# Alanlee0323/ISWM

Hardware: AMD Instinct MI355X
Metric: training images/sec (513x513) DeepLabV3+-ResNet101 (higher is better)
Workload: dtype f32; 1 GPU; deeplabv3plus_resnet101 output_stride=16, 513x513 synthetic tiles, 16 images/GPU (BASELINE.json configs[2]: global batch 128 over 8 GPUs), weighted CE [1,3], SGD-nesterov + cosine LR; fp32 tensors, conv products via six bf16 MFMAs on an exact 3-way operand split (bf16x6, fp32-level error); conv_math=bf16x6, global_batch=16, parallelism=dp1

## Files before the change

### include/iswm_hip.h

```cpp
#ifndef ISWM_HIP_H
#define ISWM_HIP_H

#include <stddef.h>
#include <stdint.h>

#ifdef __cplusplus
extern "C" {
#endif

typedef void* iswm_stream_t;

const char* iswm_last_error(void);
int iswm_version(void);

typedef struct {
    int N, H, W, Cin;
    int Ho, Wo, Cout;
    int KH, KW, stride, pad, dil;
    int ldx;
    int ldy;
} iswm_conv_desc;

int iswm_set_conv_math(int mode);
int iswm_get_conv_math(void);
int iswm_conv2d_kernel_name(const iswm_conv_desc* d, int kind, char* buf, int buflen);
int iswm_conv2d_stat_tile_rows(const iswm_conv_desc* d);
int iswm_conv2d_stat_tiles(const iswm_conv_desc* d);
int iswm_conv2d_fwd(const iswm_conv_desc* d, const float* x, const float* w, const float* bias,
                    float* y, float* stat_partials, iswm_stream_t stream);
int iswm_conv2d_dgrad(const iswm_conv_desc* d, const float* dy, const float* w, float* dx,
                      int accumulate, iswm_stream_t stream);
int iswm_transpose_weights(const iswm_conv_desc* d, const float* w, float* wt, iswm_stream_t stream);
int iswm_conv2d_dgrad_wants_wt(const iswm_conv_desc* d);
int iswm_conv2d_dgrad_wt(const iswm_conv_desc* d, const float* dy, const float* wt, float* dx, int accumulate,
                         iswm_stream_t stream);
size_t iswm_conv2d_packed_weight_bytes(const iswm_conv_desc* d, int kind);
int iswm_conv2d_pack_weights(const iswm_conv_desc* d, int kind, const float* w, void* packed, iswm_stream_t stream);
typedef struct iswm_pack_job {
    const float* w;
    void* packed;
    int Cout, taps, Cin, kind;
    int first_block, reserved;
} iswm_pack_job;
size_t iswm_packed_weight_bytes(int Cout, int taps, int Cin, int kind);
int iswm_pack_job_blocks(int Cout, int taps, int Cin, int kind);
int iswm_pack_weights_batch(const iswm_pack_job* jobs_dev, int njobs, int total_blocks, iswm_stream_t stream);
int iswm_conv2d_fwd_packed_stat_layout(const iswm_conv_desc* d, int* tiles, int* tile_rows);
int iswm_conv2d_fwd_packed(const iswm_conv_desc* d, const float* x, const void* wpk, const float* bias,
                           float* y, float* stat_partials, iswm_stream_t stream);
int iswm_conv2d_dgrad_packed(const iswm_conv_desc* d, const float* dy, const void* wpk, float* dx, int accumulate,
                             iswm_stream_t stream);
int iswm_split_planes(const float* x, int64_t M, int C, int ldx, void* planes, int ldp, int64_t plane_stride,
                      iswm_stream_t stream);
int iswm_join_planes(const void* planes, int ldp, int64_t plane_stride, int64_t M, int C, float* x, int ldx,
                     iswm_stream_t stream);
int iswm_bn_apply_pl(const float* y, int64_t M, int C, int ldy, const float* scale, const float* shift, const float* mean,
                     const void* residual, int ldr, int64_t res_ps, int relu, void* out, int ldo, int64_t out_ps,
                     iswm_stream_t stream);
int iswm_bn_backward_pl(const float* dout, int ldd, const void* out, int ldo, int64_t out_ps, const float* y, int ldy,
                        int64_t M, int C, const float* mean, const float* invstd, const float* gamma,
                        const float* mask_scale, const float* mask_shift, int relu, int training, float* dgamma,
                        float* dbeta, void* dy, int lddy, int64_t dy_ps, float* dres, int lddres, void* workspace,
                        size_t workspace_bytes, iswm_stream_t stream);
int iswm_maxpool3x3s2_fwd_pl(const float* x, int N, int H, int W, int C, void* y, int64_t y_ps, uint8_t* idx, int Ho,
                             int Wo, iswm_stream_t stream);
int iswm_gap_fwd_pl(const void* x, int64_t x_ps, int N, int HW, int C, int ldx, float* y, iswm_stream_t stream);
int iswm_bcast_fwd_pl(const float* v, int N, int HW, int C, void* y, int ldy, int64_t y_ps, iswm_stream_t stream);
int iswm_bilinear_fwd_pl(const float* x, int N, int Hi, int Wi, int C, int ldx, void* y, int64_t y_ps, int Ho, int Wo,
                         int ldy, iswm_stream_t stream);
size_t iswm_conv2d_pl2_weight_bytes(const iswm_conv_desc* d, int kind);
int iswm_conv2d_pl2_pack_weights(const iswm_conv_desc* d, int kind, const float* w, void* packed, iswm_stream_t stream);
int iswm_conv2d_pl2_tile_rows(const iswm_conv_desc* d, int kind);
int iswm_conv2d_fwd_pl2(const iswm_conv_desc* d, const void* xp, int64_t plane_stride, const void* wpk,
                        const float* bias, float* y, float* stat_partials, iswm_stream_t stream);
int iswm_conv2d_dgrad_pl2(const iswm_conv_desc* d, const void* dyp, int64_t plane_stride, const void* wpk,
                          float* dx, int accumulate, iswm_stream_t stream);
int iswm_conv2d_dgrad_pl2_stat_tiles(const iswm_conv_desc* d);
int iswm_conv2d_dgrad_pl2_bn(const iswm_conv_desc* d, const void* dyp, int64_t plane_stride, const void* wpk, float* dx,
                             int accumulate, const float* y, int ldy, const float* mean, const float* invstd,
                             const float* mask_scale, const float* mask_shift, int relu, const void* mask_hi,
                             int ld_mask, double* partials, int tiles, iswm_stream_t stream);
int iswm_bn_backward_stats_pl(const float* dout, int ldd, const void* out, int ldo, int64_t out_ps, const float* y, int ldy,
                              int64_t M, int C, const float* mean, const float* invstd, const float* gamma,
                              const float* mask_scale, const float* mask_shift, int relu, int training, float* dgamma,
                              float* dbeta, void* dy, int lddy, int64_t dy_ps, float* dres, int lddres,
                              const double* partials, int tiles, void* workspace, size_t workspace_bytes,
                              iswm_stream_t stream);
size_t iswm_aspp_plan_bytes(const iswm_conv_desc* d, int nbranch, const int* ksize, const int* dil, int kind);
int iswm_aspp_plan(const iswm_conv_desc* d, int nbranch, const int* ksize, const int* dil, int kind, void* host_plan,
                   int grid_hint);
int iswm_aspp_fwd(const iswm_conv_desc* d, int nbranch, const int* ksize, const int* dil, const void* plan_dev, const void* xp,
                  int64_t x_ps, const void* const* wpk, float* const* y, float* const* stats, iswm_stream_t stream);
int iswm_aspp_bwd(const iswm_conv_desc* d, int nbranch, const int* ksize, const int* dil, const void* plan_dev, const void* dyp,
                  int64_t dy_ps, int ld_dy, const void* const* wpk, float* dx, int accumulate, const void* xp, int64_t x_ps,
                  float* const* dw, float* workspace, size_t workspace_bytes, iswm_stream_t stream);
int iswm_conv2d_wgrad_planes_ok(const iswm_conv_desc* d);
size_t iswm_conv2d_wgrad_planes_workspace(const iswm_conv_desc* d);
int iswm_conv2d_wgrad_planes(const iswm_conv_desc* d, const void* xp, int64_t x_ps, const void* dyp, int64_t dy_ps, float* dw,
                             float* workspace, size_t workspace_bytes, iswm_stream_t stream);
int iswm_dwconv2d_fwd(const iswm_conv_desc* d, const float* x, const float* w, int Cw, const float* bias, float* y,
                      iswm_stream_t stream);
int iswm_dwconv2d_dgrad(const iswm_conv_desc* d, const float* dy, const float* w, int Cw, float* dx, int accumulate,
                        iswm_stream_t stream);
size_t iswm_dwconv2d_wgrad_workspace(const iswm_conv_desc* d);
int iswm_dwconv2d_wgrad(const iswm_conv_desc* d, const float* x, const float* dy, int Cw, float* dw, void* workspace,
                        size_t workspace_bytes, iswm_stream_t stream);
int iswm_dwconv3x3_stat_tile_rows(const iswm_conv_desc* d);
int iswm_dwconv3x3_stat_tiles(const iswm_conv_desc* d);
int iswm_dwconv3x3_fwd_stats(const iswm_conv_desc* d, const float* x, const float* w, int Cw, float* y,
                             float* stat_partials, iswm_stream_t stream);
size_t iswm_dwconv3x3_bwd_workspace(const iswm_conv_desc* d);
int iswm_dwconv3x3_bwd(const iswm_conv_desc* d, const float* x, const float* dy, const float* w, int Cw, float* dx,
                       int lddx, int accumulate, float* dw, void* workspace, size_t workspace_bytes, iswm_stream_t stream);
size_t iswm_conv2d_wgrad_workspace(const iswm_conv_desc* d);
int iswm_conv2d_wgrad(const iswm_conv_desc* d, const float* x, const float* dy, float* dw,
                      float* workspace, size_t workspace_bytes, iswm_stream_t stream);

int iswm_colstat_tiles(int64_t M);
int64_t iswm_colstat_tile_rows(int64_t M);
int iswm_colstat(const float* x, int64_t M, int C, int ld, float* partials, iswm_stream_t stream);
int iswm_bn_finalize(const float* partials, int tiles, int C, int64_t count, int64_t tile_rows,
                     const float* gamma, const float* beta, float* running_mean, float* running_var, float momentum,
                     float eps, float* scale, float* shift, float* save_mean, float* save_invstd,
                     iswm_stream_t stream);
int iswm_bn_eval_coeffs(int C, const float* gamma, const float* beta, const float* running_mean,
                        const float* running_var, float eps, float* scale, float* shift,
                        float* save_mean, float* save_invstd, iswm_stream_t stream);
int iswm_bn_apply(const float* y, int64_t M, int C, int ldy, const float* scale, const float* shift,
                  const float* mean, const float* residual, int ldr, int relu, float* out, int ldo,
                  iswm_stream_t stream);
size_t iswm_bn_bwd_workspace(int64_t M, int C);
int iswm_bn_backward(const float* dout, int ldd, const float* out, int ldo, const float* y, int ldy,
                     int64_t M, int C, const float* mean, const float* invstd, const float* gamma,
                     const float* mask_scale, const float* mask_shift,
                     int relu, int training, float* dgamma, float* dbeta, float* dy, int lddy,
                     float* dres, int lddres, void* workspace, size_t workspace_bytes,
                     iswm_stream_t stream);
int iswm_colsum_finalize(const float* partials, int tiles, int C, float* out, float* scratch,
                         iswm_stream_t stream);

int iswm_maxpool3x3s2_fwd(const float* x, int N, int H, int W, int C, float* y, uint8_t* idx, int Ho,
                          int Wo, iswm_stream_t stream);
int iswm_maxpool3x3s2_bwd(const float* dy, const uint8_t* idx, int N, int H, int W, int C, int Ho,
                          int Wo, float* dx, iswm_stream_t stream);
int iswm_gap_fwd(const float* x, int N, int HW, int C, int ldx, float* y, iswm_stream_t stream);
int iswm_gap_bwd(const float* dy, int N, int HW, int C, float* dx, int lddx, int accumulate,
                 iswm_stream_t stream);
int iswm_bcast_fwd(const float* v, int N, int HW, int C, float* y, int ldy, iswm_stream_t stream);
int iswm_bcast_bwd(const float* dy, int lddy, int N, int HW, int C, float* dv, iswm_stream_t stream);

int iswm_bilinear_fwd(const float* x, int N, int Hi, int Wi, int C, int ldx, float* y, int Ho, int Wo,
                      int ldy, iswm_stream_t stream);
int iswm_bilinear_bwd(const float* dy, int N, int Hi, int Wi, int C, int lddy, int Ho, int Wo, float* dx,
                      int lddx, iswm_stream_t stream);
int iswm_bilinear_nhwc_to_nchw_fwd(const float* x, int N, int Hi, int Wi, int C, int ldx, float* y,
                                   int Ho, int Wo, iswm_stream_t stream);
int iswm_bilinear_nhwc_to_nchw_bwd(const float* dy, int N, int Hi, int Wi, int C, int lddx, int Ho,
                                   int Wo, float* dx, iswm_stream_t stream);

int iswm_nchw_to_nhwc(const float* x, int N, int C, int HW, float* y, int Cp, iswm_stream_t stream);
int iswm_nhwc_to_nchw(const float* x, int N, int C, int HW, int ldx, float* y, iswm_stream_t stream);
int iswm_copy_channels(const float* src, int lds, float* dst, int ldd, int64_t M, int C,
                       iswm_stream_t stream);
int iswm_add_inplace(float* dst, const float* src, int64_t n, iswm_stream_t stream);
int iswm_scale_inplace(float* x, int64_t n, const float* scalar_dev, float host_mul, iswm_stream_t stream);
int iswm_bn_apply_classify(const float* y, int64_t M, int C, int ldy, const float* scale, const float* shift, const float* mean,
                           const float* wc4, const float* bias4, float* logits, int ldl, iswm_stream_t stream);
size_t iswm_bn_classify_bwd_workspace(int64_t M, int C);
int iswm_bn_backward_classify(const float* dlogit, int ldl, const float* wc4, const float* y, int ldy, int64_t M, int C,
                              const float* mean, const float* invstd, const float* gamma, const float* mask_scale,
                              const float* mask_shift, int training, float* dgamma, float* dbeta, float* dwc4, void* dy, int lddy,
                              int64_t dy_ps, void* workspace, size_t workspace_bytes, iswm_stream_t stream);
int iswm_pad_weights(const float* w, int cout, int cin, int kh, int kw, const int64_t* strides, int cout_p, int cin_p, float* out_ohwi,
                     iswm_stream_t stream);
int iswm_unpad_weights(const float* dw_ohwi, int cout_p, int cin_p, int cout, int cin, int kh, int kw, float* grad,
                       const int64_t* strides, iswm_stream_t stream);
int iswm_fill_zero(void* p, size_t bytes, iswm_stream_t stream);
int iswm_zero_cols(void* y, int64_t M, int64_t ld_bytes, int byte0, int byte1, int64_t plane_bytes, int nplanes, iswm_stream_t stream);
int iswm_dropout_fwd(const float* x, float* y, uint8_t* mask, int64_t n, float p, uint64_t seed,
                     uint64_t offset, iswm_stream_t stream);
int iswm_dropout_bwd(const float* dy, const uint8_t* mask, float* dx, int64_t n, float p,
                     iswm_stream_t stream);

int iswm_loss_blocks(int64_t npix);
int iswm_loss_fwd(const float* logits, const void* labels, int label_bytes, int B, int C, int64_t HW,
                  const float* class_weight, int ignore_index, float alpha, float gamma, int mode,
                  float* grad_unnorm, float* partials, iswm_stream_t stream);
int iswm_loss_finalize(const float* partials, int blocks, int mode, int64_t npix, float* sums,
                       float* loss, iswm_stream_t stream);
int iswm_loss_bwd_scale(float* grad, int64_t n, const float* sums, const float* upstream, int mode,
                        int64_t npix, iswm_stream_t stream);
int iswm_argmax_nchw(const float* logits, int B, int C, int64_t HW, int64_t* out, iswm_stream_t stream);

int iswm_confusion_matrix(const void* labels, int label_dtype, const void* preds, int pred_dtype, int64_t npix,
                          int n_classes, int64_t* hist, iswm_stream_t stream);
int iswm_confusion_matrix_logits(const void* labels, int label_dtype, const float* logits, int B, int C, int64_t HW,
                                 int n_classes, int64_t* hist, iswm_stream_t stream);

int iswm_mask_morph(const void* src, int src_dtype, int N, int H, int W, int radius, int dilate, uint8_t* dst,
                    iswm_stream_t stream);
int iswm_ccl(const uint8_t* mask, int N, int H, int W, int32_t* labels, int32_t* areas, iswm_stream_t stream);
size_t iswm_mask_preprocess_workspace(int N, int H, int W);
int iswm_mask_preprocess(const void* src, int src_dtype, int N, int H, int W, uint8_t* out, double* weight,
                         int64_t* area, void* workspace, size_t workspace_bytes, iswm_stream_t stream);
int iswm_mask_fronts(const uint8_t* mask, const double* weight, int N, int H, int W, int32_t* fronts, int64_t* stats,
                     iswm_stream_t stream);
int iswm_front_error(const int32_t* pred_fronts, const int32_t* gt_fronts, int N, int H, double tau, double* out,
                     iswm_stream_t stream);
int iswm_mask_pair_scores(const int32_t* curr_fronts, const int64_t* curr_stats, const uint8_t* prev_mask,
                          const double* prev_weight, const int64_t* prev_stats, int N, int H, int W, double* stability,
                          double* motion, iswm_stream_t stream);
size_t iswm_region_workspace(int N, int H, int W);
int iswm_region_score(const void* pred, int pred_dtype, const void* gt, int gt_dtype, int N, int H, int W, double* score,
                      int32_t* valid, void* workspace, size_t workspace_bytes, iswm_stream_t stream);

typedef struct iswm_aug_sample {
    long long img_off;
    long long lbl_off;
    int src_h, src_w;
    int rs_h, rs_w;
    int pad;
    int crop_i, crop_j;
    int flip;
    int tab_off;
    int ksize_h, ksize_v;
    int reserved;
} iswm_aug_sample;
int iswm_augment_batch(const unsigned char* images, const unsigned char* labels, const void* samples,
                       const int* tables, int B, int crop_h, int crop_w, const float* mean3, const float* std3,
                       float* out_nchw, unsigned char* out_labels, iswm_stream_t stream);

size_t iswm_label_prepare_workspace(long long nbytes);
int iswm_label_prepare(unsigned char* labels, long long nbytes, long long* counts, void* workspace,
                       size_t workspace_bytes, iswm_stream_t stream);
size_t iswm_label_count_workspace(long long n);
int iswm_label_count(const unsigned char* labels, long long n, int ignore_index, long long* counts_accum,
                     void* workspace, size_t workspace_bytes, iswm_stream_t stream);
size_t iswm_aug_tables_workspace(const void* host_samples, int B);
int iswm_aug_tables(const void* samples, int B, int max_rs, int* tables, size_t tables_bytes, iswm_stream_t stream);
int iswm_gather_normalize(const unsigned char* images, const unsigned char* labels, const long long* offsets, int B,
                          int H, int W, const float* mean3, const float* std3, float* out_nchw,
                          unsigned char* out_labels, iswm_stream_t stream);

int iswm_predict_normalize(const unsigned char* img, int N, int H, int W, const float* mean3, const float* std3,
                           float* out_nchw, iswm_stream_t stream);
size_t iswm_predict_maps_workspace(int N, int H, int W);
int iswm_predict_maps(const float* yl, int N, int Hi, int Wi, int ldx, int C, int fg, int Ho, int Wo, float thr,
                      int band_lo, int band_hi, unsigned char* pred, unsigned char* conf, unsigned char* band,
                      float* prob, double* stats, void* workspace, size_t workspace_bytes, iswm_stream_t stream);

typedef struct {
    int N, H, W, Cin;
    int Ho, Wo, Cout;
    int KH, KW, stride, pad, dil;
    int ldx;
    int ldy;
    int ldr;
    int relu;
    int lo;
    int out_f32;
    int cstore;
} iswm_qconv_desc;
size_t iswm_qconv_weight_bytes(const iswm_qconv_desc* d);
int iswm_qconv_fwd(const iswm_qconv_desc* d, const signed char* x, const signed char* w, const double* mul,
                   const double* add, const signed char* res, double s_res, double inv_s_out, void* y,
                   iswm_stream_t stream);
size_t iswm_absmax_workspace(int64_t rows, int C);
int iswm_absmax(const void* x, int64_t ps, int64_t rows, int C, int ld, float* slab, size_t slab_bytes, float* amax,
                iswm_stream_t stream);
int iswm_quantize_i8(const void* x, int64_t ps, int64_t rows, int C, int ld, double inv_s, int lo, signed char* y,
                     int ldy, iswm_stream_t stream);
int iswm_qgap(const signed char* x, int N, int HW, int C, int ldx, double s_in, double inv_s_in, signed char* y,
              int ldy, iswm_stream_t stream);
int iswm_qbcast(const signed char* v, int N, int HW, int C, int ldv, signed char* y, int ldy, iswm_stream_t stream);
int iswm_qbilinear(const signed char* x, int N, int Hi, int Wi, int C, int ldx, double s_in, int Ho, int Wo,
                   double inv_s_out, signed char* y, int ldy, iswm_stream_t stream);

int iswm_sgd_step(float* p, const float* g, float* buf, int64_t n, const float* lr_dev, float momentum,
                  float weight_decay, int nesterov, iswm_stream_t stream);
int iswm_adam_step(float* p, const float* g, float* m, float* v, int64_t n, const float* hyper_dev,
                   float beta1, float beta2, float eps, float weight_decay, int decoupled,
                   iswm_stream_t stream);

#ifdef __cplusplus
}
#endif
#endif
```

### iswm_amd/_lib.py

```python
import ctypes
import os
from ctypes import POINTER, Structure, c_char_p, c_double, c_float, c_int, c_int64, c_size_t, c_uint64, c_void_p

HERE = os.path.dirname(os.path.abspath(__file__))
LIB_PATH = os.path.join(HERE, "libiswm_hip.so")


class ConvDesc(Structure):
    _fields_ = [(n, c_int) for n in ("N", "H", "W", "Cin", "Ho", "Wo", "Cout", "KH", "KW", "stride", "pad",
                                     "dil", "ldx", "ldy")]


class QConvDesc(Structure):
    _fields_ = [(n, c_int) for n in ("N", "H", "W", "Cin", "Ho", "Wo", "Cout", "KH", "KW", "stride", "pad",
                                     "dil", "ldx", "ldy", "ldr", "relu", "lo", "out_f32", "cstore")]


P = c_void_p
_SIGS = {
    "iswm_last_error": (c_char_p, []),
    "iswm_version": (c_int, []),
    "iswm_set_conv_math": (c_int, [c_int]),
    "iswm_get_conv_math": (c_int, []),
    "iswm_conv2d_kernel_name": (c_int, [POINTER(ConvDesc), c_int, c_char_p, c_int]),
    "iswm_conv2d_stat_tile_rows": (c_int, [POINTER(ConvDesc)]),
    "iswm_conv2d_stat_tiles": (c_int, [POINTER(ConvDesc)]),
    "iswm_conv2d_fwd": (c_int, [POINTER(ConvDesc), P, P, P, P, P, P]),
    "iswm_conv2d_dgrad": (c_int, [POINTER(ConvDesc), P, P, P, c_int, P]),
    "iswm_transpose_weights": (c_int, [POINTER(ConvDesc), P, P, P]),
    "iswm_conv2d_dgrad_wants_wt": (c_int, [POINTER(ConvDesc)]),
    "iswm_conv2d_dgrad_wt": (c_int, [POINTER(ConvDesc), P, P, P, c_int, P]),
    "iswm_conv2d_packed_weight_bytes": (c_size_t, [POINTER(ConvDesc), c_int]),
    "iswm_conv2d_pack_weights": (c_int, [POINTER(ConvDesc), c_int, P, P, P]),
    "iswm_packed_weight_bytes": (c_size_t, [c_int, c_int, c_int, c_int]),
    "iswm_pack_job_blocks": (c_int, [c_int, c_int, c_int, c_int]),
    "iswm_pack_weights_batch": (c_int, [P, c_int, c_int, P]),
    "iswm_conv2d_fwd_packed_stat_layout": (c_int, [POINTER(ConvDesc), POINTER(c_int), POINTER(c_int)]),
    "iswm_conv2d_fwd_packed": (c_int, [POINTER(ConvDesc), P, P, P, P, P, P]),
    "iswm_conv2d_dgrad_packed": (c_int, [POINTER(ConvDesc), P, P, P, c_int, P]),
    "iswm_split_planes": (c_int, [P, c_int64, c_int, c_int, P, c_int, c_int64, P]),
    "iswm_join_planes": (c_int, [P, c_int, c_int64, c_int64, c_int, P, c_int, P]),
    "iswm_bn_apply_pl": (c_int, [P, c_int64, c_int, c_int, P, P, P, P, c_int, c_int64, c_int, P, c_int, c_int64, P]),
    "iswm_bn_backward_pl": (c_int, [P, c_int, P, c_int, c_int64, P, c_int, c_int64, c_int, P, P, P, P, P, c_int, c_int, P, P, P,
                                    c_int, c_int64, P, c_int, P, c_size_t, P]),
    "iswm_maxpool3x3s2_fwd_pl": (c_int, [P, c_int, c_int, c_int, c_int, P, c_int64, P, c_int, c_int, P]),
    "iswm_gap_fwd_pl": (c_int, [P, c_int64, c_int, c_int, c_int, c_int, P, P]),
    "iswm_bcast_fwd_pl": (c_int, [P, c_int, c_int, c_int, P, c_int, c_int64, P]),
    "iswm_bilinear_fwd_pl": (c_int, [P, c_int, c_int, c_int, c_int, c_int, P, c_int64, c_int, c_int, c_int, P]),
    "iswm_conv2d_pl2_weight_bytes": (c_size_t, [POINTER(ConvDesc), c_int]),
    "iswm_conv2d_pl2_pack_weights": (c_int, [POINTER(ConvDesc), c_int, P, P, P]),
    "iswm_conv2d_pl2_tile_rows": (c_int, [POINTER(ConvDesc), c_int]),
    "iswm_conv2d_fwd_pl2": (c_int, [POINTER(ConvDesc), P, c_int64, P, P, P, P, P]),
    "iswm_conv2d_dgrad_pl2": (c_int, [POINTER(ConvDesc), P, c_int64, P, P, c_int, P]),
    "iswm_conv2d_dgrad_pl2_stat_tiles": (c_int, [POINTER(ConvDesc)]),
    "iswm_conv2d_dgrad_pl2_bn": (c_int, [POINTER(ConvDesc), P, c_int64, P, P, c_int, P, c_int, P, P, P, P, c_int, P, c_int, P,
                                         c_int, P]),
    "iswm_bn_backward_stats_pl": (c_int, [P, c_int, P, c_int, c_int64, P, c_int, c_int64, c_int, P, P, P, P, P, c_int, c_int, P, P,
                                          P, c_int, c_int64, P, c_int, P, c_int, P, c_size_t, P]),
    "iswm_aspp_plan_bytes": (c_size_t, [POINTER(ConvDesc), c_int, POINTER(c_int), POINTER(c_int), c_int]),
    "iswm_aspp_plan": (c_int, [POINTER(ConvDesc), c_int, POINTER(c_int), POINTER(c_int), c_int, P, c_int]),
    "iswm_aspp_fwd": (c_int, [POINTER(ConvDesc), c_int, POINTER(c_int), POINTER(c_int), P, P, c_int64, POINTER(c_void_p),
                              POINTER(c_void_p), POINTER(c_void_p), P]),
    "iswm_aspp_bwd": (c_int, [POINTER(ConvDesc), c_int, POINTER(c_int), POINTER(c_int), P, P, c_int64, c_int, POINTER(c_void_p), P,
                              c_int, P, c_int64, POINTER(c_void_p), P, c_size_t, P]),
    "iswm_conv2d_wgrad_planes_ok": (c_int, [POINTER(ConvDesc)]),
    "iswm_conv2d_wgrad_planes_workspace": (c_size_t, [POINTER(ConvDesc)]),
    "iswm_conv2d_wgrad_planes": (c_int, [POINTER(ConvDesc), P, c_int64, P, c_int64, P, P, c_size_t, P]),
    "iswm_conv2d_wgrad_workspace": (c_size_t, [POINTER(ConvDesc)]),
    "iswm_dwconv2d_fwd": (c_int, [POINTER(ConvDesc), P, P, c_int, P, P, P]),
    "iswm_dwconv2d_dgrad": (c_int, [POINTER(ConvDesc), P, P, c_int, P, c_int, P]),
    "iswm_dwconv2d_wgrad_workspace": (c_size_t, [POINTER(ConvDesc)]),
    "iswm_dwconv2d_wgrad": (c_int, [POINTER(ConvDesc), P, P, c_int, P, P, c_size_t, P]),
    "iswm_dwconv3x3_stat_tile_rows": (c_int, [POINTER(ConvDesc)]),
    "iswm_dwconv3x3_stat_tiles": (c_int, [POINTER(ConvDesc)]),
    "iswm_dwconv3x3_fwd_stats": (c_int, [POINTER(ConvDesc), P, P, c_int, P, P, P]),
    "iswm_dwconv3x3_bwd_workspace": (c_size_t, [POINTER(ConvDesc)]),
    "iswm_dwconv3x3_bwd": (c_int, [POINTER(ConvDesc), P, P, P, c_int, P, c_int, c_int, P, P, c_size_t, P]),
    "iswm_conv2d_wgrad": (c_int, [POINTER(ConvDesc), P, P, P, P, c_size_t, P]),
    "iswm_colstat_tiles": (c_int, [c_int64]),
    "iswm_colstat_tile_rows": (c_int64, [c_int64]),
    "iswm_colstat": (c_int, [P, c_int64, c_int, c_int, P, P]),
    "iswm_bn_finalize": (c_int, [P, c_int, c_int, c_int64, c_int64, P, P, P, P, c_float, c_float, P, P, P, P, P]),
    "iswm_bn_eval_coeffs": (c_int, [c_int, P, P, P, P, c_float, P, P, P, P, P]),
    "iswm_bn_apply": (c_int, [P, c_int64, c_int, c_int, P, P, P, P, c_int, c_int, P, c_int, P]),
    "iswm_bn_bwd_workspace": (c_size_t, [c_int64, c_int]),
    "iswm_bn_backward": (c_int, [P, c_int, P, c_int, P, c_int, c_int64, c_int, P, P, P, P, P, c_int, c_int, P, P, P, c_int,
                                 P, c_int, P, c_size_t, P]),
    "iswm_colsum_finalize": (c_int, [P, c_int, c_int, P, P, P]),
    "iswm_maxpool3x3s2_fwd": (c_int, [P, c_int, c_int, c_int, c_int, P, P, c_int, c_int, P]),
    "iswm_maxpool3x3s2_bwd": (c_int, [P, P, c_int, c_int, c_int, c_int, c_int, c_int, P, P]),
    "iswm_gap_fwd": (c_int, [P, c_int, c_int, c_int, c_int, P, P]),
    "iswm_gap_bwd": (c_int, [P, c_int, c_int, c_int, P, c_int, c_int, P]),
    "iswm_bcast_fwd": (c_int, [P, c_int, c_int, c_int, P, c_int, P]),
    "iswm_bcast_bwd": (c_int, [P, c_int, c_int, c_int, c_int, P, P]),
    "iswm_bilinear_fwd": (c_int, [P, c_int, c_int, c_int, c_int, c_int, P, c_int, c_int, c_int, P]),
    "iswm_bilinear_bwd": (c_int, [P, c_int, c_int, c_int, c_int, c_int, c_int, c_int, P, c_int, P]),
    "iswm_bilinear_nhwc_to_nchw_fwd": (c_int, [P, c_int, c_int, c_int, c_int, c_int, P, c_int, c_int, P]),
    "iswm_bilinear_nhwc_to_nchw_bwd": (c_int, [P, c_int, c_int, c_int, c_int, c_int, c_int, c_int, P, P]),
    "iswm_nchw_to_nhwc": (c_int, [P, c_int, c_int, c_int, P, c_int, P]),
    "iswm_nhwc_to_nchw": (c_int, [P, c_int, c_int, c_int, c_int, P, P]),
    "iswm_copy_channels": (c_int, [P, c_int, P, c_int, c_int64, c_int, P]),
    "iswm_add_inplace": (c_int, [P, P, c_int64, P]),
    "iswm_scale_inplace": (c_int, [P, c_int64, P, c_float, P]),
    "iswm_bn_apply_classify": (c_int, [P, c_int64, c_int, c_int, P, P, P, P, P, P, c_int, P]),
    "iswm_bn_classify_bwd_workspace": (c_size_t, [c_int64, c_int]),
    "iswm_bn_backward_classify": (c_int, [P, c_int, P, P, c_int, c_int64, c_int, P, P, P, P, P, c_int, P, P, P, P, c_int, c_int64,
                                          P, c_size_t, P]),
    "iswm_pad_weights": (c_int, [P, c_int, c_int, c_int, c_int, P, c_int, c_int, P, P]),
    "iswm_unpad_weights": (c_int, [P, c_int, c_int, c_int, c_int, c_int, c_int, P, P, P]),
    "iswm_fill_zero": (c_int, [P, c_size_t, P]),
    "iswm_zero_cols": (c_int, [P, c_int64, c_int64, c_int, c_int, c_int64, c_int, P]),
    "iswm_dropout_fwd": (c_int, [P, P, P, c_int64, c_float, c_uint64, c_uint64, P]),
    "iswm_dropout_bwd": (c_int, [P, P, P, c_int64, c_float, P]),
    "iswm_loss_blocks": (c_int, [c_int64]),
    "iswm_loss_fwd": (c_int, [P, P, c_int, c_int, c_int, c_int64, P, c_int, c_float, c_float, c_int, P, P, P]),
    "iswm_loss_finalize": (c_int, [P, c_int, c_int, c_int64, P, P, P]),
    "iswm_loss_bwd_scale": (c_int, [P, c_int64, P, P, c_int, c_int64, P]),
    "iswm_argmax_nchw": (c_int, [P, c_int, c_int, c_int64, P, P]),
    "iswm_augment_batch": (c_int, [P, P, P, P, c_int, c_int, c_int, POINTER(c_float), POINTER(c_float), P, P, P]),
    "iswm_label_prepare_workspace": (c_size_t, [c_int64]),
    "iswm_label_prepare": (c_int, [P, c_int64, P, P, c_size_t, P]),
    "iswm_label_count_workspace": (c_size_t, [c_int64]),
    "iswm_label_count": (c_int, [P, c_int64, c_int, P, P, c_size_t, P]),
    "iswm_aug_tables_workspace": (c_size_t, [P, c_int]),
    "iswm_aug_tables": (c_int, [P, c_int, c_int, P, c_size_t, P]),
    "iswm_gather_normalize": (c_int, [P, P, P, c_int, c_int, c_int, POINTER(c_float), POINTER(c_float), P, P, P]),
    "iswm_confusion_matrix": (c_int, [P, c_int, P, c_int, c_int64, c_int, P, P]),
    "iswm_confusion_matrix_logits": (c_int, [P, c_int, P, c_int, c_int, c_int64, c_int, P, P]),
    "iswm_mask_morph": (c_int, [P, c_int, c_int, c_int, c_int, c_int, c_int, P, P]),
    "iswm_ccl": (c_int, [P, c_int, c_int, c_int, P, P, P]),
    "iswm_mask_preprocess_workspace": (c_size_t, [c_int, c_int, c_int]),
    "iswm_mask_preprocess": (c_int, [P, c_int, c_int, c_int, c_int, P, P, P, P, c_size_t, P]),
    "iswm_mask_fronts": (c_int, [P, P, c_int, c_int, c_int, P, P, P]),
    "iswm_front_error": (c_int, [P, P, c_int, c_int, c_double, P, P]),
    "iswm_mask_pair_scores": (c_int, [P, P, P, P, P, c_int, c_int, c_int, P, P, P]),
    "iswm_region_workspace": (c_size_t, [c_int, c_int, c_int]),
    "iswm_region_score": (c_int, [P, c_int, P, c_int, c_int, c_int, c_int, P, P, P, c_size_t, P]),
    "iswm_predict_normalize": (c_int, [P, c_int, c_int, c_int, POINTER(c_float), POINTER(c_float), P, P]),
    "iswm_predict_maps_workspace": (c_size_t, [c_int, c_int, c_int]),
    "iswm_predict_maps": (c_int, [P, c_int, c_int, c_int, c_int, c_int, c_int, c_int, c_int, c_float, c_int, c_int, P, P,
                                  P, P, P, P, c_size_t, P]),
    "iswm_qconv_weight_bytes": (c_size_t, [POINTER(QConvDesc)]),
    "iswm_qconv_fwd": (c_int, [POINTER(QConvDesc), P, P, P, P, P, c_double, c_double, P, P]),
    "iswm_absmax_workspace": (c_size_t, [c_int64, c_int]),
    "iswm_absmax": (c_int, [P, c_int64, c_int64, c_int, c_int, P, c_size_t, P, P]),
    "iswm_quantize_i8": (c_int, [P, c_int64, c_int64, c_int, c_int, c_double, c_int, P, c_int, P]),
    "iswm_qgap": (c_int, [P, c_int, c_int, c_int, c_int, c_double, c_double, P, c_int, P]),
    "iswm_qbcast": (c_int, [P, c_int, c_int, c_int, c_int, P, c_int, P]),
    "iswm_qbilinear": (c_int, [P, c_int, c_int, c_int, c_int, c_int, c_double, c_int, c_int, c_double, P, c_int, P]),
    "iswm_sgd_step": (c_int, [P, P, P, c_int64, P, c_float, c_float, c_int, P]),
    "iswm_adam_step": (c_int, [P, P, P, P, c_int64, P, c_float, c_float, c_float, c_float, c_int, P]),
}

EXPORTS = tuple(_SIGS)
_lib = None


class IswmError(RuntimeError):
    pass


def load():
    global _lib
    if _lib is not None:
        return _lib
    if not os.path.exists(LIB_PATH):
        raise ImportError(
            "libiswm_hip.so is not built (%s). Run `python -m iswm_amd.build` (hipcc, gfx950). "
            "iswm_amd has no CPU or torch-op fallback." % LIB_PATH)
    import torch
    lib = ctypes.CDLL(LIB_PATH)
    for name, (res, args) in _SIGS.items():
        fn = getattr(lib, name)
        fn.restype = res
        fn.argtypes = args
    _lib = lib
    return lib


def call(name, *args):
    lib = load()
    rc = getattr(lib, name)(*args)
    if rc != 0:
        msg = lib.iswm_last_error()
        raise IswmError("%s failed (%d): %s" % (name, rc, msg.decode() if msg else "?"))
```

### iswm_amd/csrc/conv_mfma.hip

```cpp
#include <stdlib.h>
#include <string.h>

#include <atomic>

#include "conv_common.h"

namespace iswm {

template <int BN>
__global__ __launch_bounds__(256, 2) void k_conv_fwd(const ConvArgs a) {
    constexpr int BM = 128;
    constexpr int NB = BN / 64;
    constexpr int BROWS = BN / 32;
    __shared__ __attribute__((aligned(16))) float smem[2 * (BM + BN) * KC_PITCH];
    float* As = smem;
    float* Bs = smem + 2 * BM * KC_PITCH;

    const int t = threadIdx.x, lane = t & 63, wave = t >> 6;
    const int wm = wave >> 1, wn = wave & 1, li = lane & 31, lh = lane >> 5;
    const int L = xcd_remap(blockIdx.x, gridDim.x);
    const int mt = L / a.NT, nt = L - mt * a.NT;
    const int m0 = mt * BM, n0 = nt * BN;
    const int q = t & 7, r0 = t >> 3;

// ... 435 lines not shown
                *reinterpret_cast<float4*>(&As[(buf * 32 + ak0 + AKR * j) * BM + aq * 4]) = ra[j];
#pragma unroll
            for (int j = 0; j < BPASS; ++j)
                *reinterpret_cast<float4*>(&Bs[(buf * 32 + bk0 + BKR * j) * BN + bq * 4]) = rb[j];
        }
    };

    f32x16 acc[MB][NB];
#pragma unroll
    for (int i = 0; i < MB; ++i)
#pragma unroll
        for (int j = 0; j < NB; ++j)
#pragma unroll
            for (int r = 0; r < 16; ++r) acc[i][j][r] = 0.f;

    const int nK = (p_end - p_begin + 31) >> 5;
    int kc = 0;
    bool first = true;
    auto next = [&]() -> bool {
        for (;;) {
            if (!first) {
                ++kc;
                if (kc < nK) advance(kc);
            }
            first = false;
            if (kc >= nK) return false;
            if (!skip(kc)) return true;
        }
    };
    if constexpr (X6) {
        const int tg = lane >> 4, ti = lane & 15, tq = ti >> 2, tp = ti & 3;
        const int th = tg >> 1, tc = (tg & 1) * 16 + tp * 4;
        typedef short s16x4 __attribute__((ext_vector_type(4)));
        typedef __attribute__((address_space(3))) s16x4* lds_s16x4;
        auto tr_frag = [&](const unsigned char* plane, int pitch, int sw, int col0, int ks) -> uint4 {
            const unsigned char* p = plane + (ks * 16 + th * 8 + tq) * pitch + (((col0 + tc) * 2) ^ (tq * sw));
            s16x4 lo = __builtin_amdgcn_ds_read_tr16_b64_v4i16((lds_s16x4)(p));
            s16x4 hi = __builtin_amdgcn_ds_read_tr16_b64_v4i16((lds_s16x4)(p + 4 * pitch));
            uint2 a2 = __builtin_bit_cast(uint2, lo), b2 = __builtin_bit_cast(uint2, hi);
            return make_uint4(a2.x, a2.y, b2.x, b2.y);
        };
        bool more = next();
        if (more) gload(kc);
        while (more) {
            lstore(0);
            __syncthreads();
            const bool more2 = next();
            if (more2) gload(kc);
#pragma unroll
            for (int ks = 0; ks < 2; ++ks) {
                uint4 ah[MB], am[MB], al[MB], bh[NB], bm[NB], bl[NB];
#pragma unroll
                for (int mb = 0; mb < MB; ++mb) {
                    const int c0 = wm * (BM / 2) + mb * 32;
                    ah[mb] = tr_frag(Ax, XPA, SWA, c0, ks);
                    if constexpr (NP == 3) {
                        am[mb] = tr_frag(Ax + XPLA, XPA, SWA, c0, ks);
                        al[mb] = tr_frag(Ax + 2 * XPLA, XPA, SWA, c0, ks);
                    }
                }
#pragma unroll
                for (int nb = 0; nb < NB; ++nb) {
                    const int c0 = wn * (BN / 2) + nb * 32;
                    bh[nb] = tr_frag(Bx, XPB, SWB, c0, ks);
                    if constexpr (NP == 3) {
                        bm[nb] = tr_frag(Bx + XPLB, XPB, SWB, c0, ks);
                        bl[nb] = tr_frag(Bx + 2 * XPLB, XPB, SWB, c0, ks);
                    }
                }
#pragma unroll
                for (int mb = 0; mb < MB; ++mb)
#pragma unroll
                    for (int nb = 0; nb < NB; ++nb) {
                        f32x16 c = acc[mb][nb];
                        if constexpr (NP == 3) {
                            c = mfma_bf16(al[mb], bh[nb], c);
                            c = mfma_bf16(ah[mb], bl[nb], c);
                            c = mfma_bf16(am[mb], bm[nb], c);
                            c = mfma_bf16(am[mb], bh[nb], c);
                            c = mfma_bf16(ah[mb], bm[nb], c);
                        }
                        c = mfma_bf16(ah[mb], bh[nb], c);
                        acc[mb][nb] = c;
                    }
            }
            __syncthreads();
            more = more2;
        }
    } else {
        bool more = next();
        if (more) {
            gload(kc);
            lstore(0);
        }
        __syncthreads();
        int cur = 0;
        while (more) {
            const bool more2 = next();
            if (more2) gload(kc);
            const float* Ab = &As[(cur * 32 + lh * 4) * BM + wm * (BM / 2) + li];
            const float* Bb = &Bs[(cur * 32 + lh * 4) * BN + wn * (BN / 2) + li];
    #pragma unroll
            for (int g = 0; g < 4; ++g) {
                float af[MB][4], bf[NB][4];
    #pragma unroll
                for (int mb = 0; mb < MB; ++mb)
    #pragma unroll
                    for (int j = 0; j < 4; ++j) af[mb][j] = Ab[(g * 8 + j) * BM + mb * 32];
    #pragma unroll
                for (int nb = 0; nb < NB; ++nb)
    #pragma unroll
                    for (int j = 0; j < 4; ++j) bf[nb][j] = Bb[(g * 8 + j) * BN + nb * 32];
    #pragma unroll
                for (int j = 0; j < 4; ++j)
    #pragma unroll
                    for (int mb = 0; mb < MB; ++mb)
    #pragma unroll
                        for (int nb = 0; nb < NB; ++nb)
                            acc[mb][nb] = mfma32(af[mb][j], bf[nb][j], acc[mb][nb]);
            }
            if (more2) lstore(cur ^ 1);
            __syncthreads();
            cur ^= 1;
            more = more2;
        }
    }
    float* out = a.stats + (size_t)split * a.Cout * a.Ktot;
#pragma unroll
    for (int nb = 0; nb < NB; ++nb) {
        const int col = n0 + wn * (BN / 2) + nb * 32 + li;
        const bool cok = col < a.Ktot;
#pragma unroll
        for (int mb = 0; mb < MB; ++mb)
#pragma unroll
            for (int r = 0; r < 16; ++r) {
                int row = m0 + wm * (BM / 2) + mb * 32 + (r & 3) + 8 * (r >> 2) + 4 * lh;
                if (cok && row < a.Cout) out[(size_t)row * a.Ktot + col] = acc[mb][nb][r];
            }
    }
}

__global__ void k_reduce_slabs(const float* __restrict__ slabs, float* __restrict__ dst, int64_t n4,
                               int nsplit) {
    for (int64_t i = blockIdx.x * (int64_t)blockDim.x + threadIdx.x; i < n4;
         i += (int64_t)gridDim.x * blockDim.x) {
        const float4* p = reinterpret_cast<const float4*>(slabs) + i;
        float4 s = p[0];
        int k = 1;
        for (; k + 7 < nsplit; k += 8) {
            float4 v[8];
#pragma unroll
            for (int u = 0; u < 8; ++u) v[u] = p[(int64_t)(k + u) * n4];
#pragma unroll
            for (int u = 0; u < 8; ++u) {
                s.x += v[u].x;
                s.y += v[u].y;
                s.z += v[u].z;
                s.w += v[u].w;
            }
        }
        for (; k < nsplit; ++k) {
            const float4 v = p[(int64_t)k * n4];
            s.x += v.x;
            s.y += v.y;
            s.z += v.z;
            s.w += v.w;
        }
        reinterpret_cast<float4*>(dst)[i] = s;
    }
}

void launch_reduce_slabs(const float* slabs, float* dst, int64_t n4, int nsplit, hipStream_t s) {
    hipLaunchKernelGGL(k_reduce_slabs, dim3(stream_grid(n4, 256)), dim3(256), 0, s, slabs, dst, n4, nsplit);
}

static int validate(const iswm_conv_desc* d) {
    ISWM_REQUIRE(d != nullptr, "conv: null descriptor");
    ISWM_REQUIRE(d->N > 0 && d->H > 0 && d->W > 0 && d->Cin > 0 && d->Cout > 0, "conv: empty tensor");
    ISWM_REQUIRE(d->Cin % 4 == 0 && d->Cout % 4 == 0, "conv: Cin (%d) and Cout (%d) must be multiples of 4",
                 d->Cin, d->Cout);
    ISWM_REQUIRE(d->ldx % 4 == 0 && d->ldy % 4 == 0 && d->ldx >= d->Cin && d->ldy >= d->Cout,
                 "conv: bad pixel pitch ldx=%d ldy=%d", d->ldx, d->ldy);
    ISWM_REQUIRE(d->KH > 0 && d->KW > 0 && d->stride > 0 && d->dil > 0 && d->pad >= 0, "conv: bad geometry");
    int ho = (d->H + 2 * d->pad - d->dil * (d->KH - 1) - 1) / d->stride + 1;
    int wo = (d->W + 2 * d->pad - d->dil * (d->KW - 1) - 1) / d->stride + 1;
    ISWM_REQUIRE(ho == d->Ho && wo == d->Wo, "conv: output size %dx%d does not match geometry (%dx%d)", d->Ho,
                 d->Wo, ho, wo);
    ISWM_REQUIRE((int64_t)d->N * d->H * d->W * d->ldx < (1ll << 31) &&
                     (int64_t)d->N * d->Ho * d->Wo * d->ldy < (1ll << 31),
                 "conv: tensor exceeds 2^31 elements");
    return 0;
}

static bool use_narrow_tile(int64_t MT, int cols) {
    if (cols <= 64 || (cols % 128 != 0 && cols % 128 <= 64)) return true;
    const int64_t t128 = MT * ((cols + 127) / 128), t64 = MT * ((cols + 63) / 64);
    const double c128 = (double)((t128 + 255) / 256) * 128.0;
    const double c64 = (double)((t64 + 255) / 256) * 64.0 * 1.10;
    return c64 < c128;
}

static ConvArgs base_args(const iswm_conv_desc* d) {
    ConvArgs a{};
    a.N = d->N; a.H = d->H; a.W = d->W; a.Cin = d->Cin;
    a.Ho = d->Ho; a.Wo = d->Wo; a.Cout = d->Cout;
    a.KH = d->KH; a.KW = d->KW; a.stride = d->stride; a.pad = d->pad; a.dil = d->dil;
    a.ldx = d->ldx; a.ldy = d->ldy;
    return a;
}

struct WgradPlan {
    int bm, bn, MT, NT, nsplit, psplit;
};

static WgradPlan plan_wgrad(const iswm_conv_desc* d, bool x6) {
    WgradPlan p;
    const int Ktot = d->KH * d->KW * d->Cin;
    p.bm = (d->Cout % 128 == 0) ? 128 : 64;
    p.bn = (p.bm == 128 && (Ktot % 128 == 0 || Ktot >= 1024)) ? 128 : 64;
    if (p.bn == 64) p.bm = 64;
    p.MT = (d->Cout + p.bm - 1) / p.bm;
    p.NT = (Ktot + p.bn - 1) / p.bn;
    const int64_t P = (int64_t)d->N * d->Ho * d->Wo;
    const int64_t tiles = (int64_t)p.MT * p.NT;
    (void)x6;
    const int64_t slots = 512;
    const double chunk_us = 4.5 * (double)(p.bm * p.bn) / 16384.0;
    const double slab_us = (double)d->Cout * Ktot * 8.0 / 4.0e6;
    int64_t maxs = (P + 255) / 256;
    if (maxs > 64) maxs = 64;
    double best = 1e300;
    p.psplit = (int)((P + 31) / 32 * 32);
    p.nsplit = 1;
    for (int64_t ns = 1; ns <= maxs; ++ns) {
        int64_t ps = ((P + ns - 1) / ns + 31) / 32 * 32;
        int64_t nsp = (P + ps - 1) / ps;
        int64_t rounds = (tiles * nsp + slots - 1) / slots;
        double t = (double)rounds * (double)(ps / 32 + 3) * chunk_us + (nsp > 1 ? (double)nsp * slab_us + 5.0 : 0.0);
        if (t < best) {
            best = t;
            p.psplit = (int)ps;
            p.nsplit = (int)nsp;
        }
    }
    return p;
}

}

using namespace iswm;

static std::atomic<int> g_conv_math{-1};
static int conv_math() {
    int m = g_conv_math.load();
    if (m < 0) {
        const char* e = getenv("ISWM_CONV_MATH");
        const int env = (e && (!strcmp(e, "f32") || !strcmp(e, "0"))) ? 0
                        : (e && (!strcmp(e, "bf16") || !strcmp(e, "2"))) ? 2 : 1;
        int unset = -1;
        g_conv_math.compare_exchange_strong(unset, env);
        m = g_conv_math.load();
    }
    return m;
}
extern "C" int iswm_set_conv_math(int mode) {
    ISWM_REQUIRE(mode >= 0 && mode <= 2, "set_conv_math: mode must be 0 (f32), 1 (bf16x6) or 2 (bf16)");
    g_conv_math = mode;
    return 0;
}
extern "C" int iswm_get_conv_math(void) { return conv_math(); }
static int math_planes() { return conv_math() == 2 ? 1 : 3; }

static bool patch_plan(const iswm_conv_desc* d, bool dgrad, int* PH, int* PW) {
    if (d->stride != 1 || d->KH * d->KW <= 1) return false;
    return dgrad ? conv_patch_plan(d->H, d->W, d->KH, d->KW, d->dil, PH, PW)
                 : conv_patch_plan(d->Ho, d->Wo, d->KH, d->KW, d->dil, PH, PW);
}

static PatchArgs patch_args(const iswm_conv_desc* d, bool dgrad, int PH, int PW) {
    PatchArgs p{};
    p.N = d->N;
    p.KH = d->KH; p.KW = d->KW; p.dil = d->dil;
    p.PH = PH; p.PW = PW;
    if (!dgrad) {
        p.RH = d->Ho; p.RW = d->Wo; p.GH = d->H; p.GW = d->W; p.GC = d->Cin; p.NC = d->Cout;
        p.orgh = -d->pad; p.orgw = -d->pad; p.flip = 0; p.ldg = d->ldx; p.ldo = d->ldy;
    } else {
        p.RH = d->H; p.RW = d->W; p.GH = d->Ho; p.GW = d->Wo; p.GC = d->Cout; p.NC = d->Cin;
        p.orgh = d->pad - d->dil * (d->KH - 1); p.orgw = d->pad - d->dil * (d->KW - 1);
        p.flip = 1; p.ldg = d->ldy; p.ldo = d->ldx;
    }
    return p;
}

namespace iswm { int wgrad_pl_is_wide(const iswm_conv_desc* d); int wgrad_pl_kernel_kind(const iswm_conv_desc* d); }

static bool pl2_wide_ok(const iswm_conv_desc* d, bool dgrad) {
    if (math_planes() != 3 || (dgrad && d->stride != 1)) return false;
    return !dgrad || d->KH * d->KW * d->Cout >= 512;
}
static int pl2_K(const iswm_conv_desc* d, bool dgrad) { return d->KH * d->KW * (dgrad ? d->Cout : d->Cin); }

extern "C" int iswm_conv2d_kernel_name(const iswm_conv_desc* d, int kind, char* buf, int buflen) {
    ISWM_REQUIRE(d && buf && buflen > 0 && kind >= 0 && kind <= 7, "kernel_name: bad argument");
    if (kind == 7) {
        const int kk = wgrad_pl_kernel_kind(d);
        snprintf(buf, buflen, kk == 2 ? "k_wgrad_pls<%d>" : kk == 1 ? "k_wgrad_plw<%d>" : "k_wgrad_pl<%d>", math_planes());
        return 0;
    }
    if (kind >= 5) {
        const bool dg = kind == 6;
        const int cols = dg ? d->Cin : d->Cout;
        int rbw, wide;
        conv_pl2_plan(dg ? (int64_t)d->N * d->H * d->W : (int64_t)d->N * d->Ho * d->Wo, cols, pl2_K(d, dg), pl2_wide_ok(d, dg), &rbw, &wide);
        if (wide) snprintf(buf, buflen, "k_conv_pl2w<%d, %d, %s>", rbw, math_planes(), dg ? "true" : "false");
        else if (cols <= 64) snprintf(buf, buflen, "k_conv_pl2<%d, 2, %d, %s>", rbw / 2, math_planes(), dg ? "true" : "false");
        else snprintf(buf, buflen, "k_conv_pl2<%d, 1, %d, %s>", rbw, math_planes(), dg ? "true" : "false");
        return 0;
    }
    if (kind >= 3) {
        const bool dg = kind == 4;
        int pbm, pbn;
        if (patch_plan(d, dg, &pbm, &pbn)) {
            snprintf(buf, buflen, "k_conv_x6_patch<%s, %d>", dg ? "true" : "false", math_planes());
            return 0;
        }
        conv_pick_tile_x6(dg ? (int64_t)d->N * d->H * d->W : (int64_t)d->N * d->Ho * d->Wo, dg ? d->Cin : d->Cout,
                          d->KH * d->KW * (dg ? d->Cout : d->Cin), dg, d->KH * d->KW == 1, &pbm, &pbn);
        snprintf(buf, buflen, "k_conv_x6<%d, 64, %s, true, %d>", pbm, dg ? "true" : "false", math_planes());
        return 0;
    }
    int bm, bn;
    if (kind == 0) {
        const int64_t M = (int64_t)d->N * d->Ho * d->Wo;
        if (d->Cin % 32 == 0) {
            if (conv_math() == 1) conv_pick_tile_x6(M, d->Cout, d->KH * d->KW * d->Cin, false, d->KH * d->KW == 1, &bm, &bn);
            else conv_pick_tile(M, d->Cout, &bm, &bn);
            snprintf(buf, buflen, conv_math() == 1 ? "k_conv_x6<%d, %d, false, false, 3>" : "k_conv_fwd_u<%d, %d>", bm, bn);
        } else if (conv_math() == 1 && stem_geometry(base_args(d))) {
            snprintf(buf, buflen, "k_stem_fwd<%d>", stem_tile_rows() / 16);
        } else {
            snprintf(buf, buflen, "k_conv_fwd<%d>", use_narrow_tile((M + 127) / 128, d->Cout) ? 64 : 128);
        }
    } else if (kind == 1) {
        const int64_t M = (int64_t)d->N * d->H * d->W;
        if (d->Cout % 32 == 0) {
            if (conv_math() == 1) conv_pick_tile_x6(M, d->Cin, d->KH * d->KW * d->Cout, true, d->KH * d->KW == 1, &bm, &bn);
            else conv_pick_tile(M, d->Cin, &bm, &bn);
            if (conv_math() == 1) snprintf(buf, buflen, "k_conv_x6<%d, %d, true, false, 3>", bm, bn);
            else snprintf(buf, buflen, "k_conv_dgrad_u<%d, %d>", bm, bn);
        } else {
            snprintf(buf, buflen, "k_conv_dgrad<%d>", use_narrow_tile((M + 127) / 128, d->Cin) ? 64 : 128);
        }
    } else {
        if (conv_math() == 1 && stem_geometry(base_args(d))) {
            snprintf(buf, buflen, "k_stem_wgrad");
            return 0;
        }
        WgradPlan p = plan_wgrad(d, conv_math() >= 1);
        const bool same = d->stride == 1 && d->Ho == d->H && d->Wo == d->W;
        const int mode = (same && d->KH == 1 && d->KW == 1 && d->pad == 0) ? 2 : (same ? 1 : 0);
        snprintf(buf, buflen, "k_conv_wgrad<%d, %d, %d, %s, %d>", p.bm, p.bn, mode, conv_math() >= 1 ? "true" : "false",
                 conv_math() == 2 ? 1 : 3);
    }
    return 0;
}

extern "C" int iswm_conv2d_stat_tile_rows(const iswm_conv_desc* d) {
    if (!d) return 0;
    if (conv_math() == 1 && stem_geometry(base_args(d))) return stem_tile_rows();
    if (conv_math() == 1 && d->Cin % 32 == 0) {
        int bm, bn;
        conv_pick_tile_x6((int64_t)d->N * d->Ho * d->Wo, d->Cout, d->KH * d->KW * d->Cin, false, d->KH * d->KW == 1, &bm, &bn);
        return bm;
    }
    return conv_fwd_tile_rows((int64_t)d->N * d->Ho * d->Wo, d->Cin, d->Cout);
}

extern "C" int iswm_conv2d_stat_tiles(const iswm_conv_desc* d) {
    if (!d) return 0;
    const int64_t M = (int64_t)d->N * d->Ho * d->Wo, R = iswm_conv2d_stat_tile_rows(d);
    return (int)((M + R - 1) / R);
}

extern "C" int iswm_conv2d_fwd(const iswm_conv_desc* d, const float* x, const float* w, const float* bias,
                               float* y, float* stat_partials, iswm_stream_t stream) {
    if (int e = validate(d)) return e;
    ISWM_REQUIRE(x && w && y, "conv_fwd: null pointer");
    ISWM_REQUIRE(aligned16(x) && aligned16(w) && aligned16(y), "conv_fwd: pointers must be 16-byte aligned");
    ConvArgs a = base_args(d);
    a.x = x; a.w = w; a.bias = bias; a.y = y; a.stats = stat_partials;
    a.M = d->N * d->Ho * d->Wo;
    a.Ktot = d->KH * d->KW * d->Cin;
    a.MT = (a.M + 127) / 128;
    hipStream_t s = (hipStream_t)stream;
    if (conv_math() == 1 && launch_stem_fwd(a, s)) return check_launch("stem_fwd");
    if (conv_math() == 1 && d->Cin % 32 == 0) {
        int bm, bn;
        conv_pick_tile_x6(a.M, d->Cout, a.Ktot, false, d->KH * d->KW == 1, &bm, &bn);
        if (launch_conv_fwd_x6(a, s, bm, bn)) return check_launch("conv_fwd_x6");
    }
    if (launch_conv_fwd_u(a, s)) return check_launch("conv_fwd_u");
    if (use_narrow_tile(a.MT, d->Cout)) {
        a.NT = (d->Cout + 63) / 64;
        hipLaunchKernelGGL(k_conv_fwd<64>, dim3(a.MT * a.NT), dim3(256), 0, s, a);
    } else {
        a.NT = (d->Cout + 127) / 128;
        hipLaunchKernelGGL(k_conv_fwd<128>, dim3(a.MT * a.NT), dim3(256), 0, s, a);
    }
    return check_launch("conv_fwd");
}

extern "C" int iswm_conv2d_dgrad(const iswm_conv_desc* d, const float* dy, const float* w, float* dx,
                                 int accumulate, iswm_stream_t stream) {
    if (int e = validate(d)) return e;
    ISWM_REQUIRE(dy && w && dx, "conv_dgrad: null pointer");
    ISWM_REQUIRE(aligned16(dy) && aligned16(w) && aligned16(dx), "conv_dgrad: pointers must be 16-byte aligned");
    ConvArgs a = base_args(d);
    a.x = dy; a.w = w; a.y = dx; a.accumulate = accumulate;
    a.ldx = d->ldy; a.ldy = d->ldx;
    a.M = d->N * d->H * d->W;
    a.Ktot = d->KH * d->KW * d->Cout;
    a.MT = (a.M + 127) / 128;
    hipStream_t s = (hipStream_t)stream;
    if (launch_conv_dgrad_u(a, s)) return check_launch("conv_dgrad_u");
    if (use_narrow_tile(a.MT, d->Cin)) {
        a.NT = (d->Cin + 63) / 64;
        hipLaunchKernelGGL(k_conv_dgrad<64>, dim3(a.MT * a.NT), dim3(256), 0, s, a);
    } else {
        a.NT = (d->Cin + 127) / 128;
        hipLaunchKernelGGL(k_conv_dgrad<128>, dim3(a.MT * a.NT), dim3(256), 0, s, a);
    }
    return check_launch("conv_dgrad");
}

extern "C" int iswm_transpose_weights(const iswm_conv_desc* d, const float* w, float* wt, iswm_stream_t stream) {
    if (int e = validate(d)) return e;
    ISWM_REQUIRE(w && wt && w != wt, "transpose_weights: bad pointer");
    launch_transpose_ohwi(w, wt, d->Cout, d->KH * d->KW, d->Cin, (hipStream_t)stream);
    return check_launch("transpose_weights");
}

extern "C" int iswm_conv2d_dgrad_wants_wt(const iswm_conv_desc* d) {
    return (d && conv_math() == 1 && d->Cout % 32 == 0) ? 1 : 0;
}

extern "C" int iswm_conv2d_dgrad_wt(const iswm_conv_desc* d, const float* dy, const float* wt, float* dx,
                                    int accumulate, iswm_stream_t stream) {
    if (int e = validate(d)) return e;
    ISWM_REQUIRE(dy && wt && dx, "conv_dgrad_wt: null pointer");
    ISWM_REQUIRE(aligned16(dy) && aligned16(wt) && aligned16(dx), "conv_dgrad_wt: pointers must be 16-byte aligned");
    ISWM_REQUIRE(d->Cout % 32 == 0, "conv_dgrad_wt: Cout must be a multiple of 32");
    ConvArgs a = base_args(d);
    a.x = dy; a.w = wt; a.y = dx; a.accumulate = accumulate;
    a.ldx = d->ldy; a.ldy = d->ldx;
    a.M = d->N * d->H * d->W;
    a.Ktot = d->KH * d->KW * d->Cout;
    int bm, bn;
    conv_pick_tile_x6(a.M, d->Cin, a.Ktot, true, d->KH * d->KW == 1, &bm, &bn);
    launch_conv_dgrad_x6(a, (hipStream_t)stream, bm, bn);
    return check_launch("conv_dgrad_x6");
}

extern "C" int iswm_conv2d_fwd_packed_stat_layout(const iswm_conv_desc* d, int* tiles, int* tile_rows) {
    ISWM_REQUIRE(d && tiles && tile_rows, "fwd_packed_stat_layout: null pointer");
    int PH, PW;
    if (patch_plan(d, false, &PH, &PW)) {
        *tiles = d->N * ((d->Ho + PH - 1) / PH) * ((d->Wo + PW - 1) / PW);
        *tile_rows = 0;
    } else {
        int bm, bn;
        const int64_t M = (int64_t)d->N * d->Ho * d->Wo;
        conv_pick_tile_x6(M, d->Cout, d->KH * d->KW * d->Cin, false, d->KH * d->KW == 1, &bm, &bn);
        *tile_rows = bm;
        *tiles = (int)((M + bm - 1) / bm);
    }
    return 0;
}

extern "C" size_t iswm_conv2d_packed_weight_bytes(const iswm_conv_desc* d, int kind) {
    if (!d || conv_math() < 1 || (kind != 0 && kind != 1)) return 0;
    const int gc = kind ? d->Cout : d->Cin;
    if (gc % 32 != 0) return 0;
    return packed_weight_bytes_x6(d->Cout, d->KH * d->KW, d->Cin, kind == 1, math_planes());
}

extern "C" int iswm_conv2d_pack_weights(const iswm_conv_desc* d, int kind, const float* w, void* packed,
                                        iswm_stream_t stream) {
    if (int e = validate(d)) return e;
    ISWM_REQUIRE(kind == 0 || kind == 1, "pack_weights: kind must be 0 (forward) or 1 (data gradient)");
    ISWM_REQUIRE(w && packed && aligned16(packed), "pack_weights: bad pointer");
    ISWM_REQUIRE((kind ? d->Cout : d->Cin) % 32 == 0, "pack_weights: gathered channel count must be a multiple of 32");
    launch_pack_weights_x6(w, packed, d->Cout, d->KH * d->KW, d->Cin, kind == 1, math_planes(), (hipStream_t)stream);
    return check_launch("pack_weights");
}

extern "C" size_t iswm_packed_weight_bytes(int Cout, int taps, int Cin, int kind) {
    if (Cout <= 0 || taps <= 0 || Cin <= 0 || kind < 0 || kind > 3 || conv_math() < 1) return 0;
    if (kind >= 2) {
        if (((kind == 3) ? Cout : Cin) % 64 != 0) return 0;
        return packed_weight_bytes_pl2(Cout, taps, Cin, kind == 3, math_planes());
    }
    if ((kind ? Cout : Cin) % 32 != 0) return 0;
    return packed_weight_bytes_x6(Cout, taps, Cin, kind == 1, math_planes());
}

extern "C" int iswm_pack_job_blocks(int Cout, int taps, int Cin, int kind) {
    if (iswm_packed_weight_bytes(Cout, taps, Cin, kind) == 0) return 0;
    if (kind >= 2) return pack_job_blocks_pl2(Cout, taps, Cin, kind == 3);
    return pack_job_blocks_x6(Cout, taps, Cin, kind == 1);
}

extern "C" int iswm_pack_weights_batch(const iswm_pack_job* jobs_dev, int njobs, int total_blocks,
                                       iswm_stream_t stream) {
    ISWM_REQUIRE(jobs_dev && njobs > 0 && total_blocks > 0, "pack_weights_batch: bad argument");
    static_assert(sizeof(iswm_pack_job) == 40, "iswm_pack_job layout");
    launch_pack_weights_batch(jobs_dev, njobs, total_blocks, math_planes(), (hipStream_t)stream);
    return check_launch("pack_weights_batch");
}

extern "C" int iswm_conv2d_fwd_packed(const iswm_conv_desc* d, const float* x, const void* wpk, const float* bias,
                                      float* y, float* stat_partials, iswm_stream_t stream) {
    if (int e = validate(d)) return e;
    ISWM_REQUIRE(x && wpk && y, "conv_fwd_packed: null pointer");
    ISWM_REQUIRE(aligned16(x) && aligned16(wpk) && aligned16(y), "conv_fwd_packed: pointers must be 16-byte aligned");
    ISWM_REQUIRE(d->Cin % 32 == 0, "conv_fwd_packed: Cin must be a multiple of 32");
    ConvArgs a = base_args(d);
    a.x = x; a.w = reinterpret_cast<const float*>(wpk); a.bias = bias; a.y = y; a.stats = stat_partials;
    a.M = d->N * d->Ho * d->Wo;
    a.Ktot = d->KH * d->KW * d->Cin;
    int PH, PW;
    if (patch_plan(d, false, &PH, &PW)) {
        PatchArgs p = patch_args(d, false, PH, PW);
        p.x = x; p.wpk = reinterpret_cast<const uint4*>(wpk); p.bias = bias; p.y = y; p.stats = stat_partials;
        launch_conv_x6_patch(p, false, math_planes(), (hipStream_t)stream);
        return check_launch("conv_fwd_patch");
    }
    int bm, bn;
    conv_pick_tile_x6(a.M, d->Cout, a.Ktot, false, d->KH * d->KW == 1, &bm, &bn);
    launch_conv_x6_pk(a, (hipStream_t)stream, false, bm, math_planes());
    return check_launch("conv_fwd_packed");
}

extern "C" int iswm_conv2d_dgrad_packed(const iswm_conv_desc* d, const float* dy, const void* wpk, float* dx,
                                        int accumulate, iswm_stream_t stream) {
    if (int e = validate(d)) return e;
    ISWM_REQUIRE(dy && wpk && dx, "conv_dgrad_packed: null pointer");
    ISWM_REQUIRE(aligned16(dy) && aligned16(wpk) && aligned16(dx), "conv_dgrad_packed: pointers must be 16-byte aligned");
    ISWM_REQUIRE(d->Cout % 32 == 0, "conv_dgrad_packed: Cout must be a multiple of 32");
    ConvArgs a = base_args(d);
    a.x = dy; a.w = reinterpret_cast<const float*>(wpk); a.y = dx; a.accumulate = accumulate;
    a.ldx = d->ldy; a.ldy = d->ldx;
    a.M = d->N * d->H * d->W;
    a.Ktot = d->KH * d->KW * d->Cout;
    int PH, PW;
    if (patch_plan(d, true, &PH, &PW)) {
        PatchArgs p = patch_args(d, true, PH, PW);
        p.x = dy; p.wpk = reinterpret_cast<const uint4*>(wpk); p.y = dx; p.accumulate = accumulate;
        launch_conv_x6_patch(p, true, math_planes(), (hipStream_t)stream);
        return check_launch("conv_dgrad_patch");
    }
    int bm, bn;
    conv_pick_tile_x6(a.M, d->Cin, a.Ktot, true, d->KH * d->KW == 1, &bm, &bn);
    launch_conv_x6_pk(a, (hipStream_t)stream, true, bm, math_planes());
    return check_launch("conv_dgrad_packed");
}

extern "C" int iswm_split_planes(const float* x, int64_t M, int C, int ldx, void* planes, int ldp, int64_t plane_stride,
                                 iswm_stream_t stream) {
    ISWM_REQUIRE(x && planes && M > 0 && C > 0, "split_planes: bad argument");
    ISWM_REQUIRE(C % 4 == 0 && ldx % 4 == 0 && ldx >= C && ldp % 4 == 0 && ldp >= C, "split_planes: C %d ldx %d ldp %d", C, ldx, ldp);
    ISWM_REQUIRE(aligned16(x) && plane_stride % 4 == 0 && plane_stride >= M * ldp,
                 "split_planes: planes must be 16-byte aligned and disjoint");
    launch_split_planes(x, M, C, ldx, (unsigned short*)planes, ldp, plane_stride, math_planes(), (hipStream_t)stream);
    return check_launch("split_planes");
}

extern "C" int iswm_join_planes(const void* planes, int ldp, int64_t plane_stride, int64_t M, int C, float* x, int ldx,
                                iswm_stream_t stream) {
    ISWM_REQUIRE(x && planes && M > 0 && C > 0, "join_planes: bad argument");
    ISWM_REQUIRE(C % 4 == 0 && ldx % 4 == 0 && ldx >= C && ldp % 4 == 0 && ldp >= C, "join_planes: C %d ldx %d ldp %d", C, ldx, ldp);
    ISWM_REQUIRE(plane_stride == -1 || plane_stride >= M * ldp, "join_planes: bad plane stride");
    launch_join_planes((const unsigned short*)planes, ldp, plane_stride, M, C, x, ldx, (hipStream_t)stream);
    return check_launch("join_planes");
}

extern "C" size_t iswm_conv2d_pl2_weight_bytes(const iswm_conv_desc* d, int kind) {
    if (!d || conv_math() < 1 || (kind != 0 && kind != 1)) return 0;
    const int gc = kind ? d->Cout : d->Cin;
    if (gc % 64 != 0) return 0;
    return packed_weight_bytes_pl2(d->Cout, d->KH * d->KW, d->Cin, kind == 1, math_planes());
}

extern "C" int iswm_conv2d_pl2_pack_weights(const iswm_conv_desc* d, int kind, const float* w, void* packed,
                                            iswm_stream_t stream) {
    if (int e = validate(d)) return e;
    ISWM_REQUIRE(kind == 0 || kind == 1, "pl2_pack_weights: kind must be 0 (forward) or 1 (data gradient)");
    ISWM_REQUIRE(w && packed && aligned16(packed), "pl2_pack_weights: bad pointer");
    ISWM_REQUIRE((kind ? d->Cout : d->Cin) % 64 == 0, "pl2_pack_weights: gathered channel count must be a multiple of 64");
    launch_pack_weights_pl2(w, packed, d->Cout, d->KH * d->KW, d->Cin, kind == 1, math_planes(), (hipStream_t)stream);
    return check_launch("pl2_pack_weights");
}

extern "C" int iswm_conv2d_pl2_tile_rows(const iswm_conv_desc* d, int kind) {
    if (!d) return 0;
    int rbw, wide;
    if (kind) conv_pl2_plan((int64_t)d->N * d->H * d->W, d->Cin, pl2_K(d, true), pl2_wide_ok(d, true), &rbw, &wide);
// ... 134 lines not shown
```

### iswm_amd/csrc/conv_wgrad_pl.hip

```cpp
#include <stdlib.h>

#include <algorithm>
#include <type_traits>

#include "conv_common.h"

namespace iswm {

static __device__ __attribute__((aligned(256))) unsigned short g_zero_row_wg[128];

struct WgArgs {
    const unsigned short* dy;
    const unsigned short* x;
    float* out;
    long long dyps, xps;
    int N, H, W, Cin, Ho, Wo, Cout, KH, KW, stride, pad, dil, ldx, ldy;
    int P, Ktot, MT, NT, nsplit, psplit;
    int always;
    int vote;
    int rect;
    unsigned char tap_order[32];
};

template <int NP>
// ... 117 lines not shown
#pragma unroll
        for (int mb = 0; mb < 2; ++mb)
#pragma unroll
            for (int pl = 0; pl < NP; ++pl) af[mb][pl] = tr_frag(Ax + pl * PLANE, wm * 64 + mb * 32);
#pragma unroll
        for (int nb = 0; nb < 2; ++nb)
#pragma unroll
            for (int pl = 0; pl < NP; ++pl) bf[nb][pl] = tr_frag(Bx + pl * PLANE, wn * 64 + nb * 32);
#pragma unroll
        for (int mb = 0; mb < 2; ++mb)
#pragma unroll
            for (int nb = 0; nb < 2; ++nb) {
                f32x16 c = acc[mb][nb];
                if constexpr (NP == 3) {
                    c = mfma_bf16(af[mb][2], bf[nb][0], c);
                    c = mfma_bf16(af[mb][0], bf[nb][2], c);
                    c = mfma_bf16(af[mb][1], bf[nb][1], c);
                    c = mfma_bf16(af[mb][1], bf[nb][0], c);
                    c = mfma_bf16(af[mb][0], bf[nb][1], c);
                }
                c = mfma_bf16(af[mb][0], bf[nb][0], c);
                acc[mb][nb] = c;
            }
    };

    {
        int nissued = 0, wr = 0, rd = 0;
        bool src_more = true;
        auto advance = [&]() __attribute__((always_inline)) -> bool {
            if (src_more && next()) return true;
            src_more = false;
            return false;
        };
        auto post = [&]() __attribute__((always_inline)) {
            issue(wr);
            wr = wr == NST - 1 ? 0 : wr + 1;
            ++nissued;
        };
        if (advance()) post();
        if (advance()) post();
        while (nissued > 0) {
            if (nissued >= 2) {
                if constexpr (NP == 3) __builtin_amdgcn_s_waitcnt(0x0F76);
                else __builtin_amdgcn_s_waitcnt(0x0F72);
            } else {
                __builtin_amdgcn_s_waitcnt(0x0F70);
            }
            __builtin_amdgcn_s_barrier();
            asm volatile("" ::: "memory");
            if (advance()) post();
            compute(rd);
            rd = rd == NST - 1 ? 0 : rd + 1;
            --nissued;
        }
    }

    __syncthreads();
    float* xch = reinterpret_cast<float*>(smem);
    if (kh == 1) {
#pragma unroll
        for (int mb = 0; mb < 2; ++mb)
#pragma unroll
            for (int nb = 0; nb < 2; ++nb)
#pragma unroll
                for (int r = 0; r < 16; ++r) xch[((((wm * 2 + wn) * 2 + mb) * 2 + nb) * 16 + r) * 64 + lane] = acc[mb][nb][r];
    }
    __syncthreads();
    if (kh == 0) {
        float* out = a.out + (size_t)split * a.Cout * a.Ktot;
        const int li = lane & 31, lh = lane >> 5;
#pragma unroll
        for (int nb = 0; nb < 2; ++nb) {
            const int col = n0 + wn * 64 + nb * 32 + li;
            const bool cok = col < a.Ktot;
#pragma unroll
            for (int mb = 0; mb < 2; ++mb)
#pragma unroll
                for (int r = 0; r < 16; ++r) {
                    const int row = m0 + wm * 64 + mb * 32 + (r & 3) + 8 * (r >> 2) + 4 * lh;
                    const float v = acc[mb][nb][r] + xch[((((wm * 2 + wn) * 2 + mb) * 2 + nb) * 16 + r) * 64 + lane];
                    if (cok && row < a.Cout) out[(size_t)row * a.Ktot + col] = v;
                }
        }
    }
}


template <int NP>
__global__ __launch_bounds__(512, 2) void k_wgrad_plw(const WgArgs a) {
    constexpr int PLANE = 32 * 256;
    constexpr int IMG = NP * PLANE;
    constexpr int STAGE = 3 * IMG;
    constexpr int NST = 2;
    constexpr int SMEM = NST * STAGE < 65536 ? 65536 : NST * STAGE;
    __shared__ __attribute__((aligned(1024))) unsigned char smem[SMEM];
    const unsigned lds_base = (unsigned)(uintptr_t)(lds_vptr)smem;

    const int t = threadIdx.x, lane = t & 63;
    const int wave = __builtin_amdgcn_readfirstlane(t >> 6);
    const int wm = wave >> 2, wn = wave & 3;
    const int tiles = a.MT * a.NT;
    const int L = xcd_remap(blockIdx.x, gridDim.x);
    const int split = L / tiles, tile = L - split * tiles;
    const int mt = tile / a.NT, nt = tile - mt * a.NT;
    const int m0 = mt * 128, n0 = nt * 256;
    const int p_begin = split * a.psplit;
    const int p_end = min(a.P, p_begin + a.psplit);
    const int nK = (p_end - p_begin + 31) >> 5;

    const int kr = 4 * wave + (lane >> 4);
    const int gsrc = (lane & 15) ^ (4 * ((lane >> 4) & 3));
    const unsigned char* zrow = reinterpret_cast<const unsigned char*>(g_zero_row_wg) + (lane & 15) * 16;
    const int ach = m0 + 8 * gsrc;
    const bool aok = ach < a.Cout;
    const unsigned char* abase = reinterpret_cast<const unsigned char*>(a.dy) + (size_t)ach * 2;
    bool bok[2];
    int dh[2], dw[2];
    const unsigned char* bbase[2];
#pragma unroll
    for (int i = 0; i < 2; ++i) {
        const int bcol = n0 + 128 * i + 8 * gsrc;
        bok[i] = bcol < a.Ktot;
        const int tap = bok[i] ? bcol / a.Cin : 0, bch = bok[i] ? bcol - tap * a.Cin : 0;
        const int tkh = tap / a.KW, tkw = tap - tkh * a.KW;
        dh[i] = tkh * a.dil - a.pad;
        dw[i] = tkw * a.dil - a.pad;
        bbase[i] = reinterpret_cast<const unsigned char*>(a.x) + (size_t)bch * 2;
    }
    const int HoWo = a.Ho * a.Wo;

    const unsigned char* asrc = zrow;
    const unsigned char* bsrc[2] = {zrow, zrow};
    long long apst = 0, bpst[2] = {0, 0};
    int kc = -1;
    int pn, poh, pow_;
    {
        const int p = p_begin + kr;
        pn = p / HoWo;
        const int rem = p - pn * HoWo;
        poh = rem / a.Wo;
        pow_ = rem - poh * a.Wo;
    }
    const int d_oh = 32 / a.Wo, d_ow = 32 - d_oh * a.Wo;
    const bool fast_adv = d_oh + 1 <= a.Ho;
    auto next = [&]() __attribute__((always_inline)) -> bool {
        for (;;) {
            if (++kc >= nK) return false;
            const int p = p_begin + kc * 32 + kr;
            const bool pin = p < p_end;
            asrc = (pin && aok) ? abase + (size_t)p * a.ldy * 2 : zrow;
            apst = (pin && aok) ? a.dyps : 0;
            if (a.always) {
#pragma unroll
                for (int i = 0; i < 2; ++i) {
                    const bool v = pin && bok[i];
                    bsrc[i] = v ? bbase[i] + (size_t)p * a.ldx * 2 : zrow;
                    bpst[i] = v ? a.xps : 0;
                }
                return true;
            }
            if (kc > 0) {
                if (fast_adv) {
                    int ow = pow_ + d_ow;
                    const int c1 = ow >= a.Wo ? 1 : 0;
                    pow_ = ow - (c1 ? a.Wo : 0);
                    int oh = poh + d_oh + c1;
                    const int c2 = oh >= a.Ho ? 1 : 0;
                    poh = oh - (c2 ? a.Ho : 0);
                    pn += c2;
                } else {
                    pn = p / HoWo;
                    const int rem = p - pn * HoWo;
                    poh = rem / a.Wo;
                    pow_ = rem - poh * a.Wo;
                }
            }
            bool any = false;
#pragma unroll
            for (int i = 0; i < 2; ++i) {
                const int ih = poh * a.stride + dh[i], iw = pow_ * a.stride + dw[i];
                const bool v = pin && bok[i] && (unsigned)ih < (unsigned)a.H && (unsigned)iw < (unsigned)a.W;
                bsrc[i] = v ? bbase[i] + (size_t)((pn * a.H + ih) * a.W + iw) * a.ldx * 2 : zrow;
                bpst[i] = v ? a.xps : 0;
                any = any || v;
            }
            if (!a.vote) return true;
            if (__syncthreads_or(any ? 1 : 0)) return true;
        }
    };
    auto dma = [&](int i, int st) __attribute__((always_inline)) {
        const int img = i / NP, pl = i - img * NP;
        const unsigned dst = lds_base + st * STAGE + img * IMG + pl * PLANE + wave * 1024;
        if (img == 0) glds16b(asrc + pl * apst, dst);
        else glds16b(bsrc[img - 1] + pl * bpst[img - 1], dst);
    };
    auto issue = [&](int st) __attribute__((always_inline)) {
#pragma unroll
        for (int i = 0; i < 3 * NP; ++i) dma(i, st);
    };

    const int tg = lane >> 4, ti = lane & 15, tq = ti >> 2, tp = ti & 3;
    const int th = tg >> 1, tc = (tg & 1) * 16 + tp * 4;
    typedef short s16x4 __attribute__((ext_vector_type(4)));
    typedef __attribute__((address_space(3))) s16x4* lds_s16x4;
    auto tr_frag = [&](const unsigned char* plane, int ks, int col0) __attribute__((always_inline)) -> uint4 {
        const unsigned char* p = plane + (ks * 16 + th * 8 + tq) * 256 + (((col0 + tc) * 2) ^ (tq * 64));
        s16x4 lo = __builtin_amdgcn_ds_read_tr16_b64_v4i16((lds_s16x4)(p));
        s16x4 hi = __builtin_amdgcn_ds_read_tr16_b64_v4i16((lds_s16x4)(p + 4 * 256));
        uint2 a2 = __builtin_bit_cast(uint2, lo), b2 = __builtin_bit_cast(uint2, hi);
        return make_uint4(a2.x, a2.y, b2.x, b2.y);
    };

    f32x16 acc[2][2];
#pragma unroll
    for (int i = 0; i < 2; ++i)
#pragma unroll
        for (int j = 0; j < 2; ++j)
#pragma unroll
            for (int r = 0; r < 16; ++r) acc[i][j][r] = 0.f;

    uint4 F[4][NP];
    auto ldA = [&](int st, int mb, int ks) __attribute__((always_inline)) {
        const unsigned char* Ax = smem + st * STAGE;
#pragma unroll
        for (int pl = 0; pl < NP; ++pl) F[mb][pl] = tr_frag(Ax + pl * PLANE, ks, wm * 64 + mb * 32);
    };
    auto ldB = [&](int st, int nb, int ks) __attribute__((always_inline)) {
        const unsigned char* Bx = smem + st * STAGE + (1 + (wn >> 1)) * IMG;
#pragma unroll
        for (int pl = 0; pl < NP; ++pl) F[2 + nb][pl] = tr_frag(Bx + pl * PLANE, ks, (wn & 1) * 64 + nb * 32);
    };
    auto mm = [&](int mb, int nb) __attribute__((always_inline)) {
        f32x16 c = acc[mb][nb];
        if constexpr (NP == 3) {
            c = mfma_bf16(F[mb][2], F[2 + nb][0], c);
            c = mfma_bf16(F[mb][0], F[2 + nb][2], c);
            c = mfma_bf16(F[mb][1], F[2 + nb][1], c);
            c = mfma_bf16(F[mb][1], F[2 + nb][0], c);
            c = mfma_bf16(F[mb][0], F[2 + nb][1], c);
        }
        c = mfma_bf16(F[mb][0], F[2 + nb][0], c);
        acc[mb][nb] = c;
    };
    auto compute = [&](int st) __attribute__((always_inline)) {
#define ISWM_SB() __builtin_amdgcn_sched_barrier(0)
        ldA(st, 0, 0); ldB(st, 0, 0);
        ISWM_SB(); ldB(st, 1, 0); ISWM_SB(); mm(0, 0); ISWM_SB();
        ISWM_SB(); ldA(st, 1, 0); ISWM_SB(); mm(0, 1); ISWM_SB();
        ISWM_SB(); ldA(st, 0, 1); ISWM_SB(); mm(1, 1); ISWM_SB();
        ISWM_SB(); ldB(st, 1, 1); ISWM_SB(); mm(1, 0); ISWM_SB();
        ISWM_SB(); ldB(st, 0, 1); ISWM_SB(); mm(0, 1); ISWM_SB();
        ISWM_SB(); ldA(st, 1, 1); ISWM_SB(); mm(0, 0); ISWM_SB();
        ISWM_SB(); mm(1, 0); ISWM_SB();
        ISWM_SB(); mm(1, 1); ISWM_SB();
        ISWM_SB();
#undef ISWM_SB
    };

    {
        bool have = next();
        if (have) issue(0);
        int st = 0;
        while (have) {
            __builtin_amdgcn_s_waitcnt(0x0F70);
            __builtin_amdgcn_s_barrier();
            asm volatile("" ::: "memory");
            const bool more = next();
            if (more) issue(st ^ 1);
            compute(st);
            st ^= 1;
            have = more;
        }
    }

    if (a.nsplit > 1) {
        float4* slab = reinterpret_cast<float4*>(a.out) + ((size_t)split * tiles + tile) * 8192 + (size_t)wave * 1024 + lane;
#pragma unroll
        for (int mb = 0; mb < 2; ++mb)
#pragma unroll
            for (int nb = 0; nb < 2; ++nb)
#pragma unroll
                for (int q = 0; q < 4; ++q)
                    slab[((mb * 2 + nb) * 4 + q) * 64] =
                        make_float4(acc[mb][nb][4 * q], acc[mb][nb][4 * q + 1], acc[mb][nb][4 * q + 2], acc[mb][nb][4 * q + 3]);
        return;
    }
    float* out = a.out;
    const int li = lane & 31, lh = lane >> 5;
#pragma unroll
    for (int nb = 0; nb < 2; ++nb) {
        const int col = n0 + wn * 64 + nb * 32 + li;
        const bool cok = col < a.Ktot;
#pragma unroll
        for (int mb = 0; mb < 2; ++mb)
#pragma unroll
            for (int r = 0; r < 16; ++r) {
                const int row = m0 + wm * 64 + mb * 32 + (r & 3) + 8 * (r >> 2) + 4 * lh;
                if (cok && row < a.Cout) out[(size_t)row * a.Ktot + col] = acc[mb][nb][r];
            }
    }
}

template <int NP>
__global__ __launch_bounds__(512, 2) void k_wgrad_pls(const WgArgs a) {
    constexpr int MW = 4;
    constexpr int KS = 16;
    constexpr int PLANE = KS * 256;
    constexpr int IMG = NP * PLANE;
    constexpr int STAGE = 3 * IMG;
    constexpr int NST = 4;
    __shared__ __attribute__((aligned(1024))) unsigned char smem[NST * STAGE];
    const unsigned lds_base = (unsigned)(uintptr_t)(lds_vptr)smem;

    const int t = threadIdx.x, lane = t & 63;
    const int wave = __builtin_amdgcn_readfirstlane(t >> 6);
    const int tiles = a.MT * a.NT;
    const int L = xcd_remap(blockIdx.x, gridDim.x);
    int split = L / tiles, tile = L - split * tiles;
    int mt = tile / a.NT;
    int nt = tile - mt * a.NT;
    if (a.rect == 2) {
        const int idx = blockIdx.x >> 3, per_split = (a.NT >> 3) * a.MT;
        split = idx / per_split;
        const int rem = idx - split * per_split;
        mt = rem % a.MT;
        nt = (rem / a.MT) * 8 + (blockIdx.x & 7);
    }
    int r_oh0 = 0, r_ow0 = 0, r_h = a.Ho, r_w = a.Wo, r_dh = 0, r_dw = 0;
    int p_begin = split * a.psplit;
    int p_end = min(a.P, p_begin + a.psplit);
    if (a.rect) {
        const int chunks = a.Cin >> 8;
        const int slot = nt / chunks;
        const int tap = a.tap_order[slot];
        nt = tap * chunks + (nt - slot * chunks);
        const int tkh = tap / a.KW, tkw = tap - tkh * a.KW;
        r_dh = tkh * a.dil - a.pad;
        r_dw = tkw * a.dil - a.pad;
        r_oh0 = max(0, -r_dh);
        r_ow0 = max(0, -r_dw);
        r_h = max(0, min(a.Ho, a.H - r_dh) - r_oh0);
        r_w = max(0, min(a.Wo, a.W - r_dw) - r_ow0);
        const int Pt = a.N * r_h * r_w;
        const int per = (((Pt + a.nsplit - 1) / a.nsplit) + KS - 1) / KS * KS;
        p_begin = split * per;
        p_end = min(Pt, p_begin + per);
    }
    const int m0 = mt * 128, n0 = nt * 256;
    const int nK = p_end > p_begin ? (p_end - p_begin + KS - 1) / KS : 0;

    if (wave >= MW) {
        const int rg = wave - MW;
        const int kr = 4 * rg + (lane >> 4);
        const int gsrc = (lane & 15) ^ (4 * ((lane >> 4) & 3));
        const unsigned char* zrow = reinterpret_cast<const unsigned char*>(g_zero_row_wg) + (lane & 15) * 16;
        const int ach = m0 + 8 * gsrc;
        const bool aok = ach < a.Cout;
        const unsigned char* abase = reinterpret_cast<const unsigned char*>(a.dy) + (size_t)ach * 2;
        bool bok[2];
        int dh[2], dw[2];
        const unsigned char* bbase[2];
#pragma unroll
        for (int i = 0; i < 2; ++i) {
            const int bcol = n0 + 128 * i + 8 * gsrc;
            bok[i] = bcol < a.Ktot;
            const int tap = bok[i] ? bcol / a.Cin : 0, bch = bok[i] ? bcol - tap * a.Cin : 0;
            const int tkh = tap / a.KW, tkw = tap - tkh * a.KW;
            dh[i] = tkh * a.dil - a.pad;
            dw[i] = tkw * a.dil - a.pad;
            bbase[i] = reinterpret_cast<const unsigned char*>(a.x) + (size_t)bch * 2;
        }
        const int GW_ = max(1, r_w), GHW = max(1, r_h * r_w);
        int pn, poh, pow_;
        {
            const int p = p_begin + kr;
            pn = p / GHW;
            const int rem = p - pn * GHW;
            poh = rem / GW_;
            pow_ = rem - poh * GW_;
        }
        const int d_oh = KS / GW_, d_ow = KS - d_oh * GW_;
        const bool fast_adv = d_oh + 1 <= r_h;
        auto issue = [&](int kc) __attribute__((always_inline)) {
            const int p = p_begin + kc * KS + kr;
            const bool pin = p < p_end;
            const unsigned char* asrc;
            long long apst;
            const unsigned char* bsrc[2];
            long long bpst[2];
            if (a.rect) {
                if (kc > 0) {
                    if (fast_adv) {
                        int ow = pow_ + d_ow;
                        const int c1 = ow >= GW_ ? 1 : 0;
                        pow_ = ow - (c1 ? GW_ : 0);
                        int oh = poh + d_oh + c1;
                        const int c2 = oh >= r_h ? 1 : 0;
                        poh = oh - (c2 ? r_h : 0);
                        pn += c2;
                    } else {
                        pn = p / GHW;
                        const int rem = p - pn * GHW;
                        poh = rem / GW_;
                        pow_ = rem - poh * GW_;
                    }
                }
                const int oh = r_oh0 + poh, ow = r_ow0 + pow_;
                const bool va = pin && aok;
                asrc = va ? abase + (size_t)((pn * a.Ho + oh) * a.Wo + ow) * a.ldy * 2 : zrow;
                apst = va ? a.dyps : 0;
                const size_t xpix = (size_t)((pn * a.H + oh + r_dh) * a.W + ow + r_dw);
#pragma unroll
                for (int i = 0; i < 2; ++i) {
                    const bool v = pin && bok[i];
                    bsrc[i] = v ? bbase[i] + xpix * a.ldx * 2 : zrow;
                    bpst[i] = v ? a.xps : 0;
                }
                const unsigned dstr = lds_base + (kc & 3) * STAGE + rg * 1024;
#pragma unroll
                for (int pl = 0; pl < NP; ++pl) glds16b(asrc + pl * apst, dstr + pl * PLANE);
#pragma unroll
                for (int i = 0; i < 2; ++i)
#pragma unroll
                    for (int pl = 0; pl < NP; ++pl) glds16b(bsrc[i] + pl * bpst[i], dstr + (1 + i) * IMG + pl * PLANE);
                return;
            }
            asrc = (pin && aok) ? abase + (size_t)p * a.ldy * 2 : zrow;
            apst = (pin && aok) ? a.dyps : 0;
            if (a.always) {
#pragma unroll
                for (int i = 0; i < 2; ++i) {
                    const bool v = pin && bok[i];
                    bsrc[i] = v ? bbase[i] + (size_t)p * a.ldx * 2 : zrow;
                    bpst[i] = v ? a.xps : 0;
                }
            } else {
                if (kc > 0) {
                    if (fast_adv) {
                        int ow = pow_ + d_ow;
                        const int c1 = ow >= GW_ ? 1 : 0;
                        pow_ = ow - (c1 ? GW_ : 0);
                        int oh = poh + d_oh + c1;
                        const int c2 = oh >= r_h ? 1 : 0;
                        poh = oh - (c2 ? r_h : 0);
                        pn += c2;
                    } else {
                        pn = p / GHW;
                        const int rem = p - pn * GHW;
                        poh = rem / GW_;
                        pow_ = rem - poh * GW_;
                    }
                }
#pragma unroll
                for (int i = 0; i < 2; ++i) {
                    const int ih = poh * a.stride + dh[i], iw = pow_ * a.stride + dw[i];
                    const bool v = pin && bok[i] && (unsigned)ih < (unsigned)a.H && (unsigned)iw < (unsigned)a.W;
                    bsrc[i] = v ? bbase[i] + (size_t)((pn * a.H + ih) * a.W + iw) * a.ldx * 2 : zrow;
                    bpst[i] = v ? a.xps : 0;
                }
            }
            const unsigned dst = lds_base + (kc & 3) * STAGE + rg * 1024;
#pragma unroll
            for (int pl = 0; pl < NP; ++pl) glds16b(asrc + pl * apst, dst + pl * PLANE);
#pragma unroll
            for (int i = 0; i < 2; ++i)
#pragma unroll
                for (int pl = 0; pl < NP; ++pl) glds16b(bsrc[i] + pl * bpst[i], dst + (1 + i) * IMG + pl * PLANE);
        };
        const int pre = nK < 3 ? nK : 3;
        for (int kc = 0; kc < pre; ++kc) issue(kc);
        for (int s2 = 0; s2 < nK; ++s2) {
            const int beyond = min(nK - 1, s2 + 2) - s2;
            if constexpr (NP == 3) {
                if (beyond >= 2) __builtin_amdgcn_s_waitcnt(0x4F72);
                else if (beyond == 1) __builtin_amdgcn_s_waitcnt(0x0F79);
                else __builtin_amdgcn_s_waitcnt(0x0F70);
            } else {
                if (beyond >= 2) __builtin_amdgcn_s_waitcnt(0x0F76);
                else if (beyond == 1) __builtin_amdgcn_s_waitcnt(0x0F73);
                else __builtin_amdgcn_s_waitcnt(0x0F70);
            }
            __builtin_amdgcn_s_barrier();
            asm volatile("" ::: "memory");
            if (s2 + 3 < nK) issue(s2 + 3);
        }
        return;
    }

    constexpr int NBW = 4;
    const int wm = wave >> 1;
    const int wn4 = 2 * (wave & 1);
    const int tg = lane >> 4, ti = lane & 15, tq = ti >> 2, tp = ti & 3;
    const int th = tg >> 1, tc = (tg & 1) * 16 + tp * 4;
    typedef short s16x4 __attribute__((ext_vector_type(4)));
    typedef __attribute__((address_space(3))) s16x4* lds_s16x4;
    auto tr_frag = [&](const unsigned char* plane, int col0) __attribute__((always_inline)) -> uint4 {
        const unsigned char* p = plane + (th * 8 + tq) * 256 + (((col0 + tc) * 2) ^ (tq * 64));
        s16x4 lo = __builtin_amdgcn_ds_read_tr16_b64_v4i16((lds_s16x4)(p));
        s16x4 hi = __builtin_amdgcn_ds_read_tr16_b64_v4i16((lds_s16x4)(p + 4 * 256));
        uint2 a2 = __builtin_bit_cast(uint2, lo), b2 = __builtin_bit_cast(uint2, hi);
        return make_uint4(a2.x, a2.y, b2.x, b2.y);
    };
    f32x16 acc[2][NBW];
#pragma unroll
    for (int i = 0; i < 2; ++i)
#pragma unroll
        for (int j = 0; j < NBW; ++j)
#pragma unroll
            for (int r = 0; r < 16; ++r) acc[i][j][r] = 0.f;
    uint4 FA[2][NP], FB[NBW][NP];
    auto ldA = [&](int slot, int mb) __attribute__((always_inline)) {
        const unsigned char* Ax = smem + slot * STAGE;
#pragma unroll
        for (int pl = 0; pl < NP; ++pl) FA[mb][pl] = tr_frag(Ax + pl * PLANE, wm * 64 + mb * 32);
    };
    auto ldB = [&](int slot, int nb) __attribute__((always_inline)) {
        const unsigned char* Bx = smem + slot * STAGE + (1 + (wn4 >> 1)) * IMG;
#pragma unroll
        for (int pl = 0; pl < NP; ++pl) FB[nb][pl] = tr_frag(Bx + pl * PLANE, (wn4 & 1) * 64 + nb * 32);
    };
    auto mm = [&](int mb, int nb) __attribute__((always_inline)) {
        f32x16 c = acc[mb][nb];
        if constexpr (NP == 3) {
            c = mfma_bf16(FA[mb][2], FB[nb][0], c);
            c = mfma_bf16(FA[mb][0], FB[nb][2], c);
            c = mfma_bf16(FA[mb][1], FB[nb][1], c);
            c = mfma_bf16(FA[mb][1], FB[nb][0], c);
            c = mfma_bf16(FA[mb][0], FB[nb][1], c);
        }
        c = mfma_bf16(FA[mb][0], FB[nb][0], c);
        acc[mb][nb] = c;
    };
#define ISWM_SB() __builtin_amdgcn_sched_barrier(0)
    for (int s2 = 0; s2 < nK; ++s2) {
        __builtin_amdgcn_s_barrier();
        asm volatile("" ::: "memory");
        const int slot = s2 & 3;
        ldA(slot, 0); ldB(slot, 0);
        ISWM_SB(); ldB(slot, 1); ISWM_SB(); mm(0, 0); ISWM_SB();
        ISWM_SB(); ldB(slot, 2); ISWM_SB(); mm(0, 1); ISWM_SB();
        ISWM_SB(); ldB(slot, 3); ISWM_SB(); mm(0, 2); ISWM_SB();
        ISWM_SB(); ldA(slot, 1); ISWM_SB(); mm(0, 3); ISWM_SB();
        ISWM_SB(); mm(1, 3); ISWM_SB();
        ISWM_SB(); mm(1, 2); ISWM_SB();
        ISWM_SB(); mm(1, 1); ISWM_SB();
        ISWM_SB(); mm(1, 0); ISWM_SB();
    }
#undef ISWM_SB

    if (a.nsplit > 1) {
        float4* slab = reinterpret_cast<float4*>(a.out) + ((size_t)split * tiles + (mt * a.NT + nt)) * 8192 + lane;
#pragma unroll
        for (int mb = 0; mb < 2; ++mb)
#pragma unroll
            for (int nb = 0; nb < NBW; ++nb) {
                const int w8 = wm * 4 + wn4 + (nb >> 1);
#pragma unroll
                for (int q = 0; q < 4; ++q)
                    slab[(size_t)w8 * 1024 + ((mb * 2 + (nb & 1)) * 4 + q) * 64] =
                        make_float4(acc[mb][nb][4 * q], acc[mb][nb][4 * q + 1], acc[mb][nb][4 * q + 2], acc[mb][nb][4 * q + 3]);
            }
        return;
    }
    float* out = a.out;
    const int li = lane & 31, lh = lane >> 5;
#pragma unroll
    for (int nb = 0; nb < NBW; ++nb) {
        const int col = n0 + wn4 * 64 + nb * 32 + li;
        const bool cok = col < a.Ktot;
#pragma unroll
        for (int mb = 0; mb < 2; ++mb)
#pragma unroll
            for (int r = 0; r < 16; ++r) {
                const int row = m0 + wm * 64 + mb * 32 + (r & 3) + 8 * (r >> 2) + 4 * lh;
                if (cok && row < a.Cout) out[(size_t)row * a.Ktot + col] = acc[mb][nb][r];
            }
    }
}

__global__ __launch_bounds__(256) void k_reduce_slabs_frag(const float4* __restrict__ slabs, float* __restrict__ dw, int tiles,
                                                           int NT, int nsplit, int Cout, int Ktot) {
    const int64_t total = (int64_t)tiles * 8192;
    for (int64_t i = blockIdx.x * (int64_t)blockDim.x + threadIdx.x; i < total; i += (int64_t)gridDim.x * blockDim.x) {
        float4 s = slabs[i];
        int k = 1;
        for (; k + 3 < nsplit; k += 4) {
            const float4 v0 = slabs[i + (int64_t)k * total], v1 = slabs[i + (int64_t)(k + 1) * total];
            const float4 v2 = slabs[i + (int64_t)(k + 2) * total], v3 = slabs[i + (int64_t)(k + 3) * total];
            s.x += v0.x; s.y += v0.y; s.z += v0.z; s.w += v0.w;
            s.x += v1.x; s.y += v1.y; s.z += v1.z; s.w += v1.w;
            s.x += v2.x; s.y += v2.y; s.z += v2.z; s.w += v2.w;
            s.x += v3.x; s.y += v3.y; s.z += v3.z; s.w += v3.w;
        }
        for (; k < nsplit; ++k) {
            const float4 v = slabs[i + (int64_t)k * total];
            s.x += v.x; s.y += v.y; s.z += v.z; s.w += v.w;
        }
        const int tile = (int)(i >> 13), f = (int)(i & 8191);
        const int wave = f >> 10, j = (f >> 6) & 15, lane = f & 63;
        const int mt = tile / NT, nt = tile - mt * NT;
        const int wm = wave >> 2, wn = wave & 3, mb = j >> 3, nb = (j >> 2) & 1, q = j & 3;
        const int col = nt * 256 + wn * 64 + nb * 32 + (lane & 31);
        const int row = mt * 128 + wm * 64 + mb * 32 + 8 * q + 4 * (lane >> 5);
        if (col < Ktot) {
            float* o = dw + (size_t)row * Ktot + col;
            if (row < Cout) o[0] = s.x;
            if (row + 1 < Cout) o[(size_t)Ktot] = s.y;
            if (row + 2 < Cout) o[(size_t)2 * Ktot] = s.z;
            if (row + 3 < Cout) o[(size_t)3 * Ktot] = s.w;
        }
    }
}

static int wgrad_pl_wide(int Ktot, int taps, int64_t P) {
    if (Ktot <= 128) return 0;
    if (taps == 1 && P > 20000) return 0;
    const int pad256 = (Ktot + 255) / 256 * 256, pad128 = (Ktot + 127) / 128 * 128;
    return pad256 * 10 <= pad128 * 14;
}

int wgrad_pl_is_wide(const iswm_conv_desc* d) {
    return wgrad_pl_wide(d->KH * d->KW * d->Cin, d->KH * d->KW, (int64_t)d->N * d->Ho * d->Wo);
}

void plan_wgrad_pl(int Cout, int Ktot, int taps, int64_t P, int* nsplit, int* psplit) {
    const int wide = wgrad_pl_wide(Ktot, taps, P);
    const int tn = wide ? 256 : 128;
    const int64_t tiles = (int64_t)((Cout + 127) / 128) * ((Ktot + tn - 1) / tn);
    const double step_us = wide ? 1.45 : 0.75;
    const double slab_us = (double)Cout * Ktot * 8.0 / 4.0e6;
    int64_t maxs = (P + 255) / 256;
    if (maxs > 256) maxs = 256;
    double best = 1e300;
    *psplit = (int)((P + 31) / 32 * 32);
    *nsplit = 1;
    for (int64_t ns = 1; ns <= maxs; ++ns) {
        const int64_t ps = ((P + ns - 1) / ns + 31) / 32 * 32;
        const int64_t nsp = (P + ps - 1) / ps;
        const int64_t rounds = (tiles * nsp + 255) / 256;
        const double tm = (double)rounds * ((double)(ps / 32) + 6.0) * step_us + (nsp > 1 ? (double)nsp * slab_us + 5.0 : 0.0);
        if (tm < best) {
            best = tm;
            *psplit = (int)ps;
            *nsplit = (int)nsp;
        }
    }
}

void launch_wgrad_pl(const WgArgs& a, int planes, int wide, hipStream_t s) {
    dim3 grid(a.MT * a.NT * a.nsplit), blk(512);
    if (wide && !a.vote) {
        if (planes == 1) hipLaunchKernelGGL(k_wgrad_pls<1>, grid, blk, 0, s, a);
        else hipLaunchKernelGGL(k_wgrad_pls<3>, grid, blk, 0, s, a);
    } else if (wide) {
        if (planes == 1) hipLaunchKernelGGL(k_wgrad_plw<1>, grid, blk, 0, s, a);
        else hipLaunchKernelGGL(k_wgrad_plw<3>, grid, blk, 0, s, a);
    } else {
        if (planes == 1) hipLaunchKernelGGL(k_wgrad_pl<1>, grid, blk, 0, s, a);
        else hipLaunchKernelGGL(k_wgrad_pl<3>, grid, blk, 0, s, a);
    }
}

}

using namespace iswm;

namespace iswm {
void launch_reduce_slabs(const float* slabs, float* dst, int64_t n4, int nsplit, hipStream_t s);
}

static const char* wg_refusal(const iswm_conv_desc* d) {
    if (d == nullptr) return "wgrad_planes: null descriptor";
    if (!(d->N > 0 && d->H > 0 && d->W > 0 && d->Cin > 0 && d->Cout > 0)) return "wgrad_planes: empty tensor";
    if (!(d->Cin % 8 == 0 && d->Cout % 8 == 0 && d->ldx % 8 == 0 && d->ldy % 8 == 0 && d->ldx >= d->Cin && d->ldy >= d->Cout))
        return "wgrad_planes: channel counts and pitches must be multiples of 8";
    if (!(d->KH > 0 && d->KW > 0 && d->stride > 0 && d->dil > 0 && d->pad >= 0)) return "wgrad_planes: bad geometry";
    const int ho = (d->H + 2 * d->pad - d->dil * (d->KH - 1) - 1) / d->stride + 1;
    const int wo = (d->W + 2 * d->pad - d->dil * (d->KW - 1) - 1) / d->stride + 1;
    if (!(ho == d->Ho && wo == d->Wo)) return "wgrad_planes: output size does not match geometry";
    if (!((int64_t)d->N * d->H * d->W * d->ldx < (1ll << 30) && (int64_t)d->N * d->Ho * d->Wo * d->ldy < (1ll << 30)))
        return "wgrad_planes: tensor too large (2^30 elements per operand)";
    return nullptr;
}

static int wg_validate(const iswm_conv_desc* d) {
    const char* why = wg_refusal(d);
    ISWM_REQUIRE(why == nullptr, "%s (Cin %d Cout %d ldx %d ldy %d)", why, d ? d->Cin : 0, d ? d->Cout : 0, d ? d->ldx : 0,
                 d ? d->ldy : 0);
    return 0;
}

extern "C" int iswm_conv2d_wgrad_planes_ok(const iswm_conv_desc* d) {
    return (wg_refusal(d) == nullptr && iswm_get_conv_math() >= 1) ? 1 : 0;
}

static bool wgrad_rect_mode(const iswm_conv_desc* d, int64_t* p_eff, unsigned char* order, bool* similar = nullptr) {
    const int taps = d->KH * d->KW;
    if (d->pad < 4 || d->stride != 1 || d->Cin % 256 != 0 || taps <= 1 || taps > 32 || iswm_get_conv_math() != 1) return false;
    int64_t area[32], sum = 0;
    for (int t = 0; t < taps; ++t) {
        const int dh = (t / d->KW) * d->dil - d->pad, dw = (t % d->KW) * d->dil - d->pad;
        const int h = std::max(0, std::min(d->Ho, d->H - dh) - std::max(0, -dh));
        const int w = std::max(0, std::min(d->Wo, d->W - dw) - std::max(0, -dw));
        area[t] = (int64_t)d->N * h * w;
        sum += area[t];
    }
    if (order) {
        for (int t = 0; t < taps; ++t) order[t] = (unsigned char)t;
        for (int i = 0; i < taps; ++i)
            for (int j = i + 1; j < taps; ++j)
                if (area[order[j]] > area[order[i]]) std::swap(order[i], order[j]);
    }
    if (p_eff) *p_eff = std::max<int64_t>(32, sum / taps);
    if (similar) {
        int64_t lo = area[0], hi = area[0];
        for (int t = 1; t < taps; ++t) {
            lo = std::min(lo, area[t]);
            hi = std::max(hi, area[t]);
        }
        *similar = 100 * lo >= 35 * hi;
    }
    return true;
}

namespace iswm {
int wgrad_pl_kernel_kind(const iswm_conv_desc* d) {
    if (!wgrad_pl_is_wide(d)) return 0;
    const bool rect = wgrad_rect_mode(d, nullptr, nullptr);
    const bool vote = d->pad >= 4 && !rect;
    return vote ? 1 : 2;
}
}

extern "C" size_t iswm_conv2d_wgrad_planes_workspace(const iswm_conv_desc* d) {
    if (!d) return 0;
    int ns, ps;
    const int Ktot = d->KH * d->KW * d->Cin;
    int64_t P = (int64_t)d->N * d->Ho * d->Wo;
    wgrad_rect_mode(d, &P, nullptr);
    plan_wgrad_pl(d->Cout, Ktot, d->KH * d->KW, P, &ns, &ps);
    if (ns <= 1) return 0;
    if (wgrad_pl_wide(Ktot, d->KH * d->KW, (int64_t)d->N * d->Ho * d->Wo))
        return (size_t)ns * ((d->Cout + 127) / 128) * ((Ktot + 255) / 256) * 32768 * sizeof(float);
    return (size_t)ns * d->Cout * Ktot * sizeof(float);
}

extern "C" int iswm_conv2d_wgrad_planes(const iswm_conv_desc* d, const void* xp, int64_t x_ps, const void* dyp, int64_t dy_ps,
                                        float* dw, float* workspace, size_t workspace_bytes, iswm_stream_t stream) {
    if (int e = wg_validate(d)) return e;
    ISWM_REQUIRE(xp && dyp && dw && aligned16(xp) && aligned16(dyp) && aligned16(dw), "wgrad_planes: bad pointer");
    const int planes = iswm_get_conv_math() == 2 ? 1 : 3;
    ISWM_REQUIRE(planes == 1 || (x_ps % 8 == 0 && dy_ps % 8 == 0 && x_ps > 0 && dy_ps > 0), "wgrad_planes: bad plane stride");
    WgArgs a{};
    a.dy = (const unsigned short*)dyp; a.x = (const unsigned short*)xp;
    a.dyps = dy_ps * 2; a.xps = x_ps * 2;
    a.N = d->N; a.H = d->H; a.W = d->W; a.Cin = d->Cin; a.Ho = d->Ho; a.Wo = d->Wo; a.Cout = d->Cout;
    a.KH = d->KH; a.KW = d->KW; a.stride = d->stride; a.pad = d->pad; a.dil = d->dil; a.ldx = d->ldx; a.ldy = d->ldy;
    a.P = d->N * d->Ho * d->Wo;
    a.Ktot = d->KH * d->KW * d->Cin;
    a.MT = (d->Cout + 127) / 128;
    const int wide = wgrad_pl_wide(a.Ktot, d->KH * d->KW, a.P);
    a.NT = wide ? (a.Ktot + 255) / 256 : (a.Ktot + 127) / 128;
    int64_t p_plan = a.P;
    bool similar = false;
    a.rect = (wide && wgrad_rect_mode(d, &p_plan, a.tap_order, &similar)) ? 1 : 0;
    {
        if (a.rect && (d->Cin >> 8) == 8 && similar) a.rect = 2;
    }
    plan_wgrad_pl(d->Cout, a.Ktot, d->KH * d->KW, p_plan, &a.nsplit, &a.psplit);
    a.vote = (d->pad >= 4 && !a.rect) ? 1 : 0;
    a.always = (d->KH == 1 && d->KW == 1 && d->pad == 0 && d->stride == 1) ? 1 : 0;
    const size_t need = iswm_conv2d_wgrad_planes_workspace(d);
    ISWM_REQUIRE(workspace_bytes >= need && (need == 0 || (workspace && aligned16(workspace))),
                 "wgrad_planes: workspace too small (%zu < %zu)", workspace_bytes, need);
    a.out = a.nsplit > 1 ? workspace : dw;
    launch_wgrad_pl(a, planes, wide, (hipStream_t)stream);
    if (int e = check_launch("wgrad_planes")) return e;
    if (a.nsplit > 1) {
        if (wide) {
            const int tiles = a.MT * a.NT;
            hipLaunchKernelGGL(k_reduce_slabs_frag, dim3(stream_grid((int64_t)tiles * 8192, 256)), dim3(256), 0,
                               (hipStream_t)stream, reinterpret_cast<const float4*>(workspace), dw, tiles, a.NT, a.nsplit,
                               d->Cout, a.Ktot);
        } else {
            launch_reduce_slabs(workspace, dw, (int64_t)d->Cout * a.Ktot / 4, a.nsplit, (hipStream_t)stream);
        }
        return check_launch("wgrad_planes_reduce");
    }
    return 0;
}
```

### iswm_amd/network/_hip.py

```python

import torch
import torch.nn as nn

from .. import ops


MASK_RECORDER = None
POOL_RECORDER = None
CALIB_RECORDER = None


def pad4(c):
    return (c + 3) // 4 * 4


def pad_cin(c):
    if c % 32 == 0 or c < 128:
        return pad4(c)
    return (c + 31) // 32 * 32


def dense_flat(t):
    if t.dim() == 4 and not t.is_contiguous():
        v = t.permute(0, 2, 3, 1)
        assert v.is_contiguous(), "parameter is neither contiguous nor channels_last"
        return v.reshape(-1)
    assert t.is_contiguous()
    return t.reshape(-1)


class GradSink:

    def __init__(self, on_ready=None):
        self.on_ready = on_ready
        self._pending = {}

    def target(self, p):
        if p.grad is None:
            view = getattr(p, "_iswm_grad_view", None)
            p.grad = view if view is not None else torch.empty_like(p)
            return p.grad
        tmp = torch.empty_like(p)
        self._pending[id(p)] = tmp
        return tmp

    def done(self, p):
        tmp = self._pending.pop(id(p), None)
        if tmp is not None:
            ops.add_inplace(dense_flat(p.grad), dense_flat(tmp))
        if self.on_ready is not None:
            self.on_ready(p)


class HipModule(nn.Module):

    def fwd(self, x, save):
        raise NotImplementedError

    def bwd(self, dy, sink):
        raise NotImplementedError

    def out_channels_of(self, cin):
        return None

    def forward(self, x):
        return run_module(self, x)


class _Bridge(torch.autograd.Function):

    @staticmethod
    def forward(ctx, mod, cout, x, *params):
        xh = ops.nchw_to_nhwc(x)
        yh = mod.fwd(xh, True)
        ctx.mod, ctx.cin, ctx.need_dx = mod, x.shape[1], x.requires_grad
        return ops.nhwc_to_nchw(yh, cout or yh.shape[3])

    @staticmethod
    def backward(ctx, dy):
        mod = ctx.mod
        dyh = ops.nchw_to_nhwc(dy.contiguous())
        sink = GradSink(getattr(mod, "_iswm_on_ready", None))
        dxh = mod.bwd(dyh, sink)
        dx = ops.nhwc_to_nchw(dxh, ctx.cin) if (ctx.need_dx and dxh is not None) else None
        return (None, None, dx) + (None,) * (len(ctx.needs_input_grad) - 3)


def run_module(mod, x):
    if not (torch.is_tensor(x) and x.is_cuda and x.dtype == torch.float32 and x.dim() == 4):
        raise ValueError("iswm_amd modules take a 4-D fp32 CUDA NCHW tensor (no CPU fallback); got %s" %
                         (x.shape if torch.is_tensor(x) else type(x),))
    params = [p for p in mod.parameters() if p.requires_grad]
    cout = mod.out_channels_of(x.shape[1])
    if torch.is_grad_enabled() and (x.requires_grad or params):
        return _Bridge.apply(mod, cout, x, *params)
    yh = mod.fwd(ops.nchw_to_nhwc(x), False)
    return ops.nhwc_to_nchw(yh, cout or yh.shape[3])


class Conv2d(HipModule, nn.Conv2d):

    def __init__(self, *args, **kwargs):
        nn.Conv2d.__init__(self, *args, **kwargs)
        if self.groups != 1 or self.padding_mode != "zeros":
            raise NotImplementedError("HIP conv supports groups=1, zero padding")
        if self.kernel_size[0] != self.kernel_size[1] or self.dilation[0] != self.dilation[1] or \
                self.stride[0] != self.stride[1] or self.padding[0] != self.padding[1]:
            raise NotImplementedError("HIP conv supports square kernels/strides/dilations")
        with torch.no_grad():
            self.weight.data = self.weight.data.contiguous(memory_format=torch.channels_last)
        self._saved = None

    @property
    def cin_p(self):
        return pad_cin(self.in_channels)

    @property
    def cout_p(self):
        return pad4(self.out_channels)

    def needs_pack(self):
        return self.cin_p != self.in_channels or self.cout_p != self.out_channels

    def ohwi(self):
        w = self.weight
        v = w.permute(0, 2, 3, 1)
        if not self.needs_pack():
            return v if v.is_contiguous() else v.contiguous()
        return ops.pad_weights(w, self.cout_p, self.cin_p)

    def packed2(self, kind):
        e = getattr(self, "_iswm_wpk", None)
        if e is None or not e["live"] or e["epoch"] != ops.WEIGHTS_EPOCH or e["version"] != self.weight._version or \
                e["ptr"] != self.weight.data_ptr():
            return None
        return e["buf"].get(kind + 2)

    def packed(self, kind):
        e = getattr(self, "_iswm_wpk", None)
        if e is None or not e["live"] or e["epoch"] != ops.WEIGHTS_EPOCH or e["version"] != self.weight._version or \
                e["ptr"] != self.weight.data_ptr():
            return None
        return e["buf"][kind]

    def bias_p(self):
        if self.bias is None:
            return None
        if self.cout_p == self.out_channels:
            return self.bias
        return ops.pad_weights(self.bias.view(-1, 1, 1, 1), self.cout_p, 1).view(-1)

    def geometry(self, x):
        if x.shape[3] != self.cin_p:
            raise ValueError("conv expects %d (padded) input channels, got %d" % (self.cin_p, x.shape[3]))
        g = ops.ConvGeom(x, self.cout_p, self.kernel_size[0], self.kernel_size[1], self.stride[0],
                         self.padding[0], self.dilation[0])
        g.alg_cin, g.alg_cout = self.in_channels, self.out_channels
        return g

    def write_wgrad(self, x, dy, g, sink):
        p = self.weight
        if not p.requires_grad:
            return
        buf = sink.target(p)
        v = buf.permute(0, 2, 3, 1)
        if not self.needs_pack() and v.is_contiguous():
            ops.conv2d_wgrad(x, dy, g, v)
        else:
            ops.unpad_weights(ops.conv2d_wgrad(x, dy, g), buf)
        sink.done(p)

    def fwd(self, x, save, out=None):
        g = self.geometry(x)
        y, _, _ = ops.conv2d_fwd(x, self.ohwi(), g, bias=self.bias_p(), out=out, wpk=self.packed(0), wpk2=self.packed2(0))
        self._saved = (x, g) if save else None
        return y

    def bwd(self, dy, sink, need_dx=True, dx=None, accumulate=False):
        x, g = self._saved
        self._saved = None
        if self.bias is not None and self.bias.requires_grad:
            ops.unpad_weights(ops.colsum(dy).view(-1, 1, 1, 1), sink.target(self.bias).view(-1, 1, 1, 1))
            sink.done(self.bias)
        self.write_wgrad(x, dy, g, sink)
        if not need_dx:
            return None
        return ops.conv2d_dgrad(dy, self.ohwi(), g, tuple(x.shape), dx, accumulate, wpk=self.packed(1), wpk2=self.packed2(1))

    def out_channels_of(self, cin):
        return self.out_channels


class DepthwiseConv2d(HipModule, nn.Conv2d):

    def __init__(self, *args, **kwargs):
        nn.Conv2d.__init__(self, *args, **kwargs)
        if self.groups != self.in_channels or self.out_channels != self.in_channels or self.padding_mode != "zeros":
            raise NotImplementedError("HIP depthwise conv needs groups == in_channels == out_channels, zero padding")
        if self.kernel_size[0] != self.kernel_size[1] or self.dilation[0] != self.dilation[1] or \
                self.stride[0] != self.stride[1] or self.padding[0] != self.padding[1]:
            raise NotImplementedError("HIP depthwise conv supports square kernels/strides/dilations")
        self._saved = None

    def geometry(self, x):
        c = x.shape[3]
        if c < self.in_channels or c % 4 != 0:
            raise ValueError("depthwise conv over %d channels got a %d-channel buffer" % (self.in_channels, c))
        return ops.ConvGeom(x, c, self.kernel_size[0], self.kernel_size[1], self.stride[0], self.padding[0],
                            self.dilation[0])

    def fwd(self, x, save, out=None):
        g = self.geometry(x)
        y = ops.dwconv2d_fwd(x, self.weight.contiguous(), g, self.bias, out)
        self._saved = (x, g) if save else None
        return y

    def is_dw3x3(self):
        return (self.kernel_size[0] == 3 and self.stride[0] in (1, 2) and self.padding[0] == self.dilation[0] and
                self.bias is None)

    def fwd_stats(self, x, save, want_stats):
        g = self.geometry(x)
        y, partials, tiles = ops.dwconv3x3_fwd_stats(x, self.weight.contiguous(), g, want_stats)
        self._saved = (x, g) if save else None
        return y, partials, tiles

    def bwd_fused(self, dy, sink, need_dx=True, dx=None, accumulate=False):
        x, g = self._saved
        self._saved = None
        need_dw, buf, tgt = self.weight.requires_grad, None, None
        if need_dw:
            buf = sink.target(self.weight)
            tgt = buf if buf.is_contiguous() else None
        if not (need_dx or need_dw):
            return None
        dx, dw = ops.dwconv3x3_bwd(x, dy, self.weight.contiguous(), g, self.in_channels, dx, accumulate, tgt, need_dx, need_dw)
        if need_dw:
            if tgt is None:
                buf.copy_(dw)
            sink.done(self.weight)
        return dx

    def bwd(self, dy, sink, need_dx=True, dx=None, accumulate=False):
        x, g = self._saved
        self._saved = None
        if self.bias is not None and self.bias.requires_grad:
            ops.unpad_weights(ops.colsum(dy).view(-1, 1, 1, 1), sink.target(self.bias).view(-1, 1, 1, 1))
            sink.done(self.bias)
        if self.weight.requires_grad:
            buf = sink.target(self.weight)
            if buf.is_contiguous():
                ops.dwconv2d_wgrad(x, dy, g, self.in_channels, buf)
            else:
                buf.copy_(ops.dwconv2d_wgrad(x, dy, g, self.in_channels))
            sink.done(self.weight)
        if not need_dx:
            return None
        return ops.dwconv2d_dgrad(dy, self.weight.contiguous(), g, tuple(x.shape), dx, accumulate)

    def out_channels_of(self, cin):
        return self.out_channels


class BatchNorm2d(nn.BatchNorm2d):
    pass


class ReLU(nn.ReLU):
    pass


class ReLU6(nn.ReLU6):
    pass


class Dropout(HipModule, nn.Dropout):

    def __init__(self, *a, **k):
        nn.Dropout.__init__(self, *a, **k)
        self._calls = 0
        self._mask = None

    def fwd(self, x, save):
        if not self.training or self.p == 0.0:
            self._mask = None
            return x
        self._calls += 1
        y, mask = ops.dropout_fwd(x, self.p, torch.initial_seed() & 0x7FFFFFFFFFFFFFFF, self._calls)
        self._mask = mask if save else None
        return y

    def bwd(self, dy, sink):
        if self._mask is None:
            return dy
        dx = ops.dropout_bwd(dy.contiguous(), self._mask, self.p)
        self._mask = None
        return dx


def cba_fwd(conv, bn, relu, x, save, residual=None, out=None, out_fmt=None):
    sep = None
    if isinstance(conv, SeparableBase):
        sep, conv = conv, conv.body[1]
        x = sep.body[0].fwd(x, save)
    training = bn.training
    if bn.momentum is None or not bn.track_running_stats or not bn.affine:
        raise NotImplementedError("HIP BatchNorm2d supports affine=True, momentum!=None, running stats")
    if isinstance(conv, DepthwiseConv2d):
        g = conv.geometry(x)
        if conv.is_dw3x3():
            y, partials, tiles = conv.fwd_stats(x, save, training)
            return _cba_finish(conv, bn, relu, x, y, g, partials, tiles, training, save, residual, out, sep, True, out_fmt)
        y = conv.fwd(x, save)
        partials, tiles = None, (0, 0)
        if training:
            partials, nt, tr = ops.colstat(y)
            tiles = (nt, tr)
        return _cba_finish(conv, bn, relu, x, y, g, partials, tiles, training, save, residual, out, sep, True, out_fmt)
    g = conv.geometry(x)
    if conv.bias is None:
        y, partials, tiles = ops.conv2d_fwd(x, conv.ohwi(), g, want_stats=training, wpk=conv.packed(0), wpk2=conv.packed2(0))
    else:
        y, _, _ = ops.conv2d_fwd(x, conv.ohwi(), g, bias=conv.bias_p())
        partials, tiles = None, (0, 0)
        if training:
            partials, nt, tr = ops.colstat(y)
            tiles = (nt, tr)
    return _cba_finish(conv, bn, relu, x, y, g, partials, tiles, training, save, residual, out, sep, False, out_fmt)


def _cba_finish(conv, bn, relu, x, y, g, partials, tiles, training, save, residual, out, sep, dw, out_fmt=None):
    if training:
        count = y.shape[0] * y.shape[1] * y.shape[2]
        if count <= 1:
            raise ValueError("Expected more than 1 value per channel when training, got input size %s" %
                             (tuple(y.shape),))
        coef = ops.bn_finalize(partials, tiles[0], count, tiles[1], bn.weight, bn.bias, bn.running_mean, bn.running_var,
                               bn.momentum, bn.eps)
        if not getattr(bn, "_iswm_nbt_fused", False):
            bn.num_batches_tracked.add_(1)
    else:
        coef = ops.bn_eval_coeffs(bn.weight, bn.bias, bn.running_mean, bn.running_var, bn.eps)
    if out_fmt is None:
        want_planes = ops.planes_on() and y.shape[3] % 64 == 0
    else:
        want_planes = out_fmt == "planes" and ops.planes_on() and y.shape[3] % 64 == 0
    o = ops.bn_apply(y, coef, relu, residual, out, planes=want_planes)
    if MASK_RECORDER is not None and relu:
        of = ops.as_f32(o)
        MASK_RECORDER[bn] = (of > 0) & (of < 6) if relu == 6 and relu is not True else (of > 0)
    if CALIB_RECORDER is not None:
        CALIB_RECORDER.record(conv, o)
    ctx = None
    if save:
        ctx = dict(x=x, y=y, out=o, coef=coef, g=g, relu=relu, training=training, res=residual is not None, sep=sep, dw=dw)
    return o, ctx


_BN3_FUSE = True


def _bn_stats_request(up):
    if up is None or not ops.planes_on() or up.get("bn_stats") is not None:
        return None
    if ops._relu_code(up["relu"]) not in (0, 1):
        return None
    if up.get("res"):
        if not (_BN3_FUSE and ops._relu_code(up["relu"]) == 1 and ops.is_planes(up["out"]) and up["training"]):
            return None
        return ops.BnStats(up["y"], up["coef"], up["relu"], mask=up["out"])
    return ops.BnStats(up["y"], up["coef"], up["relu"])


def cba_bwd_bn(conv, bn, ctx, dout, sink, dy_out=None, need_dx=True):
    y, o = ctx["y"], ctx["out"]
    sep = ctx.get("sep")
    if sep is not None:
        conv = sep.body[1]
    gw, gb = bn.weight, bn.bias
    dgamma = sink.target(gw) if gw.requires_grad else torch.empty_like(gw)
    dbeta = sink.target(gb) if gb.requires_grad else torch.empty_like(gb)
    dyp = (not ctx.get("dw")) and ops.planes_conv_ok(conv.cin_p, conv.cout_p, 1) and (need_dx or ops.is_planes(ctx["x"]))
    st = ctx.pop("bn_stats", None)
    if st is not None and st.partials is not None and st.masked:
        dout = ops.as_f32(dout)
        dy, _ = ops.bn_backward(dout, None, y, ctx["coef"], gw, False, ctx["training"], dgamma, dbeta, want_dres=False,
                                dy=dy_out, dy_planes=dyp, stats=st)
        dres = dout if ctx["res"] else None
    else:
        dy, dres = ops.bn_backward(ops.as_f32(dout), o if ctx["relu"] else None, y, ctx["coef"], gw, ctx["relu"], ctx["training"],
                                   dgamma, dbeta, want_dres=ctx["res"], dy=dy_out, dy_planes=dyp, stats=st)
    if gw.requires_grad:
        sink.done(gw)
    if gb.requires_grad:
        sink.done(gb)
    return dy, dres


def cba_bwd(conv, bn, ctx, dout, sink, need_dx=True, dx=None, accumulate=False, up=None):
    x, g = ctx["x"], ctx["g"]
    sep = ctx.get("sep")
    dy, dres = cba_bwd_bn(conv, bn, ctx, dout, sink, need_dx=need_dx or sep is not None)
    if sep is not None:
        conv = sep.body[1]
    if ctx.get("dw"):
        if conv.is_dw3x3():
            return conv.bwd_fused(dy, sink, need_dx, dx, accumulate), dres
        return conv.bwd(dy, sink, need_dx, dx, accumulate), dres
    conv.write_wgrad(x, dy, g, sink)
    if conv.bias is not None and conv.bias.requires_grad:
        ops.unpad_weights(ops.colsum(dy).view(-1, 1, 1, 1), sink.target(conv.bias).view(-1, 1, 1, 1))
        sink.done(conv.bias)
    if sep is not None:
        dmid = ops.conv2d_dgrad(dy, conv.ohwi(), g, tuple(x.shape), wpk=conv.packed(1), wpk2=conv.packed2(1))
        return sep.body[0].bwd(dmid, sink, need_dx, dx, accumulate), dres
    if need_dx:
        req = _bn_stats_request(up) if (up is not None and tuple(up["y"].shape) == tuple(x.shape)) else None
        dx = ops.conv2d_dgrad(dy, conv.ohwi(), g, tuple(x.shape), dx, accumulate, wpk=conv.packed(1), wpk2=conv.packed2(1),
                              bn_stats=req)
        if req is not None and req.partials is not None:
            up["bn_stats"] = req
    else:
        dx = None
    return dx, dres


def fuse_batch_counters(root):
    bns = [m for m in root.modules() if isinstance(m, nn.BatchNorm2d) and m.num_batches_tracked is not None]
    if not bns:
        return None
    flat = torch.stack([m.num_batches_tracked.detach().reshape(()) for m in bns]).contiguous()
    for i, m in enumerate(bns):
        m._buffers["num_batches_tracked"] = flat[i]
        m._iswm_nbt_fused = True
    return flat


class WeightPacker(object):

    def __init__(self, root):
        self.convs = [m for m in root.modules() if isinstance(m, Conv2d) and not m.needs_pack()]
        self.key, self.jobs, self.njobs, self.blocks, self.entries = None, None, 0, 0, []

    def _build(self, dev):
        import ctypes
        from .. import _lib
        lib = _lib.load()
        jobs, entries, first = [], [], 0
        keep = []
        for m in self.convs:
            w = m.weight
            v = w.permute(0, 2, 3, 1)
            if not (w.is_cuda and v.is_contiguous()):
                continue
            taps = m.kernel_size[0] * m.kernel_size[1]
            bufs = {}
            kinds = []
            for kind in (0, 1):
                if ops.planes_on() and lib.iswm_packed_weight_bytes(m.out_channels, taps, m.in_channels, kind + 2):
                    kinds.append(kind + 2)
                else:
                    kinds.append(kind)
            for kind in kinds:
                nb = lib.iswm_packed_weight_bytes(m.out_channels, taps, m.in_channels, kind)
                if nb == 0:
                    continue
                buf = torch.empty((nb // 4,), dtype=torch.float32, device=dev)
                bufs[kind] = buf
                jobs.append((w.data_ptr(), buf.data_ptr(), m.out_channels, taps, m.in_channels, kind, first, 0))
                first += lib.iswm_pack_job_blocks(m.out_channels, taps, m.in_channels, kind)
            if bufs:
                e = dict(live=False, epoch=-1, version=-1, ptr=w.data_ptr(), buf={k: bufs.get(k) for k in range(4)})
                m._iswm_wpk = e
                entries.append((m, e))
                keep.append(bufs)

        class _Job(ctypes.Structure):
            _fields_ = [("w", ctypes.c_void_p), ("packed", ctypes.c_void_p), ("Cout", ctypes.c_int), ("taps", ctypes.c_int),
                        ("Cin", ctypes.c_int), ("kind", ctypes.c_int), ("first_block", ctypes.c_int),
                        ("reserved", ctypes.c_int)]
        arr = (_Job * max(1, len(jobs)))()
        for i, j in enumerate(jobs):
            arr[i] = _Job(*j)
        self.jobs = torch.frombuffer(bytearray(bytes(arr)), dtype=torch.uint8).to(dev) if jobs else None
        self.njobs, self.blocks, self.entries = len(jobs), first, entries

    def begin(self):
        from .. import _lib
        math = _lib.load().iswm_get_conv_math()
        if math < 1 or not ops._USE_PACKED or not self.convs:
            return
        key = (math, ops.planes_on()) + tuple(m.weight.data_ptr() for m in self.convs)
        if key != self.key:
            self._build(self.convs[0].weight.device)
            self.key = key
        if self.njobs == 0:
            return
        ops.call("iswm_pack_weights_batch", ops._p(self.jobs), self.njobs, self.blocks, ops._stream())
        for m, e in self.entries:
            e["live"], e["epoch"], e["version"] = True, ops.WEIGHTS_EPOCH, m.weight._version

    def end(self):
        for _, e in self.entries:
            e["live"] = False


_CLS_FUSE = True


def cls_fusable(conv, bn, relu, cls):
    return (_CLS_FUSE and CALIB_RECORDER is None and relu is True and type(conv) is Conv2d and conv.out_channels == 256 and
            conv.bias is None and type(cls) is Conv2d and cls.in_channels == 256 and cls.out_channels <= 4 and
            tuple(cls.kernel_size) == (1, 1) and tuple(cls.stride) == (1, 1) and tuple(cls.padding) == (0, 0) and
            bn.momentum is not None and bn.track_running_stats and bn.affine)


def cba_cls_fwd(conv, bn, cls, x, save):
    g = conv.geometry(x)
    training = bn.training
    y, partials, tiles = ops.conv2d_fwd(x, conv.ohwi(), g, want_stats=training, wpk=conv.packed(0), wpk2=conv.packed2(0))
    if training:
        count = y.shape[0] * y.shape[1] * y.shape[2]
        if count <= 1:
            raise ValueError("Expected more than 1 value per channel when training, got input size %s" % (tuple(y.shape),))
        coef = ops.bn_finalize(partials, tiles[0], count, tiles[1], bn.weight, bn.bias, bn.running_mean, bn.running_var,
                               bn.momentum, bn.eps)
        if not getattr(bn, "_iswm_nbt_fused", False):
            bn.num_batches_tracked.add_(1)
    else:
        coef = ops.bn_eval_coeffs(bn.weight, bn.bias, bn.running_mean, bn.running_var, bn.eps)
    wc4 = ops.pad_weights(cls.weight, 4, 256).view(4, 256)
    b4 = None if cls.bias is None else ops.pad_weights(cls.bias.view(-1, 1, 1, 1), 4, 1).view(-1)
    logits = ops.bn_apply_classify(y, coef, wc4, b4)
    if MASK_RECORDER is not None:
        MASK_RECORDER[bn] = ops.bn_apply(y, coef, True) > 0
    ctx = dict(x=x, y=y, coef=coef, g=g, training=training, wc4=wc4, cls=cls, cls_fused=True) if save else None
    return logits, ctx


def cba_cls_bwd(conv, bn, ctx, dlogit, sink, need_dx=True, dx=None, accumulate=False):
    cls, x, y, g = ctx["cls"], ctx["x"], ctx["y"], ctx["g"]
    dlogit = ops.as_f32(dlogit)
    if cls.bias is not None and cls.bias.requires_grad:
        ops.unpad_weights(ops.colsum(dlogit).view(-1, 1, 1, 1), sink.target(cls.bias).view(-1, 1, 1, 1))
        sink.done(cls.bias)
    gw, gb = bn.weight, bn.bias
    dgamma = sink.target(gw) if gw.requires_grad else torch.empty_like(gw)
    dbeta = sink.target(gb) if gb.requires_grad else torch.empty_like(gb)
    dyp = ops.planes_conv_ok(conv.cin_p, conv.cout_p, 1)
    dy, dwc4 = ops.bn_backward_classify(dlogit, ctx["wc4"], y, ctx["coef"], gw, ctx["training"], dgamma, dbeta, dyp)
    if gw.requires_grad:
        sink.done(gw)
    if gb.requires_grad:
        sink.done(gb)
    if cls.weight.requires_grad:
        ops.unpad_weights(dwc4.view(4, 1, 1, 256), sink.target(cls.weight))
        sink.done(cls.weight)
    conv.write_wgrad(x, dy, g, sink)
    if not need_dx:
        return None
    return ops.conv2d_dgrad(dy, conv.ohwi(), g, tuple(x.shape), dx, accumulate, wpk=conv.packed(1), wpk2=conv.packed2(1))


class SeparableBase(HipModule):
    pass


class HipSequential(HipModule, nn.Sequential):

    def _stages(self):
        mods = list(self.children())
        st, i = [], 0
        while i < len(mods):
            m = mods[i]
            if isinstance(m, (Conv2d, SeparableBase, DepthwiseConv2d)) and i + 1 < len(mods) and \
                    isinstance(mods[i + 1], nn.BatchNorm2d):
                act = mods[i + 2] if i + 2 < len(mods) else None
                relu = 6 if isinstance(act, nn.ReLU6) else isinstance(act, nn.ReLU)
                st.append(("cba", m, mods[i + 1], relu))
                i += 3 if relu else 2
            elif isinstance(m, Conv2d):
                if i + 1 < len(mods) and isinstance(mods[i + 1], nn.BatchNorm2d):
                    relu = i + 2 < len(mods) and isinstance(mods[i + 2], nn.ReLU)
                    st.append(("cba", m, mods[i + 1], relu))
                    i += 3 if relu else 2
                else:
                    st.append(("conv", m))
                    i += 1
            elif isinstance(m, HipModule):
                st.append(("mod", m))
                i += 1
            else:
                raise NotImplementedError("no HIP implementation for %s inside a Sequential" % type(m).__name__)
        return st

    def fwd(self, x, save, out=None, out_fmt=None):
        st = self._stages()
        ctxs = []
        for k, s in enumerate(st):
            last = k == len(st) - 1
            if ctxs and ctxs[-1] == "FOLDED" and last:
                break
            if (s[0] == "cba" and k == len(st) - 2 and st[k + 1][0] == "conv" and out is None and
                    cls_fusable(s[1], s[2], s[3], st[k + 1][1])):
                x, c = cba_cls_fwd(s[1], s[2], st[k + 1][1], x, save)
                ctxs.append(c)
                ctxs.append("FOLDED")
                continue
            if s[0] == "cba":
                if last:
                    fmt = out_fmt if out is None else None
                    if out is None and out_fmt is None:
                        fmt = "f32"
                else:
                    fmt = "planes" if st[k + 1][0] in ("cba", "conv") else "f32"
                x, c = cba_fwd(s[1], s[2], s[3], x, save, out=out if last else None, out_fmt=fmt)
                ctxs.append(c)
            elif s[0] == "conv":
                x = s[1].fwd(x, save, out=out if last else None)
                ctxs.append(None)
            else:
                x = s[1].fwd(x, save)
                ctxs.append(None)
        self._saved = (st, ctxs) if save else None
        return x

    def bwd(self, dy, sink, need_dx=True, dx=None, accumulate=False):
        st, ctxs = self._saved
        self._saved = None
        for k in range(len(st) - 1, -1, -1):
            s = st[k]
            first = k == 0
            if ctxs[k] == "FOLDED":
                continue
            if s[0] == "cba" and ctxs[k] is not None and ctxs[k].get("cls_fused"):
                dy = cba_cls_bwd(s[1], s[2], ctxs[k], dy, sink, need_dx or not first, dx if first else None, accumulate and first)
                continue
            if s[0] == "cba":
                dy, _ = cba_bwd(s[1], s[2], ctxs[k], dy, sink, need_dx or not first, dx if first else None,
                                accumulate and first)
            elif s[0] == "conv":
                dy = s[1].bwd(dy, sink, need_dx or not first, dx if first else None, accumulate and first)
            else:
                dy = s[1].bwd(dy, sink)
        return dy

    def out_channels_of(self, cin):
        c = None
        for m in self.modules():
            if isinstance(m, nn.Conv2d):
                c = m.out_channels
        return c
```

### iswm_amd/network/backbone/resnet.py

```python
import torch
import torch.nn as nn

from .. import _hip
from ..._hip_compat import FloatFunctional
from ... import ops

__all__ = ['ResNet', 'resnet50', 'resnet101', 'resnet152']


def conv3x3(in_planes, out_planes, stride=1, groups=1, dilation=1):
    return _hip.Conv2d(in_planes, out_planes, kernel_size=3, stride=stride, padding=dilation, groups=groups,
                       bias=False, dilation=dilation)


def conv1x1(in_planes, out_planes, stride=1):
    return _hip.Conv2d(in_planes, out_planes, kernel_size=1, stride=stride, bias=False)


class Bottleneck(_hip.HipModule):
    expansion = 4

    def __init__(self, inplanes, planes, stride=1, downsample=None, groups=1, base_width=64, dilation=1,
                 norm_layer=None):
        super(Bottleneck, self).__init__()
        if norm_layer is None:
            norm_layer = _hip.BatchNorm2d
        width = int(planes * (base_width / 64.)) * groups
        self.conv1 = conv1x1(inplanes, width)
        self.bn1 = norm_layer(width)
        self.conv2 = conv3x3(width, width, stride, groups, dilation)
        self.bn2 = norm_layer(width)
        self.conv3 = conv1x1(width, planes * self.expansion)
        self.bn3 = norm_layer(planes * self.expansion)
        self.relu = _hip.ReLU(inplace=True)
        self.downsample = downsample
        self.stride = stride
        self.add = FloatFunctional()
        self._saved = None

    def fwd(self, x, save):
        o1, c1 = _hip.cba_fwd(self.conv1, self.bn1, True, x, save)
        o2, c2 = _hip.cba_fwd(self.conv2, self.bn2, True, o1, save)
        identity, cd = x, None
        if self.downsample is not None:
            identity, cd = _hip.cba_fwd(self.downsample[0], self.downsample[1], False, x, save)
        out, c3 = _hip.cba_fwd(self.conv3, self.bn3, True, o2, save, residual=identity)
        self._saved = (c1, c2, c3, cd) if save else None
        return out

    def bwd(self, dout, sink, need_dx=True, up=None, dx0=None):
        c1, c2, c3, cd = self._saved
        self._saved = None
        d2, dres = _hip.cba_bwd(self.conv3, self.bn3, c3, dout, sink, up=c2)
        d1, _ = _hip.cba_bwd(self.conv2, self.bn2, c2, d2, sink, up=c1)
        if cd is not None:
            dx, _ = _hip.cba_bwd(self.conv1, self.bn1, c1, d1, sink, dx=dx0, accumulate=dx0 is not None)
            dx, _ = _hip.cba_bwd(self.downsample[0], self.downsample[1], cd, dres, sink, dx=dx, accumulate=True)
        else:
            dx, _ = _hip.cba_bwd(self.conv1, self.bn1, c1, d1, sink, dx=dres, accumulate=True, up=up)
            if dx0 is not None:
                dx = ops.add_inplace(dx, dx0)
        return dx

    def out_channels_of(self, cin):
        return self.conv3.out_channels


class _Layer(_hip.HipModule, nn.Sequential):
    accepts_dx0 = True

    def fwd(self, x, save):
        for m in self:
            x = m.fwd(x, save)
        return x

    def bwd(self, dy, sink, dx0=None):
        blocks = list(self)
        for i in range(len(blocks) - 1, -1, -1):
            up = None
            if i > 0 and blocks[i].downsample is None and blocks[i - 1]._saved is not None:
                up = blocks[i - 1]._saved[2]
            dy = blocks[i].bwd(dy, sink, up=up, dx0=dx0 if i == 0 else None)
        return dy

    def out_channels_of(self, cin):
        return list(self)[-1].conv3.out_channels


class MaxPool2d(_hip.HipModule, nn.MaxPool2d):

    def fwd(self, x, save):
        if (self.kernel_size, self.stride, self.padding) != (3, 2, 1):
            raise NotImplementedError("HIP max-pool is the stem's 3x3 / stride 2 / pad 1")
        y, idx = ops.maxpool_fwd(x, planes=ops.planes_on() and x.shape[3] % 64 == 0)
        if _hip.POOL_RECORDER is not None:
            _hip.POOL_RECORDER[self] = idx
        if _hip.CALIB_RECORDER is not None:
            _hip.CALIB_RECORDER.record(self, y)
        self._saved = (idx, tuple(x.shape)) if save else None
        return y

    def bwd(self, dy, sink):
        idx, shape = self._saved
        self._saved = None
        return ops.maxpool_bwd(dy, idx, shape)


class ResNet(_hip.HipModule):

    def __init__(self, block, layers, num_classes=1000, zero_init_residual=False, groups=1, width_per_group=64,
                 replace_stride_with_dilation=None, norm_layer=None):
        super(ResNet, self).__init__()
        if norm_layer is None:
            norm_layer = _hip.BatchNorm2d
        self._norm_layer = norm_layer
        if groups != 1 or width_per_group != 64:
            raise NotImplementedError("HIP backbone covers the groups=1 / width 64 family (resnet50/101/152)")
        self.inplanes = 64
        self.dilation = 1
        if replace_stride_with_dilation is None:
            replace_stride_with_dilation = [False, False, False]
        if len(replace_stride_with_dilation) != 3:
            raise ValueError("replace_stride_with_dilation should be None "
                             "or a 3-element tuple, got {}".format(replace_stride_with_dilation))
        self.groups = groups
        self.base_width = width_per_group
        self.conv1 = _hip.Conv2d(3, self.inplanes, kernel_size=7, stride=2, padding=3, bias=False)
        self.bn1 = norm_layer(self.inplanes)
        self.relu = _hip.ReLU(inplace=True)
        self.maxpool = MaxPool2d(kernel_size=3, stride=2, padding=1)
        self.layer1 = self._make_layer(block, 64, layers[0])
        self.layer2 = self._make_layer(block, 128, layers[1], stride=2, dilate=replace_stride_with_dilation[0])
        self.layer3 = self._make_layer(block, 256, layers[2], stride=2, dilate=replace_stride_with_dilation[1])
        self.layer4 = self._make_layer(block, 512, layers[3], stride=2, dilate=replace_stride_with_dilation[2])
        self.avgpool = nn.AdaptiveAvgPool2d((1, 1))
        self.fc = nn.Linear(512 * block.expansion, num_classes)

        for m in self.modules():
            if isinstance(m, nn.Conv2d):
                nn.init.kaiming_normal_(m.weight, mode='fan_out', nonlinearity='relu')
            elif isinstance(m, (nn.BatchNorm2d, nn.GroupNorm)):
                nn.init.constant_(m.weight, 1)
                nn.init.constant_(m.bias, 0)
        if zero_init_residual:
            for m in self.modules():
                if isinstance(m, Bottleneck):
                    nn.init.constant_(m.bn3.weight, 0)

    def _make_layer(self, block, planes, blocks, stride=1, dilate=False):
        norm_layer = self._norm_layer
        downsample = None
        previous_dilation = self.dilation
        if dilate:
            self.dilation *= stride
            stride = 1
        if stride != 1 or self.inplanes != planes * block.expansion:
            downsample = nn.Sequential(
                conv1x1(self.inplanes, planes * block.expansion, stride),
                norm_layer(planes * block.expansion),
            )
        layers = [block(self.inplanes, planes, stride, downsample, self.groups, self.base_width,
                        previous_dilation, norm_layer)]
        self.inplanes = planes * block.expansion
        for _ in range(1, blocks):
            layers.append(block(self.inplanes, planes, groups=self.groups, base_width=self.base_width,
                                dilation=self.dilation, norm_layer=norm_layer))
        return _Layer(*layers)

    def forward(self, x):
        raise NotImplementedError("the ImageNet classification head (avgpool+fc) is not on the segmentation hot "
                                  "path; wrap the backbone in network.utils.IntermediateLayerGetter")


def _resnet(arch, block, layers, pretrained, progress, **kwargs):
    model = ResNet(block, layers, **kwargs)
    if pretrained:
        raise RuntimeError("pretrained=True needs a download; load a checkpoint with load_state_dict instead")
    return model


def resnet50(pretrained=False, progress=True, **kwargs):
    return _resnet('resnet50', Bottleneck, [3, 4, 6, 3], pretrained, progress, **kwargs)


def resnet101(pretrained=False, progress=True, **kwargs):
    return _resnet('resnet101', Bottleneck, [3, 4, 23, 3], pretrained, progress, **kwargs)


def resnet152(pretrained=False, progress=True, **kwargs):
    return _resnet('resnet152', Bottleneck, [3, 8, 36, 3], pretrained, progress, **kwargs)
```

### iswm_amd/ops.py

```python
import ctypes
import functools

import torch

from . import _lib
from ._lib import ConvDesc, call

BN_EPS = 1e-5


def _stream():
    return ctypes.c_void_p(torch.cuda.current_stream().cuda_stream)


def _p(t):
    return ctypes.c_void_p(t.data_ptr()) if t is not None else None


def geom(t, dtype=torch.float32):
    if isinstance(t, Planes):
        raise ValueError("this operation takes an fp32 NHWC tensor, not Planes (use .f32())")
    if t.dim() != 4 or t.dtype != dtype or not t.is_cuda:
        raise ValueError("expected a 4-D fp32 CUDA NHWC tensor, got %s %s %s" % (tuple(t.shape), t.dtype, t.device))
    n, h, w, c = t.shape
# ... 137 lines not shown
    def begin(self):
        return True

    def end(self, name, start, flops, tag=None):
        raise NotImplementedError

    def wants(self, name):
        return self.only is None or name == self.only or name + "+reduce" == self.only

    def add(self, name, a, b, flops, tag):
        self.records.append((name, a, b, flops, tag, self.scope))

    def scope_total(self, scope):
        d = dict(launches=0, ms=0.0, flops=0.0)
        for name, a, b, fl, _, sc in self.records:
            if sc == scope:
                d["launches"] += 1
                d["ms"] += a.elapsed_time(b)
                d["flops"] += fl
        return d

    def summary(self):
        out = {}
        for name, a, b, fl, _, _sc in self.records:
            d = out.setdefault(name, dict(launches=0, ms=0.0, flops=0.0))
            d["launches"] += 1
            d["ms"] += a.elapsed_time(b)
            d["flops"] += fl
        return out

    def by_geometry(self):
        out = {}
        for name, a, b, fl, tag, _sc in self.records:
            d = out.setdefault((name, tag), dict(launches=0, ms=0.0, flops=0.0))
            d["launches"] += 1
            d["ms"] += a.elapsed_time(b)
            d["flops"] += fl
        return out


KPROF = None


def _valid_taps(h, ho, k, stride, pad, dil):
    n = 0
    for t in range(k):
        off = t * dil - pad
        o_min = 0 if off >= 0 else (-off + stride - 1) // stride
        o_max = min(ho - 1, (h - 1 - off) // stride) if h - 1 - off >= 0 else -1
        n += max(0, o_max - o_min + 1)
    return n


def conv_out_size(h, k, stride, pad, dil):
    return (h + 2 * pad - dil * (k - 1) - 1) // stride + 1


class ConvGeom:

    def __init__(self, x, cout, kh, kw, stride, pad, dil):
        n, h, w, cin = x.shape
        self.n, self.h, self.w, self.cin, self.cout = n, h, w, cin, cout
        self.kh, self.kw, self.stride, self.pad, self.dil = kh, kw, stride, pad, dil
        self.ho = conv_out_size(h, kh, stride, pad, dil)
        self.wo = conv_out_size(w, kw, stride, pad, dil)
        self.alg_cin, self.alg_cout = cin, cout
        self._flops = None

    def tag(self):
        return "n%d %dx%d c%d->%d k%d s%d d%d" % (self.n, self.h, self.w, self.alg_cin, self.alg_cout, self.kh,
                                                  self.stride, self.dil)

    def flops(self):
        if self._flops is None:
            vh = _valid_taps(self.h, self.ho, self.kh, self.stride, self.pad, self.dil)
            vw = _valid_taps(self.w, self.wo, self.kw, self.stride, self.pad, self.dil)
            self._flops = 2.0 * self.n * vh * vw * self.alg_cin * self.alg_cout
        return self._flops

    def desc(self, ldx, ldy):
        return ConvDesc(self.n, self.h, self.w, self.cin, self.ho, self.wo, self.cout, self.kh, self.kw,
                        self.stride, self.pad, self.dil, ldx, ldy)


_NAME_CACHE = {}


def _kernel_name(d, kind):
    lib = _lib.load()
    key = (kind, lib.iswm_get_conv_math(), d.N, d.H, d.W, d.Cin, d.Cout, d.KH, d.stride, d.pad, d.dil)
    name = _NAME_CACHE.get(key)
    if name is None:
        buf = ctypes.create_string_buffer(64)
        lib.iswm_conv2d_kernel_name(ctypes.byref(d), kind, buf, 64)
        name = _NAME_CACHE[key] = buf.value.decode()
    return name


class _timed:

    def __init__(self, d, kind, g, suffix=""):
        self.on = False
        if KPROF is not None:
            name = _kernel_name(d, kind) + suffix
            if KPROF.wants(name):
                self.on, self.name, self.g = True, name, g

    def __enter__(self):
        if self.on:
            self.a = torch.cuda.Event(enable_timing=True)
            self.a.record()

    def __exit__(self, *exc):
        if self.on:
            b = torch.cuda.Event(enable_timing=True)
            b.record()
            KPROF.add(self.name, self.a, b, self.g.flops(), self.g.tag())
        return False


def _check_w(w_ohwi, g):
    if tuple(w_ohwi.shape) != (g.cout, g.kh, g.kw, g.cin) or not w_ohwi.is_contiguous():
        raise ValueError("weight must be contiguous OHWI %s, got %s strides %s" %
                         ((g.cout, g.kh, g.kw, g.cin), tuple(w_ohwi.shape), w_ohwi.stride()))


WEIGHTS_EPOCH = 0


def weights_changed():
    global WEIGHTS_EPOCH
    WEIGHTS_EPOCH += 1


def conv2d_fwd(x, w_ohwi, g, bias=None, out=None, want_stats=False, wpk=None, wpk2=None):
    _check_w(w_ohwi, g)
    if out is None:
        out = new_act(g.n, g.ho, g.wo, g.cout, x.device)
    on, oh, ow, oc, ldy = geom(out)
    assert (on, oh, ow, oc) == (g.n, g.ho, g.wo, g.cout)
    if isinstance(x, Planes):
        _, _, _, _, ldp, ps = pgeom(x)
        d = g.desc(ldp, ldy)
        nb2 = _pl2_bytes(d, 0)
        if nb2:
            partials, tiles = None, (0, 0)
            if want_stats:
                tr = _lib.load().iswm_conv2d_pl2_tile_rows(ctypes.byref(d), 0)
                tiles = ((g.n * g.ho * g.wo + tr - 1) // tr, tr)
                partials = torch.empty((2, tiles[0], g.cout), dtype=torch.float32, device=out.device)
            if wpk2 is None:
                wpk2 = torch.empty((nb2 // 4,), dtype=torch.float32, device=out.device)
                call("iswm_conv2d_pl2_pack_weights", ctypes.byref(d), 0, _p(w_ohwi), _p(wpk2), _stream())
            with _timed(d, 5, g):
                call("iswm_conv2d_fwd_pl2", ctypes.byref(d), _p(x.t), ps, _p(wpk2), _p(bias), _p(out), _p(partials), _stream())
            return out, partials, tiles
        x = x.f32()
    ldx = geom(x)[4]
    d = g.desc(ldx, ldy)
    partials, tiles = None, (0, 0)
    if want_stats:
        lib = _lib.load()
        tiles = (lib.iswm_conv2d_stat_tiles(ctypes.byref(d)), lib.iswm_conv2d_stat_tile_rows(ctypes.byref(d)))
        partials = torch.empty((2, tiles[0], g.cout), dtype=torch.float32, device=x.device)
    nb = _packed_bytes(d, 0)
    if nb:
        if want_stats:
            nt, tr = ctypes.c_int(0), ctypes.c_int(0)
            call("iswm_conv2d_fwd_packed_stat_layout", ctypes.byref(d), ctypes.byref(nt), ctypes.byref(tr))
            tiles = (nt.value, tr.value)
            flat = torch.empty((2 * nt.value * g.cout + nt.value,), dtype=torch.float32, device=x.device)
            partials = flat[:2 * nt.value * g.cout].view(2, nt.value, g.cout)
        if wpk is None:
            wpk = torch.empty((nb // 4,), dtype=torch.float32, device=x.device)
            call("iswm_conv2d_pack_weights", ctypes.byref(d), 0, _p(w_ohwi), _p(wpk), _stream())
        with _timed(d, 3, g):
            call("iswm_conv2d_fwd_packed", ctypes.byref(d), _p(x), _p(wpk), _p(bias), _p(out), _p(partials), _stream())
        return out, partials, tiles
    with _timed(d, 0, g):
        call("iswm_conv2d_fwd", ctypes.byref(d), _p(x), _p(w_ohwi), _p(bias), _p(out), _p(partials), _stream())
    return out, partials, tiles


_USE_PACKED = True


def _packed_bytes(d, kind):
    return _lib.load().iswm_conv2d_packed_weight_bytes(ctypes.byref(d), kind) if _USE_PACKED else 0


def _pl2_bytes(d, kind):
    return _lib.load().iswm_conv2d_pl2_weight_bytes(ctypes.byref(d), kind) if planes_on() else 0


def planes_conv_ok(cin, cout, kind):
    return planes_on() and (cout if kind else cin) % 64 == 0


class BnStats(object):

    def __init__(self, y, coef, relu, mask=None):
        self.y, self.coef, self.relu = y, coef, relu
        self.partials, self.tiles = None, 0
        self.mask, self.masked = mask, False


_BN_FUSE = True


def conv2d_dgrad(dy, w_ohwi, g, x_like_shape, dx=None, accumulate=False, wpk=None, wpk2=None, bn_stats=None):
    _check_w(w_ohwi, g)
    if dx is None:
        assert not accumulate
        dx = new_act(*x_like_shape, dy.device)
    ldx = geom(dx)[4]
    if isinstance(dy, Planes):
        _, _, _, _, ldp, ps = pgeom(dy)
        d = g.desc(ldx, ldp)
        nb2 = _pl2_bytes(d, 1)
        if nb2:
            if wpk2 is None:
                wpk2 = torch.empty((nb2 // 4,), dtype=torch.float32, device=dx.device)
                call("iswm_conv2d_pl2_pack_weights", ctypes.byref(d), 1, _p(w_ohwi), _p(wpk2), _stream())
            if bn_stats is not None and _BN_FUSE and g.cin % 4 == 0:
                b = bn_stats
                tiles = _lib.load().iswm_conv2d_dgrad_pl2_stat_tiles(ctypes.byref(d))
                part = torch.empty((2, tiles, g.cin), dtype=torch.float64, device=dx.device)
                masky = _relu_code(b.relu) == 1 and b.mask is None
                pm, ldm, code = None, 0, 2 if masky else 0
                if b.mask is not None:
                    pm, _, _, ldm, _ = xrows(b.mask)
                    code = 3
                with _timed(d, 6, g):
                    call("iswm_conv2d_dgrad_pl2_bn", ctypes.byref(d), _p(dy.t), ps, _p(wpk2), _p(dx), int(bool(accumulate)),
                         _p(b.y), rows(b.y)[2], _p(b.coef[2]), _p(b.coef[3]), _p(b.coef[0]) if masky else None,
                         _p(b.coef[1]) if masky else None, code, _p(pm), ldm, _p(part), tiles, _stream())
                b.partials, b.tiles, b.masked = part, tiles, b.mask is not None
                return dx
            with _timed(d, 6, g):
                call("iswm_conv2d_dgrad_pl2", ctypes.byref(d), _p(dy.t), ps, _p(wpk2), _p(dx), int(bool(accumulate)), _stream())
            return dx
        dy = dy.f32()
    ldy = geom(dy)[4]
    d = g.desc(ldx, ldy)
    nb = _packed_bytes(d, 1)
    if nb:
        if wpk is None:
            wpk = torch.empty((nb // 4,), dtype=torch.float32, device=dy.device)
            call("iswm_conv2d_pack_weights", ctypes.byref(d), 1, _p(w_ohwi), _p(wpk), _stream())
        with _timed(d, 4, g):
            call("iswm_conv2d_dgrad_packed", ctypes.byref(d), _p(dy), _p(wpk), _p(dx), int(bool(accumulate)), _stream())
        return dx
    if _lib.load().iswm_conv2d_dgrad_wants_wt(ctypes.byref(d)):
        wt = torch.empty((g.cin, g.kh, g.kw, g.cout), dtype=torch.float32, device=dy.device)
        call("iswm_transpose_weights", ctypes.byref(d), _p(w_ohwi), _p(wt), _stream())
        with _timed(d, 1, g):
            call("iswm_conv2d_dgrad_wt", ctypes.byref(d), _p(dy), _p(wt), _p(dx), int(bool(accumulate)), _stream())
        return dx
    with _timed(d, 1, g):
        call("iswm_conv2d_dgrad", ctypes.byref(d), _p(dy), _p(w_ohwi), _p(dx), int(bool(accumulate)), _stream())
    return dx


def _wgrad_planes_ok(x, dy, g, c8):
    ldx = pgeom(x)[4]
    ldy = pgeom(dy)[4] if (isinstance(dy, Planes) and c8 == g.cout) else c8
    d = ConvDesc(g.n, g.h, g.w, g.cin, g.ho, g.wo, c8, g.kh, g.kw, g.stride, g.pad, g.dil, ldx, ldy)
    return bool(_lib.load().iswm_conv2d_wgrad_planes_ok(ctypes.byref(d)))


def conv2d_wgrad(x, dy, g, dw_ohwi=None):
    if dw_ohwi is None:
        dw_ohwi = torch.empty((g.cout, g.kh, g.kw, g.cin), dtype=torch.float32, device=x.device)
    _check_w(dw_ohwi, g)
    c8 = (g.cout + 7) // 8 * 8
    if isinstance(x, Planes) and planes_on() and _wgrad_planes_ok(x, dy, g, c8):
        if not isinstance(dy, Planes) or c8 != g.cout:
            dyf = as_f32(dy)
            dy = new_planes(g.n, g.ho, g.wo, c8, x.device)
            if c8 != g.cout:
                zero_channels(dy, g.cout)
            split_planes(dyf, out=dy[..., :g.cout] if c8 != g.cout else dy)
        _, _, _, _, ldx, psx = pgeom(x)
        _, _, _, _, ldy, psy = pgeom(dy)
        d = ConvDesc(g.n, g.h, g.w, g.cin, g.ho, g.wo, c8, g.kh, g.kw, g.stride, g.pad, g.dil, ldx, ldy)
        need = _lib.load().iswm_conv2d_wgrad_planes_workspace(ctypes.byref(d))
        ws = torch.empty((need // 4,), dtype=torch.float32, device=x.device) if need else None
        tgt = dw_ohwi if c8 == g.cout else torch.empty((c8, g.kh, g.kw, g.cin), dtype=torch.float32, device=x.device)
        with _timed(d, 7, g, "+reduce"):
            call("iswm_conv2d_wgrad_planes", ctypes.byref(d), _p(x.t), psx, _p(dy.t), psy, _p(tgt), _p(ws), need, _stream())
        if tgt is not dw_ohwi:
            unpad_weights(tgt, dw_ohwi.permute(0, 3, 1, 2))
        return dw_ohwi
    x, dy = as_f32(x), as_f32(dy)
    ldx, ldy = geom(x)[4], geom(dy)[4]
    d = g.desc(ldx, ldy)
    need = _lib.load().iswm_conv2d_wgrad_workspace(ctypes.byref(d))
    ws = torch.empty((need // 4,), dtype=torch.float32, device=x.device) if need else None
    with _timed(d, 2, g, "+reduce"):
        call("iswm_conv2d_wgrad", ctypes.byref(d), _p(x), _p(dy), _p(dw_ohwi), _p(ws), need, _stream())
    return dw_ohwi


ASPP_TILE_ROWS = 144
_ASPP_PLANS = {}
_ASPP_FUSED = True


def _int_array(v):
    return (ctypes.c_int * len(v))(*[int(i) for i in v])


def _ptr_array(ts):
    return (ctypes.c_void_p * len(ts))(*[(t.data_ptr() if t is not None else None) for t in ts])


def aspp_desc(n, h, w, cin, cout, ldx, ldy):
    return ConvDesc(n, h, w, cin, h, w, cout, 1, 1, 1, 0, 1, ldx, ldy)


def aspp_plan(n, h, w, cin, cout, ksize, dil, kind, device):
    if not (_ASPP_FUSED and nplanes() == 3):
        return None
    key = (n, h, w, cin, cout, tuple(ksize), tuple(dil), kind, str(device))
    plan = _ASPP_PLANS.get(key)
    if plan is None:
        lib = _lib.load()
        d = aspp_desc(n, h, w, cin, cout, cin, cout)
        ks, dl = _int_array(ksize), _int_array(dil)
        nb = lib.iswm_aspp_plan_bytes(ctypes.byref(d), len(ksize), ks, dl, kind)
        if nb == 0:
            _ASPP_PLANS[key] = False
            return None
        host = torch.empty((nb,), dtype=torch.uint8)
        cus = torch.cuda.get_device_properties(device).multi_processor_count
        call("iswm_aspp_plan", ctypes.byref(d), len(ksize), ks, dl, kind, ctypes.c_void_p(host.data_ptr()), cus)
        plan = _ASPP_PLANS[key] = host.to(device)
    return None if plan is False else plan


def aspp_fwd(x, ksize, dil, cout, wpks, want_stats):
    _, n, h, w, cin, ldx, ps = xgeom(x)
    plan = aspp_plan(n, h, w, cin, cout, ksize, dil, 0, x.device)
    if plan is None:
        return None
    nb = len(ksize)
    tiles = (n * h * w + ASPP_TILE_ROWS - 1) // ASPP_TILE_ROWS
    ys = [new_act(n, h, w, cout, x.device) for _ in range(nb)]
    parts = [torch.empty((2, tiles, cout), dtype=torch.float32, device=x.device) for _ in range(nb)] if want_stats else None
    d = aspp_desc(n, h, w, cin, cout, ldx, cout)
    gs = [ConvGeom(x, cout, k, k, 1, dl * (k - 1) // 2, dl) for k, dl in zip(ksize, dil)]
    with _timed_multi("k_conv_pl2t<false>", gs):
        call("iswm_aspp_fwd", ctypes.byref(d), nb, _int_array(ksize), _int_array(dil), _p(plan), _p(x.t), ps, _ptr_array(wpks),
             _ptr_array(ys), _ptr_array(parts) if parts else None, _stream())
    return ys, parts, tiles


def aspp_dgrad(dyc, ksize, dil, cin, cout, wpks, dx=None, accumulate=False, x=None, dws=None):
    _, n, h, w, ctot, ld, ps = xgeom(dyc)
    nb = len(ksize)
    assert ctot >= nb * cout
    plan = aspp_plan(n, h, w, cin, cout, ksize, dil, 1, dyc.device)
    if plan is None:
        return None
    if dx is None:
        assert not accumulate
        dx = new_act(n, h, w, cin, dyc.device)
    d = aspp_desc(n, h, w, cin, cout, geom(dx)[4], cout)
    gs = []
    for k, dl in zip(ksize, dil):
        g = ConvGeom(dx, cout, k, k, 1, dl * (k - 1) // 2, dl)
        g.alg_cin, g.alg_cout = cin, cout
        gs.append(g)
    px, xps, pdw, ws, need = None, 0, None, None, 0
    if dws is not None:
        px, xps = x.t, pgeom(x)[5]
        pdw = _ptr_array(dws)
        lib = _lib.load()
        for k, dl in zip(ksize, dil):
            db = ConvDesc(n, h, w, cin, h, w, cout, k, k, 1, dl * (k - 1) // 2, dl, pgeom(x)[4], ld)
            need = max(need, lib.iswm_conv2d_wgrad_planes_workspace(ctypes.byref(db)))
        ws = torch.empty((max(need, 16) // 4,), dtype=torch.float32, device=dyc.device)
        d = aspp_desc(n, h, w, cin, cout, pgeom(x)[4], cout)
        assert geom(dx)[4] == pgeom(x)[4], "iswm_aspp_bwd takes ONE pitch for x and dx"
    with _timed_multi("k_conv_pl2t<true>", gs):
        call("iswm_aspp_bwd", ctypes.byref(d), nb, _int_array(ksize), _int_array(dil), _p(plan), _p(dyc.t), ps, ld, _ptr_array(wpks),
             _p(dx), int(bool(accumulate)), _p(px), xps, pdw, _p(ws), need, _stream())
    return dx


class _timed_multi:

    def __init__(self, name, geoms):
        self.on = KPROF is not None and KPROF.wants(name)
        self.name, self.geoms = name, geoms

    def __enter__(self):
        if self.on:
            self.a = torch.cuda.Event(enable_timing=True)
            self.a.record()

    def __exit__(self, *exc):
        if self.on:
            b = torch.cuda.Event(enable_timing=True)
            b.record()
            g0 = self.geoms[0]
            tag = "n%d %dx%d c%d->%dx%d aspp d%s" % (g0.n, g0.h, g0.w, g0.alg_cin, len(self.geoms), g0.alg_cout,
                                                    "/".join(str(g.dil) for g in self.geoms if g.kh > 1))
            KPROF.add(self.name, self.a, b, sum(g.flops() for g in self.geoms), tag)
        return False


def dwconv2d_fwd(x, w, g, bias=None, out=None):
    x = as_f32(x)
    ldx = geom(x)[4]
    if out is None:
        out = new_act(g.n, g.ho, g.wo, g.cin, x.device)
    d = g.desc(ldx, geom(out)[4])
    call("iswm_dwconv2d_fwd", ctypes.byref(d), _p(x), _p(w), w.shape[0], _p(bias), _p(out), _stream())
    return out


def dwconv2d_dgrad(dy, w, g, x_like_shape, dx=None, accumulate=False):
    if dx is None:
        assert not accumulate
        dx = new_act(*x_like_shape, dy.device)
    d = g.desc(geom(dx)[4], geom(dy)[4])
    call("iswm_dwconv2d_dgrad", ctypes.byref(d), _p(dy), _p(w), w.shape[0], _p(dx), int(bool(accumulate)), _stream())
    return dx


def dwconv2d_wgrad(x, dy, g, cw, dw=None):
    x, dy = as_f32(x), as_f32(dy)
    if dw is None:
        dw = torch.empty((cw, 1, g.kh, g.kw), dtype=torch.float32, device=x.device)
    d = g.desc(geom(x)[4], geom(dy)[4])
    need = _lib.load().iswm_dwconv2d_wgrad_workspace(ctypes.byref(d))
    ws = torch.empty((need // 8,), dtype=torch.float64, device=x.device)
    call("iswm_dwconv2d_wgrad", ctypes.byref(d), _p(x), _p(dy), cw, _p(dw), _p(ws), need, _stream())
    return dw


def dwconv3x3_fwd_stats(x, w, g, want_stats, out=None):
    x = as_f32(x)
    if out is None:
        out = new_act(g.n, g.ho, g.wo, g.cin, x.device)
    d = g.desc(geom(x)[4], geom(out)[4])
    partials, tiles = None, (0, 0)
    if want_stats:
        lib = _lib.load()
        tiles = (lib.iswm_dwconv3x3_stat_tiles(ctypes.byref(d)), lib.iswm_dwconv3x3_stat_tile_rows(ctypes.byref(d)))
        partials = torch.empty((2, tiles[0], g.cin), dtype=torch.float32, device=x.device)
    call("iswm_dwconv3x3_fwd_stats", ctypes.byref(d), _p(x), _p(w), w.shape[0], _p(out), _p(partials), _stream())
    return out, partials, tiles


def dwconv3x3_bwd(x, dy, w, g, cw, dx=None, accumulate=False, dw=None, need_dx=True, need_dw=True):
    x, dy = as_f32(x), as_f32(dy)
    if need_dx and dx is None:
        assert not accumulate
        dx = new_act(*x.shape, dy.device)
    if not need_dx:
        dx = None
    d = g.desc(geom(x)[4], geom(dy)[4])
    lddx = geom(dx)[4] if dx is not None else 0
    ws, need = None, 0
    if need_dw:
        if dw is None:
            dw = torch.empty((cw, 1, 3, 3), dtype=torch.float32, device=x.device)
        need = _lib.load().iswm_dwconv3x3_bwd_workspace(ctypes.byref(d))
        ws = torch.empty((need // 4,), dtype=torch.float32, device=x.device)
    else:
        dw = None
    call("iswm_dwconv3x3_bwd", ctypes.byref(d), _p(x), _p(dy), _p(w), cw, _p(dx), lddx, int(bool(accumulate)), _p(dw), _p(ws),
         need, _stream())
    return dx, dw


def rows(t):
    n, h, w, c, ld = geom(t)
    return n * h * w, c, ld


def xrows(t):
    p, n, h, w, c, ld, ps = xgeom(t)
    return p, n * h * w, c, ld, ps


def colstat(x):
    m, c, ld = rows(x)
    tile_rows = _lib.load().iswm_colstat_tile_rows(m)
    tiles = (m + tile_rows - 1) // tile_rows
    partials = torch.empty((2, tiles, c), dtype=torch.float32, device=x.device)
    call("iswm_colstat", _p(x), m, c, ld, _p(partials), _stream())
    return partials, tiles, tile_rows


def bn_finalize(partials, tiles, count, tile_rows, gamma, beta, running_mean, running_var, momentum, eps=BN_EPS):
    c = partials.shape[2]
    coef = torch.empty((4, c), dtype=torch.float32, device=partials.device)
    call("iswm_bn_finalize", _p(partials), tiles, c, count, tile_rows, _p(gamma), _p(beta), _p(running_mean),
         _p(running_var), float(momentum), float(eps), _p(coef[0]), _p(coef[1]), _p(coef[2]), _p(coef[3]), _stream())
    return coef


def bn_eval_coeffs(gamma, beta, running_mean, running_var, eps=BN_EPS):
    c = running_mean.numel()
    coef = torch.empty((4, c), dtype=torch.float32, device=running_mean.device)
    call("iswm_bn_eval_coeffs", c, _p(gamma), _p(beta), _p(running_mean), _p(running_var), float(eps), _p(coef[0]),
         _p(coef[1]), _p(coef[2]), _p(coef[3]), _stream())
    return coef


def _relu_code(relu):
    return 6 if (relu == 6 and relu is not True) else int(bool(relu))


def bn_apply(y, coef, relu, residual=None, out=None, planes=False):
    m, c, ldy = rows(y)
    if out is None:
        out = new_planes(*y.shape, y.device) if planes else torch.empty(y.shape, dtype=torch.float32, device=y.device)
    po, mo, co, ldo, pso = xrows(out)
    assert (mo, co) == (m, c)
    pr, ldr, psr = None, 0, 0
    if residual is not None:
        pr, mr, cr, ldr, psr = xrows(residual)
        assert (mr, cr) == (m, c)
    call("iswm_bn_apply_pl", _p(y), m, c, ldy, _p(coef[0]), _p(coef[1]), _p(coef[2]), _p(pr), ldr, psr, _relu_code(relu),
         _p(po), ldo, pso, _stream())
    return out


def bn_backward(dout, out, y, coef, gamma, relu, training, dgamma, dbeta, want_dres=False, dy=None, dy_planes=False,
                stats=None):
    m, c, ldy = rows(y)
    _, _, ldd = rows(dout)
    po, ldo, pso = None, 0, 0
    if out is not None:
        po, _, _, ldo, pso = xrows(out)
    need = _lib.load().iswm_bn_bwd_workspace(m, c)
    ws = torch.empty((need // 8,), dtype=torch.float64, device=y.device)
    if dy is None:
        dy = new_planes(*y.shape, y.device) if dy_planes else torch.empty(y.shape, dtype=torch.float32, device=y.device)
    pdy, _, _, lddy, psdy = xrows(dy)
    dres = torch.empty(y.shape, dtype=torch.float32, device=y.device) if want_dres else None
    masky = _relu_code(relu) == 1 and not want_dres
    if stats is not None and stats.partials is not None:
        call("iswm_bn_backward_stats_pl", _p(dout), ldd, _p(po), ldo, pso, _p(y), ldy, m, c, _p(coef[2]), _p(coef[3]), _p(gamma),
             _p(coef[0]) if masky else None, _p(coef[1]) if masky else None,
             _relu_code(relu), int(bool(training)), _p(dgamma), _p(dbeta), _p(pdy), lddy, psdy, _p(dres),
             rows(dres)[2] if dres is not None else 0, _p(stats.partials), stats.tiles, _p(ws), need, _stream())
        return dy, dres
    call("iswm_bn_backward_pl", _p(dout), ldd, _p(po), ldo, pso, _p(y), ldy, m, c, _p(coef[2]), _p(coef[3]), _p(gamma),
         _p(coef[0]) if masky else None, _p(coef[1]) if masky else None,
         _relu_code(relu), int(bool(training)), _p(dgamma), _p(dbeta), _p(pdy), lddy, psdy, _p(dres),
         rows(dres)[2] if dres is not None else 0, _p(ws), need, _stream())
    return dy, dres


def bn_apply_classify(y, coef, wc4, bias4):
    m, c, ldy = rows(y)
    out = torch.empty(tuple(y.shape[:3]) + (4,), dtype=torch.float32, device=y.device)
    call("iswm_bn_apply_classify", _p(y), m, c, ldy, _p(coef[0]), _p(coef[1]), _p(coef[2]), _p(wc4), _p(bias4), _p(out), 4, _stream())
    return out


def bn_backward_classify(dlogit, wc4, y, coef, gamma, training, dgamma, dbeta, dy_planes):
    m, c, ldy = rows(y)
    _, cl, ldl = rows(dlogit)
    assert cl == 4
    need = _lib.load().iswm_bn_classify_bwd_workspace(m, c)
    ws = torch.empty((need // 8,), dtype=torch.float64, device=y.device)
    dy = new_planes(*y.shape, y.device) if dy_planes else torch.empty(y.shape, dtype=torch.float32, device=y.device)
    pdy, _, _, lddy, psdy = xrows(dy)
    dwc4 = torch.empty((4, c), dtype=torch.float32, device=y.device)
    call("iswm_bn_backward_classify", _p(dlogit), ldl, _p(wc4), _p(y), ldy, m, c, _p(coef[2]), _p(coef[3]), _p(gamma), _p(coef[0]),
         _p(coef[1]), int(bool(training)), _p(dgamma), _p(dbeta), _p(dwc4), _p(pdy), lddy, psdy, _p(ws), need, _stream())
    return dy, dwc4


def colsum(x):
    x = as_f32(x)
    partials, tiles, _ = colstat(x)
    c = x.shape[3]
    out = torch.empty((2, c), dtype=torch.float32, device=x.device)
    call("iswm_colsum_finalize", _p(partials), tiles, c, _p(out[0]), _p(out[1]), _stream())
    return out[0]


def maxpool_fwd(x, planes=False):
    x = as_f32(x)
    n, h, w, c, ld = geom(x)
    assert ld == c
    ho, wo = (h + 2 - 3) // 2 + 1, (w + 2 - 3) // 2 + 1
    y = new_planes(n, ho, wo, c, x.device) if planes else new_act(n, ho, wo, c, x.device)
    py, _, _, _, _, _, ps = xgeom(y)
    idx = torch.empty((n, ho, wo, c), dtype=torch.uint8, device=x.device)
    call("iswm_maxpool3x3s2_fwd_pl", _p(x), n, h, w, c, _p(py), ps, _p(idx), ho, wo, _stream())
    return y, idx


def maxpool_bwd(dy, idx, in_shape):
    n, h, w, c = in_shape
    _, ho, wo, _, ld = geom(dy)
    assert ld == c
    dx = new_act(n, h, w, c, dy.device)
    call("iswm_maxpool3x3s2_bwd", _p(dy), _p(idx), n, h, w, c, ho, wo, _p(dx), _stream())
    return dx


def gap_fwd(x):
    px, n, h, w, c, ld, ps = xgeom(x)
    y = new_act(n, 1, 1, c, x.device)
    call("iswm_gap_fwd_pl", _p(px), ps, n, h * w, c, ld, _p(y), _stream())
    return y


def gap_bwd(dy, dx, accumulate):
    n, h, w, c, ld = geom(dx)
    call("iswm_gap_bwd", _p(dy), n, h * w, c, _p(dx), ld, int(bool(accumulate)), _stream())
    return dx


def bcast_fwd(v, out):
    po, n, h, w, c, ld, ps = xgeom(out)
    call("iswm_bcast_fwd_pl", _p(as_f32(v)), n, h * w, c, _p(po), ld, ps, _stream())
    return out


def bcast_bwd(dy):
    n, h, w, c, ld = geom(dy)
    dv = new_act(n, 1, 1, c, dy.device)
    call("iswm_bcast_bwd", _p(dy), ld, n, h * w, c, _p(dv), _stream())
    return dv


def bilinear_fwd(x, ho, wo, out=None):
    x = as_f32(x)
    n, hi, wi, c, ldx = geom(x)
    if out is None:
        out = new_act(n, ho, wo, c, x.device)
    po, _, _, _, _, ldy, ps = xgeom(out)
    call("iswm_bilinear_fwd_pl", _p(x), n, hi, wi, c, ldx, _p(po), ps, ho, wo, ldy, _stream())
    return out


def bilinear_bwd(dy, hi, wi):
    n, ho, wo, c, lddy = geom(dy)
    dx = new_act(n, hi, wi, c, dy.device)
    call("iswm_bilinear_bwd", _p(dy), n, hi, wi, c, lddy, ho, wo, _p(dx), c, _stream())
    return dx


def bilinear_to_nchw_fwd(x, c, ho, wo):
    x = as_f32(x)
    n, hi, wi, cp, ldx = geom(x)
    y = torch.empty((n, c, ho, wo), dtype=torch.float32, device=x.device)
    call("iswm_bilinear_nhwc_to_nchw_fwd", _p(x), n, hi, wi, c, ldx, _p(y), ho, wo, _stream())
    return y


def bilinear_to_nchw_bwd(dy, hi, wi, cp):
    n, c, ho, wo = dy.shape
    assert dy.is_contiguous() and dy.dtype == torch.float32
    dx = new_act(n, hi, wi, cp, dy.device)
    call("iswm_bilinear_nhwc_to_nchw_bwd", _p(dy), n, hi, wi, c, cp, ho, wo, _p(dx), _stream())
    return dx


def nchw_to_nhwc(x, cp=None):
    assert x.dim() == 4 and x.dtype == torch.float32 and x.is_cuda
    x = x.contiguous()
    n, c, h, w = x.shape
    cp = cp or (c + 3) // 4 * 4
    y = new_act(n, h, w, cp, x.device)
    call("iswm_nchw_to_nhwc", _p(x), n, c, h * w, _p(y), cp, _stream())
    return y


def nhwc_to_nchw(x, c=None):
    x = as_f32(x)
    n, h, w, cc, ld = geom(x)
    c = c or cc
    y = torch.empty((n, c, h, w), dtype=torch.float32, device=x.device)
    call("iswm_nhwc_to_nchw", _p(x), n, c, h * w, ld, _p(y), _stream())
    return y


def copy_channels(src, dst):
    src = as_f32(src)
    m, c, lds = rows(src)
    md, cd, ldd = rows(dst)
    assert (m, c) == (md, cd)
    call("iswm_copy_channels", _p(src), lds, _p(dst), ldd, m, c, _stream())
    return dst


def add_inplace(dst, src):
    assert dst.is_contiguous() and src.is_contiguous() and dst.numel() == src.numel()
    call("iswm_add_inplace", _p(dst), _p(src), dst.numel(), _stream())
    return dst


def dropout_fwd(x, p, seed, offset):
    x = as_f32(x)
    assert x.is_contiguous()
    y = torch.empty_like(x)
    mask = torch.empty(x.shape, dtype=torch.uint8, device=x.device)
    call("iswm_dropout_fwd", _p(x), _p(y), _p(mask), x.numel(), float(p), int(seed), int(offset), _stream())
    return y, mask

# ... 319 lines not shown
```

Measured before the change: 277.3 images/sec.

## Group bottleneck wgrad convolutions into a single multi-member planes launch

Weight-gradient work for the convs of each ResNet bottleneck block is deferred and issued as one grouped k_wgrad_plsg launch, with a joint split-K planner and one shared slab-reduce kernel, instead of one launch per conv. The goal is to fill the GPU better on small wgrad GEMMs and to cut launch and tail overhead. A cost model decides per group whether grouping is worth it. In exchange, weight gradients finish later in the backward pass, and the kernel pays for per-block member indexing and argument reloads.

Result: no change. 276.8 images/sec (-0.2%).

```diff
diff --git a/include/iswm_hip.h b/include/iswm_hip.h
--- a/include/iswm_hip.h
+++ b/include/iswm_hip.h
@@ -98,6 +98,13 @@
 size_t iswm_conv2d_wgrad_planes_workspace(const iswm_conv_desc* d);
 int iswm_conv2d_wgrad_planes(const iswm_conv_desc* d, const void* xp, int64_t x_ps, const void* dyp, int64_t dy_ps, float* dw,
                              float* workspace, size_t workspace_bytes, iswm_stream_t stream);
+int iswm_conv2d_wgrad_planes_group_ok(const iswm_conv_desc* d);
+int iswm_conv2d_wgrad_planes_group_pays(int n, const iswm_conv_desc* d);
+size_t iswm_conv2d_wgrad_planes_group_workspace(int n, const iswm_conv_desc* d);
+int iswm_conv2d_wgrad_planes_group_plan(int n, const iswm_conv_desc* d, int* nsplit);
+int iswm_conv2d_wgrad_planes_group(int n, const iswm_conv_desc* d, const void* const* xp, const int64_t* x_ps,
+                                   const void* const* dyp, const int64_t* dy_ps, float* const* dw, float* workspace,
+                                   size_t workspace_bytes, iswm_stream_t stream);
 int iswm_dwconv2d_fwd(const iswm_conv_desc* d, const float* x, const float* w, int Cw, const float* bias, float* y,
                       iswm_stream_t stream);
 int iswm_dwconv2d_dgrad(const iswm_conv_desc* d, const float* dy, const float* w, int Cw, float* dx, int accumulate,
diff --git a/iswm_amd/_lib.py b/iswm_amd/_lib.py
--- a/iswm_amd/_lib.py
+++ b/iswm_amd/_lib.py
@@ -66,6 +66,12 @@
     "iswm_conv2d_wgrad_planes_ok": (c_int, [POINTER(ConvDesc)]),
     "iswm_conv2d_wgrad_planes_workspace": (c_size_t, [POINTER(ConvDesc)]),
     "iswm_conv2d_wgrad_planes": (c_int, [POINTER(ConvDesc), P, c_int64, P, c_int64, P, P, c_size_t, P]),
+    "iswm_conv2d_wgrad_planes_group_ok": (c_int, [POINTER(ConvDesc)]),
+    "iswm_conv2d_wgrad_planes_group_pays": (c_int, [c_int, POINTER(ConvDesc)]),
+    "iswm_conv2d_wgrad_planes_group_workspace": (c_size_t, [c_int, POINTER(ConvDesc)]),
+    "iswm_conv2d_wgrad_planes_group_plan": (c_int, [c_int, POINTER(ConvDesc), POINTER(c_int)]),
+    "iswm_conv2d_wgrad_planes_group": (c_int, [c_int, POINTER(ConvDesc), POINTER(c_void_p), POINTER(c_int64), POINTER(c_void_p),
+                                               POINTER(c_int64), POINTER(c_void_p), P, c_size_t, P]),
     "iswm_conv2d_wgrad_workspace": (c_size_t, [POINTER(ConvDesc)]),
     "iswm_dwconv2d_fwd": (c_int, [POINTER(ConvDesc), P, P, c_int, P, P, P]),
     "iswm_dwconv2d_dgrad": (c_int, [POINTER(ConvDesc), P, P, c_int, P, c_int, P]),
diff --git a/iswm_amd/csrc/conv_mfma.hip b/iswm_amd/csrc/conv_mfma.hip
--- a/iswm_amd/csrc/conv_mfma.hip
+++ b/iswm_amd/csrc/conv_mfma.hip
@@ -761,7 +761,11 @@
 static int pl2_K(const iswm_conv_desc* d, bool dgrad) { return d->KH * d->KW * (dgrad ? d->Cout : d->Cin); }
 
 extern "C" int iswm_conv2d_kernel_name(const iswm_conv_desc* d, int kind, char* buf, int buflen) {
-    ISWM_REQUIRE(d && buf && buflen > 0 && kind >= 0 && kind <= 7, "kernel_name: bad argument");
+    ISWM_REQUIRE(d && buf && buflen > 0 && kind >= 0 && kind <= 8, "kernel_name: bad argument");
+    if (kind == 8) {
+        snprintf(buf, buflen, "k_wgrad_plsg<%d>", math_planes());
+        return 0;
+    }
     if (kind == 7) {
         const int kk = wgrad_pl_kernel_kind(d);
         snprintf(buf, buflen, kk == 2 ? "k_wgrad_pls<%d>" : kk == 1 ? "k_wgrad_plw<%d>" : "k_wgrad_pl<%d>", math_planes());
diff --git a/iswm_amd/csrc/conv_wgrad_pl.hip b/iswm_amd/csrc/conv_wgrad_pl.hip
--- a/iswm_amd/csrc/conv_wgrad_pl.hip
+++ b/iswm_amd/csrc/conv_wgrad_pl.hip
@@ -443,7 +443,7 @@
 }
 
 template <int NP>
-__global__ __launch_bounds__(512, 2) void k_wgrad_pls(const WgArgs a) {
+__device__ __forceinline__ void wgrad_pls_item(const WgArgs& a, const int L, const int bid) {
     constexpr int MW = 4;
     constexpr int KS = 16;
     constexpr int PLANE = KS * 256;
@@ -456,16 +456,15 @@
     const int t = threadIdx.x, lane = t & 63;
     const int wave = __builtin_amdgcn_readfirstlane(t >> 6);
     const int tiles = a.MT * a.NT;
-    const int L = xcd_remap(blockIdx.x, gridDim.x);
     int split = L / tiles, tile = L - split * tiles;
     int mt = tile / a.NT;
     int nt = tile - mt * a.NT;
     if (a.rect == 2) {
-        const int idx = blockIdx.x >> 3, per_split = (a.NT >> 3) * a.MT;
+        const int idx = bid >> 3, per_split = (a.NT >> 3) * a.MT;
         split = idx / per_split;
         const int rem = idx - split * per_split;
         mt = rem % a.MT;
-        nt = (rem / a.MT) * 8 + (blockIdx.x & 7);
+        nt = (rem / a.MT) * 8 + (bid & 7);
     }
     int r_oh0 = 0, r_ow0 = 0, r_h = a.Ho, r_w = a.Wo, r_dh = 0, r_dw = 0;
     int p_begin = split * a.psplit;
@@ -522,6 +521,9 @@
         }
         const int d_oh = KS / GW_, d_ow = KS - d_oh * GW_;
         const bool fast_adv = d_oh + 1 <= r_h;
+        const int a_ldx = a.ldx, a_ldy = a.ldy, a_H = a.H, a_W = a.W, a_Ho = a.Ho, a_Wo = a.Wo, a_stride = a.stride;
+        const int a_always = a.always, a_rect = a.rect;
+        const long long a_dyps = a.dyps, a_xps = a.xps;
         auto issue = [&](int kc) __attribute__((always_inline)) {
             const int p = p_begin + kc * KS + kr;
             const bool pin = p < p_end;
@@ -529,7 +531,7 @@
             long long apst;
             const unsigned char* bsrc[2];
             long long bpst[2];
-            if (a.rect) {
+            if (a_rect) {
                 if (kc > 0) {
                     if (fast_adv) {
                         int ow = pow_ + d_ow;
@@ -548,14 +550,14 @@
                 }
                 const int oh = r_oh0 + poh, ow = r_ow0 + pow_;
                 const bool va = pin && aok;
-                asrc = va ? abase + (size_t)((pn * a.Ho + oh) * a.Wo + ow) * a.ldy * 2 : zrow;
-                apst = va ? a.dyps : 0;
-                const size_t xpix = (size_t)((pn * a.H + oh + r_dh) * a.W + ow + r_dw);
+                asrc = va ? abase + (size_t)((pn * a_Ho + oh) * a_Wo + ow) * a_ldy * 2 : zrow;
+                apst = va ? a_dyps : 0;
+                const size_t xpix = (size_t)((pn * a_H + oh + r_dh) * a_W + ow + r_dw);
 #pragma unroll
                 for (int i = 0; i < 2; ++i) {
                     const bool v = pin && bok[i];
-                    bsrc[i] = v ? bbase[i] + xpix * a.ldx * 2 : zrow;
-                    bpst[i] = v ? a.xps : 0;
+                    bsrc[i] = v ? bbase[i] + xpix * a_ldx * 2 : zrow;
+                    bpst[i] = v ? a_xps : 0;
                 }
                 const unsigned dstr = lds_base + (kc & 3) * STAGE + rg * 1024;
 #pragma unroll
@@ -566,14 +568,14 @@
                     for (int pl = 0; pl < NP; ++pl) glds16b(bsrc[i] + pl * bpst[i], dstr + (1 + i) * IMG + pl * PLANE);
                 return;
             }
-            asrc = (pin && aok) ? abase + (size_t)p * a.ldy * 2 : zrow;
-            apst = (pin && aok) ? a.dyps : 0;
-            if (a.always) {
+            asrc = (pin && aok) ? abase + (size_t)p * a_ldy * 2 : zrow;
+            apst = (pin && aok) ? a_dyps : 0;
+            if (a_always) {
 #pragma unroll
                 for (int i = 0; i < 2; ++i) {
                     const bool v = pin && bok[i];
-                    bsrc[i] = v ? bbase[i] + (size_t)p * a.ldx * 2 : zrow;
-                    bpst[i] = v ? a.xps : 0;
+                    bsrc[i] = v ? bbase[i] + (size_t)p * a_ldx * 2 : zrow;
+                    bpst[i] = v ? a_xps : 0;
                 }
             } else {
                 if (kc > 0) {
@@ -594,10 +596,10 @@
                 }
 #pragma unroll
                 for (int i = 0; i < 2; ++i) {
-                    const int ih = poh * a.stride + dh[i], iw = pow_ * a.stride + dw[i];
-                    const bool v = pin && bok[i] && (unsigned)ih < (unsigned)a.H && (unsigned)iw < (unsigned)a.W;
-                    bsrc[i] = v ? bbase[i] + (size_t)((pn * a.H + ih) * a.W + iw) * a.ldx * 2 : zrow;
-                    bpst[i] = v ? a.xps : 0;
+                    const int ih = poh * a_stride + dh[i], iw = pow_ * a_stride + dw[i];
+                    const bool v = pin && bok[i] && (unsigned)ih < (unsigned)a_H && (unsigned)iw < (unsigned)a_W;
+                    bsrc[i] = v ? bbase[i] + (size_t)((pn * a_H + ih) * a_W + iw) * a_ldx * 2 : zrow;
+                    bpst[i] = v ? a_xps : 0;
                 }
             }
             const unsigned dst = lds_base + (kc & 3) * STAGE + rg * 1024;
@@ -704,25 +706,60 @@
         return;
     }
     float* out = a.out;
+    const int Cout = a.Cout, Ktot = a.Ktot;
     const int li = lane & 31, lh = lane >> 5;
 #pragma unroll
     for (int nb = 0; nb < NBW; ++nb) {
         const int col = n0 + wn4 * 64 + nb * 32 + li;
-        const bool cok = col < a.Ktot;
+        const bool cok = col < Ktot;
 #pragma unroll
         for (int mb = 0; mb < 2; ++mb)
 #pragma unroll
             for (int r = 0; r < 16; ++r) {
                 const int row = m0 + wm * 64 + mb * 32 + (r & 3) + 8 * (r >> 2) + 4 * lh;
-                if (cok && row < a.Cout) out[(size_t)row * a.Ktot + col] = acc[mb][nb][r];
-            }
-    }
-}
-
-__global__ __launch_bounds__(256) void k_reduce_slabs_frag(const float4* __restrict__ slabs, float* __restrict__ dw, int tiles,
-                                                           int NT, int nsplit, int Cout, int Ktot) {
-    const int64_t total = (int64_t)tiles * 8192;
-    for (int64_t i = blockIdx.x * (int64_t)blockDim.x + threadIdx.x; i < total; i += (int64_t)gridDim.x * blockDim.x) {
+                if (cok && row < Cout) out[(size_t)row * Ktot + col] = acc[mb][nb][r];
+            }
+    }
+}
+
+template <int NP>
+__global__ __launch_bounds__(512, 2) void k_wgrad_pls(const WgArgs a) {
+    wgrad_pls_item<NP>(a, xcd_remap(blockIdx.x, gridDim.x), blockIdx.x);
+}
+
+constexpr int WG_GROUP_MAX = 4;
+struct WgGroupArgs {
+    WgArgs p[WG_GROUP_MAX];
+    int first[WG_GROUP_MAX + 1];
+};
+
+template <int NP>
+__global__ __launch_bounds__(512, 2) void k_wgrad_plsg(const WgGroupArgs g) {
+    const int L = xcd_remap(blockIdx.x, gridDim.x);
+    const int i = (L >= g.first[1] ? 1 : 0) + (L >= g.first[2] ? 1 : 0) + (L >= g.first[3] ? 1 : 0);
+    wgrad_pls_item<NP>(g.p[i], L - g.first[i], blockIdx.x);
+}
+
+struct RdMember {
+    const float4* slabs;
+    float* dw;
+    int tiles, NT, nsplit, Cout, Ktot;
+};
+struct RdGroupArgs {
+    RdMember m[WG_GROUP_MAX];
+    int first[WG_GROUP_MAX + 1];
+};
+
+__global__ __launch_bounds__(256) void k_reduce_slabs_frag(const RdGroupArgs g) {
+    const int64_t all = (int64_t)g.first[WG_GROUP_MAX] * 8192;
+    for (int64_t base = blockIdx.x * (int64_t)blockDim.x; base < all; base += (int64_t)gridDim.x * blockDim.x) {
+        const int gt = (int)(base >> 13);
+        const int mi = (gt >= g.first[1] ? 1 : 0) + (gt >= g.first[2] ? 1 : 0) + (gt >= g.first[3] ? 1 : 0);
+        const RdMember& r = g.m[mi];
+        const int nsplit = r.nsplit, NT = r.NT, Cout = r.Cout, Ktot = r.Ktot;
+        const int64_t total = (int64_t)r.tiles * 8192;
+        const int64_t i = base - (int64_t)g.first[mi] * 8192 + threadIdx.x;
+        const float4* __restrict__ slabs = r.slabs;
         float4 s = slabs[i];
         int k = 1;
         for (; k + 3 < nsplit; k += 4) {
@@ -744,7 +781,7 @@
         const int col = nt * 256 + wn * 64 + nb * 32 + (lane & 31);
         const int row = mt * 128 + wm * 64 + mb * 32 + 8 * q + 4 * (lane >> 5);
         if (col < Ktot) {
-            float* o = dw + (size_t)row * Ktot + col;
+            float* o = r.dw + (size_t)row * Ktot + col;
             if (row < Cout) o[0] = s.x;
             if (row + 1 < Cout) o[(size_t)Ktot] = s.y;
             if (row + 2 < Cout) o[(size_t)2 * Ktot] = s.z;
@@ -764,28 +801,64 @@
     return wgrad_pl_wide(d->KH * d->KW * d->Cin, d->KH * d->KW, (int64_t)d->N * d->Ho * d->Wo);
 }
 
-void plan_wgrad_pl(int Cout, int Ktot, int taps, int64_t P, int* nsplit, int* psplit) {
-    const int wide = wgrad_pl_wide(Ktot, taps, P);
-    const int tn = wide ? 256 : 128;
-    const int64_t tiles = (int64_t)((Cout + 127) / 128) * ((Ktot + tn - 1) / tn);
-    const double step_us = wide ? 1.45 : 0.75;
-    const double slab_us = (double)Cout * Ktot * 8.0 / 4.0e6;
-    int64_t maxs = (P + 255) / 256;
-    if (maxs > 256) maxs = 256;
+struct WgPlanIn {
+    int Cout, Ktot, taps;
+    int64_t P;
+};
+static void plan_wgrad_group(int n, const WgPlanIn* in, int* nsplit, int* psplit) {
+    int64_t tiles[WG_GROUP_MAX], maxs_i[WG_GROUP_MAX], Pmax = 0;
+    double step_us[WG_GROUP_MAX], slab_us[WG_GROUP_MAX];
+    for (int i = 0; i < n; ++i) {
+        const int wide = wgrad_pl_wide(in[i].Ktot, in[i].taps, in[i].P);
+        const int tn = wide ? 256 : 128;
+        tiles[i] = (int64_t)((in[i].Cout + 127) / 128) * ((in[i].Ktot + tn - 1) / tn);
+        step_us[i] = wide ? 1.45 : 0.75;
+        slab_us[i] = (double)in[i].Cout * in[i].Ktot * 8.0 / 4.0e6;
+        maxs_i[i] = std::min<int64_t>(256, (in[i].P + 255) / 256);
+        Pmax = std::max(Pmax, in[i].P);
+        psplit[i] = (int)((in[i].P + 31) / 32 * 32);
+        nsplit[i] = 1;
+    }
+    const int64_t maxs = std::min<int64_t>(256, (Pmax + 255) / 256);
     double best = 1e300;
-    *psplit = (int)((P + 31) / 32 * 32);
-    *nsplit = 1;
     for (int64_t ns = 1; ns <= maxs; ++ns) {
-        const int64_t ps = ((P + ns - 1) / ns + 31) / 32 * 32;
-        const int64_t nsp = (P + ps - 1) / ps;
-        const int64_t rounds = (tiles * nsp + 255) / 256;
-        const double tm = (double)rounds * ((double)(ps / 32) + 6.0) * step_us + (nsp > 1 ? (double)nsp * slab_us + 5.0 : 0.0);
+        const int64_t len = ((Pmax + ns - 1) / ns + 31) / 32 * 32;
+        int64_t items = 0, ps_c[WG_GROUP_MAX], nsp_c[WG_GROUP_MAX];
+        double slabs = 0.0, long_steps = 0.0, long_us = 0.0;
+        bool reduce = false;
+        for (int i = 0; i < n; ++i) {
+            const int64_t P = in[i].P;
+            const int64_t cut = P == Pmax ? ns : std::max<int64_t>(1, std::min(maxs_i[i], (P + len - 1) / len));
+            const int64_t ps = ((P + cut - 1) / cut + 31) / 32 * 32;
+            const int64_t nsp = (P + ps - 1) / ps;
+            ps_c[i] = ps;
+            nsp_c[i] = nsp;
+            items += tiles[i] * nsp;
+            const double steps = (double)(ps / 32) + 6.0;
+            if (steps * step_us[i] > long_steps * long_us) {
+                long_steps = steps;
+                long_us = step_us[i];
+            }
+            if (nsp > 1) {
+                slabs += (double)nsp * slab_us[i];
+                reduce = true;
+            }
+        }
+        const int64_t rounds = (items + 255) / 256;
+        const double tm = (double)rounds * long_steps * long_us + (reduce ? slabs + 5.0 : 0.0);
         if (tm < best) {
             best = tm;
-            *psplit = (int)ps;
-            *nsplit = (int)nsp;
-        }
-    }
+            for (int i = 0; i < n; ++i) {
+                psplit[i] = (int)ps_c[i];
+                nsplit[i] = (int)nsp_c[i];
+            }
+        }
+    }
+}
+
+void plan_wgrad_pl(int Cout, int Ktot, int taps, int64_t P, int* nsplit, int* psplit) {
+    const WgPlanIn in = {Cout, Ktot, taps, P};
+    plan_wgrad_group(1, &in, nsplit, psplit);
 }
 
 void launch_wgrad_pl(const WgArgs& a, int planes, int wide, hipStream_t s) {
@@ -800,6 +873,19 @@
         if (planes == 1) hipLaunchKernelGGL(k_wgrad_pl<1>, grid, blk, 0, s, a);
         else hipLaunchKernelGGL(k_wgrad_pl<3>, grid, blk, 0, s, a);
     }
+}
+
+static RdMember rd_member(const WgArgs& a, const float* slabs, float* dw) {
+    RdMember m;
+    m.slabs = reinterpret_cast<const float4*>(slabs);
+    m.dw = dw;
+    m.tiles = a.MT * a.NT;
+    m.NT = a.NT; m.nsplit = a.nsplit; m.Cout = a.Cout; m.Ktot = a.Ktot;
+    return m;
+}
+
+static void launch_reduce_frag(const RdGroupArgs& r, hipStream_t s) {
+    hipLaunchKernelGGL(k_reduce_slabs_frag, dim3(stream_grid((int64_t)r.first[WG_GROUP_MAX] * 8192, 256)), dim3(256), 0, s, r);
 }
 
 }
@@ -873,6 +959,21 @@
 }
 }
 
+static int wg_fill(const iswm_conv_desc* d, const void* xp, int64_t x_ps, const void* dyp, int64_t dy_ps, WgArgs* pa) {
+    WgArgs& a = *pa;
+    a.dy = (const unsigned short*)dyp; a.x = (const unsigned short*)xp;
+    a.dyps = dy_ps * 2; a.xps = x_ps * 2;
+    a.N = d->N; a.H = d->H; a.W = d->W; a.Cin = d->Cin; a.Ho = d->Ho; a.Wo = d->Wo; a.Cout = d->Cout;
+    a.KH = d->KH; a.KW = d->KW; a.stride = d->stride; a.pad = d->pad; a.dil = d->dil; a.ldx = d->ldx; a.ldy = d->ldy;
+    a.P = d->N * d->Ho * d->Wo;
+    a.Ktot = d->KH * d->KW * d->Cin;
+    a.MT = (d->Cout + 127) / 128;
+    const int wide = wgrad_pl_wide(a.Ktot, d->KH * d->KW, a.P);
+    a.NT = wide ? (a.Ktot + 255) / 256 : (a.Ktot + 127) / 128;
+    a.always = (d->KH == 1 && d->KW == 1 && d->pad == 0 && d->stride == 1) ? 1 : 0;
+    return wide;
+}
+
 extern "C" size_t iswm_conv2d_wgrad_planes_workspace(const iswm_conv_desc* d) {
     if (!d) return 0;
     int ns, ps;
@@ -893,15 +994,7 @@
     const int planes = iswm_get_conv_math() == 2 ? 1 : 3;
     ISWM_REQUIRE(planes == 1 || (x_ps % 8 == 0 && dy_ps % 8 == 0 && x_ps > 0 && dy_ps > 0), "wgrad_planes: bad plane stride");
     WgArgs a{};
-    a.dy = (const unsigned short*)dyp; a.x = (const unsigned short*)xp;
-    a.dyps = dy_ps * 2; a.xps = x_ps * 2;
-    a.N = d->N; a.H = d->H; a.W = d->W; a.Cin = d->Cin; a.Ho = d->Ho; a.Wo = d->Wo; a.Cout = d->Cout;
-    a.KH = d->KH; a.KW = d->KW; a.stride = d->stride; a.pad = d->pad; a.dil = d->dil; a.ldx = d->ldx; a.ldy = d->ldy;
-    a.P = d->N * d->Ho * d->Wo;
-    a.Ktot = d->KH * d->KW * d->Cin;
-    a.MT = (d->Cout + 127) / 128;
-    const int wide = wgrad_pl_wide(a.Ktot, d->KH * d->KW, a.P);
-    a.NT = wide ? (a.Ktot + 255) / 256 : (a.Ktot + 127) / 128;
+    const int wide = wg_fill(d, xp, x_ps, dyp, dy_ps, &a);
     int64_t p_plan = a.P;
     bool similar = false;
     a.rect = (wide && wgrad_rect_mode(d, &p_plan, a.tap_order, &similar)) ? 1 : 0;
@@ -910,7 +1003,6 @@
     }
     plan_wgrad_pl(d->Cout, a.Ktot, d->KH * d->KW, p_plan, &a.nsplit, &a.psplit);
     a.vote = (d->pad >= 4 && !a.rect) ? 1 : 0;
-    a.always = (d->KH == 1 && d->KW == 1 && d->pad == 0 && d->stride == 1) ? 1 : 0;
     const size_t need = iswm_conv2d_wgrad_planes_workspace(d);
     ISWM_REQUIRE(workspace_bytes >= need && (need == 0 || (workspace && aligned16(workspace))),
                  "wgrad_planes: workspace too small (%zu < %zu)", workspace_bytes, need);
@@ -919,10 +1011,10 @@
     if (int e = check_launch("wgrad_planes")) return e;
     if (a.nsplit > 1) {
         if (wide) {
-            const int tiles = a.MT * a.NT;
-            hipLaunchKernelGGL(k_reduce_slabs_frag, dim3(stream_grid((int64_t)tiles * 8192, 256)), dim3(256), 0,
-                               (hipStream_t)stream, reinterpret_cast<const float4*>(workspace), dw, tiles, a.NT, a.nsplit,
-                               d->Cout, a.Ktot);
+            RdGroupArgs r{};
+            r.m[0] = rd_member(a, workspace, dw);
+            for (int i = 1; i <= WG_GROUP_MAX; ++i) r.first[i] = r.m[0].tiles;
+            launch_reduce_frag(r, (hipStream_t)stream);
         } else {
             launch_reduce_slabs(workspace, dw, (int64_t)d->Cout * a.Ktot / 4, a.nsplit, (hipStream_t)stream);
         }
@@ -930,3 +1022,99 @@
     }
     return 0;
 }
+
+extern "C" int iswm_conv2d_wgrad_planes_group_ok(const iswm_conv_desc* d) {
+    if (!iswm_conv2d_wgrad_planes_ok(d)) return 0;
+    return (wgrad_pl_kernel_kind(d) == 2 && !wgrad_rect_mode(d, nullptr, nullptr)) ? 1 : 0;
+}
+
+struct WgGroupPlan {
+    int nsplit[WG_GROUP_MAX], psplit[WG_GROUP_MAX], first[WG_GROUP_MAX + 1];
+    size_t slab0[WG_GROUP_MAX], bytes;
+};
+static int wg_group_plan(int n, const iswm_conv_desc* d, WgGroupPlan* pl) {
+    ISWM_REQUIRE(d && n >= 1 && n <= WG_GROUP_MAX, "wgrad_planes_group: 1 to %d members", WG_GROUP_MAX);
+    WgPlanIn in[WG_GROUP_MAX];
+    for (int i = 0; i < n; ++i) {
+        if (int e = wg_validate(&d[i])) return e;
+        ISWM_REQUIRE(iswm_conv2d_wgrad_planes_group_ok(&d[i]), "wgrad_planes_group: member %d is not eligible (Cin %d Cout %d k %d pad %d)",
+                     i, d[i].Cin, d[i].Cout, d[i].KH, d[i].pad);
+        in[i] = {d[i].Cout, d[i].KH * d[i].KW * d[i].Cin, d[i].KH * d[i].KW, (int64_t)d[i].N * d[i].Ho * d[i].Wo};
+    }
+    plan_wgrad_group(n, in, pl->nsplit, pl->psplit);
+    pl->bytes = 0;
+    pl->first[0] = 0;
+    for (int i = 0; i < n; ++i) {
+        const int tiles = ((d[i].Cout + 127) / 128) * ((in[i].Ktot + 255) / 256);
+        pl->first[i + 1] = pl->first[i] + tiles * pl->nsplit[i];
+        pl->slab0[i] = pl->bytes;
+        if (pl->nsplit[i] > 1) pl->bytes += (size_t)pl->nsplit[i] * tiles * 32768 * sizeof(float);
+    }
+    for (int i = n + 1; i <= WG_GROUP_MAX; ++i) pl->first[i] = pl->first[n];
+    return 0;
+}
+
+extern "C" int iswm_conv2d_wgrad_planes_group_pays(int n, const iswm_conv_desc* d) {
+    if (!d || n < 2 || n > WG_GROUP_MAX) return 0;
+    int tiles = 0;
+    for (int i = 0; i < n; ++i) {
+        if (!iswm_conv2d_wgrad_planes_group_ok(&d[i])) return 0;
+        tiles += ((d[i].Cout + 127) / 128) * ((d[i].KH * d[i].KW * d[i].Cin + 255) / 256);
+    }
+    return tiles <= 128 ? 1 : 0;
+}
+
+extern "C" size_t iswm_conv2d_wgrad_planes_group_workspace(int n, const iswm_conv_desc* d) {
+    WgGroupPlan pl;
+    return wg_group_plan(n, d, &pl) ? 0 : pl.bytes;
+}
+
+extern "C" int iswm_conv2d_wgrad_planes_group_plan(int n, const iswm_conv_desc* d, int* nsplit) {
+    WgGroupPlan pl;
+    if (int e = wg_group_plan(n, d, &pl)) return e;
+    ISWM_REQUIRE(nsplit, "wgrad_planes_group_plan: null result");
+    for (int i = 0; i < n; ++i) nsplit[i] = pl.nsplit[i];
+    return 0;
+}
+
+extern "C" int iswm_conv2d_wgrad_planes_group(int n, const iswm_conv_desc* d, const void* const* xp, const int64_t* x_ps,
+                                              const void* const* dyp, const int64_t* dy_ps, float* const* dw, float* workspace,
+                                              size_t workspace_bytes, iswm_stream_t stream) {
+    WgGroupPlan pl;
+    if (int e = wg_group_plan(n, d, &pl)) return e;
+    ISWM_REQUIRE(xp && x_ps && dyp && dy_ps && dw, "wgrad_planes_group: null array");
+    ISWM_REQUIRE(workspace_bytes >= pl.bytes && (pl.bytes == 0 || (workspace && aligned16(workspace))),
+                 "wgrad_planes_group: workspace too small (%zu < %zu)", workspace_bytes, pl.bytes);
+    const int planes = iswm_get_conv_math() == 2 ? 1 : 3;
+    WgGroupArgs ga{};
+    RdGroupArgs rd{};
+    int nrd = 0;
+    for (int i = 0; i < n; ++i) {
+        ISWM_REQUIRE(xp[i] && dyp[i] && dw[i] && aligned16(xp[i]) && aligned16(dyp[i]) && aligned16(dw[i]),
+                     "wgrad_planes_group: bad pointer (member %d)", i);
+        ISWM_REQUIRE(planes == 1 || (x_ps[i] % 8 == 0 && dy_ps[i] % 8 == 0 && x_ps[i] > 0 && dy_ps[i] > 0),
+                     "wgrad_planes_group: bad plane stride (member %d)", i);
+        WgArgs& a = ga.p[i];
+        wg_fill(&d[i], xp[i], x_ps[i], dyp[i], dy_ps[i], &a);
+        a.nsplit = pl.nsplit[i];
+        a.psplit = pl.psplit[i];
+        float* slabs = reinterpret_cast<float*>(reinterpret_cast<char*>(workspace) + pl.slab0[i]);
+        a.out = a.nsplit > 1 ? slabs : dw[i];
+        if (a.nsplit > 1) {
+            rd.m[nrd] = rd_member(a, slabs, dw[i]);
+            rd.first[nrd + 1] = rd.first[nrd] + rd.m[nrd].tiles;
+            ++nrd;
+        }
+    }
+    for (int i = 0; i <= WG_GROUP_MAX; ++i) ga.first[i] = pl.first[i];
+    for (int i = nrd + 1; i <= WG_GROUP_MAX; ++i) rd.first[i] = rd.first[nrd];
+    dim3 grid(pl.first[n]), blk(512);
+    if (planes == 1) hipLaunchKernelGGL(k_wgrad_plsg<1>, grid, blk, 0, (hipStream_t)stream, ga);
+    else hipLaunchKernelGGL(k_wgrad_plsg<3>, grid, blk, 0, (hipStream_t)stream, ga);
+    if (int e = check_launch("wgrad_planes_group")) return e;
+    if (nrd > 0) {
+        launch_reduce_frag(rd, (hipStream_t)stream);
+        return check_launch("wgrad_planes_group_reduce");
+    }
+    return 0;
+}
diff --git a/iswm_amd/network/_hip.py b/iswm_amd/network/_hip.py
--- a/iswm_amd/network/_hip.py
+++ b/iswm_amd/network/_hip.py
@@ -158,9 +158,12 @@
         g.alg_cin, g.alg_cout = self.in_channels, self.out_channels
         return g
 
-    def write_wgrad(self, x, dy, g, sink):
+    def write_wgrad(self, x, dy, g, sink, later=None):
         p = self.weight
         if not p.requires_grad:
+            return
+        if later is not None:
+            later.add(self, x, dy, g)
             return
         buf = sink.target(p)
         v = buf.permute(0, 2, 3, 1)
@@ -358,6 +361,39 @@
 
 
 _BN3_FUSE = True
+_WGRAD_GROUP = True
+
+
+class WgradGroup:
+
+    def __init__(self, sink):
+        self.sink, self.items = sink, []
+
+    def add(self, conv, x, dy, g):
+        self.items.append((conv, x, dy, g))
+
+    def flush(self):
+        items, self.items = self.items, []
+        work = []
+        for conv, x, dy, g in items:
+            buf = self.sink.target(conv.weight)
+            v = buf.permute(0, 2, 3, 1)
+            work.append((conv, x, dy, g, buf, v if (not conv.needs_pack() and v.is_contiguous()) else None))
+        grouped = [w for w in work if ops.wgrad_group_ok(w[1], w[2], w[3])]
+        done = {}
+        for i in range(0, len(grouped), ops.WGRAD_GROUP_MAX):
+            part = [(w[1], w[2], w[3], w[5]) for w in grouped[i:i + ops.WGRAD_GROUP_MAX]]
+            if not ops.wgrad_group_pays(part):
+                continue
+            for w, dw in zip(grouped[i:], ops.conv2d_wgrad_group(part)):
+                done[id(w[0])] = dw
+        for conv, x, dy, g, buf, v in work:
+            dw = done.get(id(conv))
+            if dw is None:
+                dw = ops.conv2d_wgrad(x, dy, g, v)
+            if v is None:
+                ops.unpad_weights(dw, buf)
+            self.sink.done(conv.weight)
 
 
 def _bn_stats_request(up):
@@ -397,7 +433,7 @@
     return dy, dres
 
 
-def cba_bwd(conv, bn, ctx, dout, sink, need_dx=True, dx=None, accumulate=False, up=None):
+def cba_bwd(conv, bn, ctx, dout, sink, need_dx=True, dx=None, accumulate=False, up=None, later=None):
     x, g = ctx["x"], ctx["g"]
     sep = ctx.get("sep")
     dy, dres = cba_bwd_bn(conv, bn, ctx, dout, sink, need_dx=need_dx or sep is not None)
@@ -407,7 +443,7 @@
         if conv.is_dw3x3():
             return conv.bwd_fused(dy, sink, need_dx, dx, accumulate), dres
         return conv.bwd(dy, sink, need_dx, dx, accumulate), dres
-    conv.write_wgrad(x, dy, g, sink)
+    conv.write_wgrad(x, dy, g, sink, later)
     if conv.bias is not None and conv.bias.requires_grad:
         ops.unpad_weights(ops.colsum(dy).view(-1, 1, 1, 1), sink.target(conv.bias).view(-1, 1, 1, 1))
         sink.done(conv.bias)
diff --git a/iswm_amd/network/backbone/resnet.py b/iswm_amd/network/backbone/resnet.py
--- a/iswm_amd/network/backbone/resnet.py
+++ b/iswm_amd/network/backbone/resnet.py
@@ -51,15 +51,18 @@
     def bwd(self, dout, sink, need_dx=True, up=None, dx0=None):
         c1, c2, c3, cd = self._saved
         self._saved = None
-        d2, dres = _hip.cba_bwd(self.conv3, self.bn3, c3, dout, sink, up=c2)
-        d1, _ = _hip.cba_bwd(self.conv2, self.bn2, c2, d2, sink, up=c1)
+        wg = _hip.WgradGroup(sink) if _hip._WGRAD_GROUP else None
+        d2, dres = _hip.cba_bwd(self.conv3, self.bn3, c3, dout, sink, up=c2, later=wg)
+        d1, _ = _hip.cba_bwd(self.conv2, self.bn2, c2, d2, sink, up=c1, later=wg)
         if cd is not None:
-            dx, _ = _hip.cba_bwd(self.conv1, self.bn1, c1, d1, sink, dx=dx0, accumulate=dx0 is not None)
-            dx, _ = _hip.cba_bwd(self.downsample[0], self.downsample[1], cd, dres, sink, dx=dx, accumulate=True)
+            dx, _ = _hip.cba_bwd(self.conv1, self.bn1, c1, d1, sink, dx=dx0, accumulate=dx0 is not None, later=wg)
+            dx, _ = _hip.cba_bwd(self.downsample[0], self.downsample[1], cd, dres, sink, dx=dx, accumulate=True, later=wg)
         else:
-            dx, _ = _hip.cba_bwd(self.conv1, self.bn1, c1, d1, sink, dx=dres, accumulate=True, up=up)
+            dx, _ = _hip.cba_bwd(self.conv1, self.bn1, c1, d1, sink, dx=dres, accumulate=True, up=up, later=wg)
             if dx0 is not None:
                 dx = ops.add_inplace(dx, dx0)
+        if wg is not None:
+            wg.flush()
         return dx
 
     def out_channels_of(self, cin):
diff --git a/iswm_amd/ops.py b/iswm_amd/ops.py
--- a/iswm_amd/ops.py
+++ b/iswm_amd/ops.py
@@ -463,6 +463,61 @@
     return dw_ohwi
 
 
+WGRAD_GROUP_MAX = 4
+
+
+def _wgrad_group_desc(x, dy, g):
+    if not (isinstance(x, Planes) and isinstance(dy, Planes) and planes_on() and g.cout % 8 == 0):
+        return None
+    d = ConvDesc(g.n, g.h, g.w, g.cin, g.ho, g.wo, g.cout, g.kh, g.kw, g.stride, g.pad, g.dil, pgeom(x)[4], pgeom(dy)[4])
+    return d if _lib.load().iswm_conv2d_wgrad_planes_group_ok(ctypes.byref(d)) else None
+
+
+def wgrad_group_ok(x, dy, g):
+    return _wgrad_group_desc(x, dy, g) is not None
+
+
+def wgrad_group_pays(items):
+    if not 2 <= len(items) <= WGRAD_GROUP_MAX:
+        return False
+    ds = (ConvDesc * len(items))(*[_wgrad_group_desc(it[0], it[1], it[2]) for it in items])
+    return bool(_lib.load().iswm_conv2d_wgrad_planes_group_pays(len(items), ds))
+
+
+def wgrad_group_plan(items):
+    ds = (ConvDesc * len(items))(*[_wgrad_group_desc(x, dy, g) for x, dy, g, _ in items])
+    ns = (ctypes.c_int * len(items))()
+    call("iswm_conv2d_wgrad_planes_group_plan", len(items), ds, ns)
+    return list(ns)
+
+
+def conv2d_wgrad_group(items):
+    n = len(items)
+    if not 1 <= n <= WGRAD_GROUP_MAX:
+        raise ValueError("conv2d_wgrad_group takes 1 to %d members, got %d" % (WGRAD_GROUP_MAX, n))
+    ds, dws = [], []
+    for x, dy, g, dw in items:
+        d = _wgrad_group_desc(x, dy, g)
+        if d is None:
+            raise ValueError("conv2d_wgrad_group: %s is not eligible for the grouped launch" % g.tag())
+        if dw is None:
+            dw = torch.empty((g.cout, g.kh, g.kw, g.cin), dtype=torch.float32, device=x.t.device)
+        _check_w(dw, g)
+        ds.append(d)
+        dws.append(dw)
+    darr = (ConvDesc * n)(*ds)
+    need = _lib.load().iswm_conv2d_wgrad_planes_group_workspace(n, darr)
+    ws = torch.empty((need // 4,), dtype=torch.float32, device=dws[0].device) if need else None
+    xs, dys = [it[0] for it in items], [it[1] for it in items]
+    psx = (ctypes.c_int64 * n)(*[pgeom(x)[5] for x in xs])
+    psy = (ctypes.c_int64 * n)(*[pgeom(dy)[5] for dy in dys])
+    name = _kernel_name(ds[0], 8) + "+reduce" if KPROF is not None else ""
+    with _timed_multi(name, [it[2] for it in items], group=True):
+        call("iswm_conv2d_wgrad_planes_group", n, darr, _ptr_array([x.t for x in xs]), psx, _ptr_array([dy.t for dy in dys]), psy,
+             _ptr_array(dws), _p(ws), need, _stream())
+    return dws
+
+
 ASPP_TILE_ROWS = 144
 _ASPP_PLANS = {}
 _ASPP_FUSED = True
@@ -552,9 +607,9 @@
 
 class _timed_multi:
 
-    def __init__(self, name, geoms):
+    def __init__(self, name, geoms, group=False):
         self.on = KPROF is not None and KPROF.wants(name)
-        self.name, self.geoms = name, geoms
+        self.name, self.geoms, self.group = name, geoms, group
 
     def __enter__(self):
         if self.on:
@@ -566,8 +621,11 @@
             b = torch.cuda.Event(enable_timing=True)
             b.record()
             g0 = self.geoms[0]
-            tag = "n%d %dx%d c%d->%dx%d aspp d%s" % (g0.n, g0.h, g0.w, g0.alg_cin, len(self.geoms), g0.alg_cout,
-                                                    "/".join(str(g.dil) for g in self.geoms if g.kh > 1))
+            if self.group:
+                tag = "group " + " + ".join(g.tag() for g in self.geoms)
+            else:
+                tag = "n%d %dx%d c%d->%dx%d aspp d%s" % (g0.n, g0.h, g0.w, g0.alg_cin, len(self.geoms), g0.alg_cout,
+                                                        "/".join(str(g.dil) for g in self.geoms if g.kh > 1))
             KPROF.add(self.name, self.a, b, sum(g.flops() for g in self.geoms), tag)
         return False
 
```
